# evanwang1990/FMwR

Measured on AMD Instinct MI355X. Metric: training examples/sec, 10Mx1M sparse FM SGD, higher is better.
Workload: dtype f32

## Files before the change

fmwr_amd/_lib.py:

```python
import ctypes as C
import os

_PKG = os.path.dirname(os.path.abspath(__file__))
LIB_PATH = os.environ.get("FMX_LIB_PATH") or os.path.join(_PKG, "libfmx.so")

OK, ERR_INVALID, ERR_HIP, ERR_NOGPU, ERR_STATE = 0, 1, 2, 3, 4
TASK_CLASSIFICATION, TASK_REGRESSION, TASK_RANKING = 10, 20, 30
SOLVER_MCMC, SOLVER_ALS, SOLVER_SGD, SOLVER_FTRL, SOLVER_TDAP = 100, 200, 300, 500, 600
MODE_SEQUENTIAL, MODE_MINIBATCH = 0, 1
LINK_NONE, LINK_LOGISTIC, LINK_CLAMP, LINK_PROBIT = 0, 1, 2, 3
DIV_REL_SCORE, DIV_REL_MINMAX = 0, 1
SIM_COSINE, SIM_DOT = 0, 1
REDUCE_MEAN, REDUCE_SUM = 0, 1
COLUMNS_UNIFORM, COLUMNS_ZIPF = 1, 2
EVAL_LL, EVAL_AUC, EVAL_ACC, EVAL_RMSE, EVAL_MSE, EVAL_MAE = 0, 111, 222, 333, 444, 555
EVAL_PAIR_ACC, EVAL_BPR = 666, 777
KERNEL_ROWS_FORWARD, KERNEL_COLS_UPDATE, KERNEL_SCALAR, KERNEL_SEQ, KERNEL_ALS_SWEEP = 0, 1, 2, 3, 4

SYMBOLS = [
    "fmx_last_error", "fmx_device_count", "fmx_config_default", "fmx_engine_create", "fmx_engine_destroy", "fmx_set_params",
    "fmx_get_params", "fmx_engine_save", "fmx_engine_load", "fmx_matrix_from_rlist", "fmx_matrix_from_dgc", "fmx_matrix_from_csr", "fmx_matrix_synthetic", "fmx_matrix_synthetic_fields", "fmx_matrix_synthetic_iid", "fmx_matrix_synthetic_ragged", "fmx_matrix_synthetic_values", "fmx_train_stream", "fmx_matrix_set_labels", "fmx_matrix_set_fields", "fmx_matrix_destroy",
    "fmx_matrix_info", "fmx_matrix_export", "fmx_matrix_scales", "fmx_matrix_normalize", "fmx_predict", "fmx_train", "fmx_train_grid", "fmx_train_order", "fmx_num_batches",
    "fmx_step", "fmx_grad", "fmx_grad_buffer", "fmx_grad_elem_bytes", "fmx_grad_layout", "fmx_grad_begin", "fmx_grad_chunk", "fmx_apply_chunk", "fmx_apply", "fmx_sync", "fmx_stream", "fmx_predict_device",
    "fmx_als_plan_info", "fmx_als_tiled_info", "fmx_als_order_info", "fmx_als_carry_q", "fmx_als_vsweep", "fmx_mcmc_vsweep", "fmx_als_train", "fmx_mcmc_train", "fmx_mcmc_train_from", "fmx_mcmc_v_hyper", "fmx_evaluate", "fmx_train_tracked", "fmx_trace_size", "fmx_trace_get", "fmx_trace_params",
    "fmx_profile_enable", "fmx_profile_get", "fmx_profile_reset", "fmx_rows_tune_info", "fmx_matrix_rows_form", "fmx_measure_gather", "fmx_measure_gather_occ", "fmx_measure_gather_matrix", "fmx_rccl_selftest",
    "fmx_get_rows", "fmx_set_rows", "fmx_init_normal", "fmx_compact_info", "fmx_compact_count", "fmx_compact_reserve", "fmx_grad_compact", "fmx_compact_records", "fmx_apply_compact",
    "fmx_vsweep_device", "fmx_group_info", "fmx_source_open", "fmx_source_next", "fmx_source_close",
    "fmx_apply_compact_parts", "fmx_layout_info", "fmx_owner_configure", "fmx_owner_info", "fmx_rows_pack", "fmx_rows_unpack",
    "fmx_topk", "fmx_topk_device", "fmx_contrib", "fmx_contrib_device", "fmx_contrib_summary",
    "fmx_matrix_pairs", "fmx_matrix_pairs_hard",
    "fmx_heldout_rank", "fmx_heldout_rank_device", "fmx_heldout_metrics",
    "fmx_rank_lists", "fmx_rank_lists_device", "fmx_topk_lists", "fmx_topk_lists_device", "fmx_project", "fmx_project_device",
    "fmx_fold_in", "fmx_fold_in_pairs",
    "fmx_diversify", "fmx_diversify_device",
    "fmx_neighbors", "fmx_neighbors_device",
    "fmx_interactions", "fmx_interactions_device", "fmx_interactions_summary",
    "fmx_metrics", "fmx_metrics_device",
    "fmx_predict_calibrated", "fmx_predict_calibrated_device", "fmx_reliability", "fmx_reliability_device",
    "fmx_calibrate_platt", "fmx_calibrate_platt_device", "fmx_calibrate_isotonic", "fmx_calibrate_isotonic_device",
    "fmx_matrix_take", "fmx_matrix_take_device", "fmx_split_assign", "fmx_split_assign_device", "fmx_matrix_select", "fmx_matrix_select_device",
    "fmx_free_device", "fmx_matrix_split_entries", "fmx_row_permutation", "fmx_row_permutation_device",
    "fmx_matrix_column_stats", "fmx_matrix_column_stats_device", "fmx_column_map_select", "fmx_column_map_select_device",
    "fmx_column_map_hash", "fmx_column_map_hash_device", "fmx_matrix_remap_columns", "fmx_matrix_remap_columns_device",
]
COLUMNS_BY_ROWS, COLUMNS_BY_ENTRIES = 0, 1
RARE_DROP, RARE_BUCKET = 0, 1
COMBINE_KEEP, COMBINE_SUM, COMBINE_FIRST = 0, 1, 2
COLUMN_DROP = 0xFFFFFFFF
SPLIT_ROWS, SPLIT_WITHIN_GROUPS, SPLIT_GROUPS = 0, 1, 2
SPLIT_ORDER_HASH, SPLIT_ORDER_TAIL = 0, 1
SPLIT_NO_PART = 0xFFFFFFFF
MET_VALUES, MET_COUNTS = 6, 4
MET_AUC, MET_LOGLOSS, MET_ACCURACY, MET_BRIER, MET_MEAN_PRED, MET_MEAN_LABEL = 0, 1, 2, 3, 4, 5
MET_MSE, MET_RMSE, MET_MAE, MET_MEAN_ERR = 0, 1, 2, 3
MET_ROWS, MET_POSITIVES, MET_PAIRS2, MET_CORRECT = 0, 1, 2, 3
CAL_NONE, CAL_PLATT, CAL_STEPS = 0, 1, 2
BINS_WIDTH, BINS_MASS = 0, 1
CAL_VALUES = 4
CAL_ECE, CAL_MCE, CAL_BRIER, CAL_LOGLOSS = 0, 1, 2, 3


TEST_HOOKS = ["fmx_debug_fail_next_plan_build", "fmx_debug_fail_next_comm_init", "fmx_debug_lose_next_seq_multiplier", "fmx_debug_stall_next_persistent_sweep",
              "fmx_debug_contrib_summary_chunk", "fmx_debug_foldin_slab", "fmx_debug_heldout_limits", "fmx_debug_pairs_hard_chunk", "fmx_debug_lists_limits", "fmx_debug_diversify_limits", "fmx_debug_neighbors_limits", "fmx_debug_interactions_limits", "fmx_debug_metrics_limits", "fmx_debug_take_limits", "fmx_debug_calibrate_limits", "fmx_debug_columns_limits", "fmx_debug_matrix_flags", "fmx_debug_cols_launches",
              "fmx_debug_long_launches", "fmx_debug_rows_launches", "fmx_debug_rows_merged_launches",
              "fmx_debug_rows_sched_launches", "fmx_debug_rows_sched_id_limit", "fmx_debug_rows_sched_export",
              "fmx_debug_rows_pace_launches", "fmx_debug_rows_pace_counters", "fmx_debug_rows_pace_counters_of", "fmx_debug_rows_pace_poison", "fmx_debug_rows_pace_trace"]


class Config(C.Structure):
    _fields_ = [
        ("struct_size", C.c_uint32), ("task", C.c_int32), ("solver", C.c_int32), ("num_factor", C.c_int32),
        ("keep_w0", C.c_int32), ("keep_w1", C.c_int32),
        ("l2_w0", C.c_double), ("l1_w1", C.c_double), ("l2_w1", C.c_double), ("l1_v", C.c_double), ("l2_v", C.c_double),
        ("learn_rate", C.c_double),
        ("alpha_w", C.c_double), ("alpha_v", C.c_double), ("beta_w", C.c_double), ("beta_v", C.c_double),
        ("random_step", C.c_int32), ("mode", C.c_int32), ("batch_rows", C.c_int64),
        ("min_target", C.c_double), ("max_target", C.c_double),
        ("device", C.c_int32), ("batch_reduce", C.c_int32), ("gamma", C.c_double), ("tile_rows", C.c_int64),
        ("state_fp64", C.c_int32), ("exchange_chunks", C.c_int32), ("n_gpus", C.c_int32), ("als_max_levels", C.c_int32), ("seq_reassociate", C.c_int32), ("gpus_share_device", C.c_int32),
    ]


class FieldsSpec(C.Structure):
    _fields_ = [("struct_size", C.c_uint32), ("n_dense", C.c_int32), ("n_fields", C.c_int32), ("reserved", C.c_int32),
                ("field_vocab", C.c_void_p), ("skew", C.c_double), ("seed", C.c_uint64)]


class TrackConfig(C.Structure):
    _fields_ = [("struct_size", C.c_uint32), ("metric", C.c_int32), ("step_size", C.c_int64), ("convergence", C.c_double),
                ("keep_params", C.c_int32), ("reserved", C.c_int32)]


class SplitSpec(C.Structure):
    _fields_ = [("struct_size", C.c_uint32), ("scope", C.c_int32), ("order", C.c_int32), ("n_folds", C.c_int32), ("hold_count", C.c_int64),
                ("hold_fraction", C.c_double), ("min_keep", C.c_int64), ("seed", C.c_uint64), ("salt", C.c_uint64)]


class ColumnRule(C.Structure):
    _fields_ = [("struct_size", C.c_uint32), ("by", C.c_int32), ("min_count", C.c_int64), ("max_count", C.c_int64), ("max_features", C.c_int64),
                ("keep_prefix", C.c_uint32), ("rare", C.c_int32), ("n_segments", C.c_int32), ("reserved", C.c_int32), ("segment_base", C.c_void_p)]


class Calibrator(C.Structure):
    _fields_ = [("struct_size", C.c_uint32), ("kind", C.c_int32), ("n_groups", C.c_int64), ("max_steps", C.c_int32), ("link", C.c_int32),
                ("platt", C.c_void_p), ("n_steps", C.c_void_p), ("thr", C.c_void_p), ("val", C.c_void_p)]


class FmxError(RuntimeError):
    def __init__(self, status, message):
        super().__init__(message)
        self.status = status


_lib = None


def lib():
    global _lib
    if _lib is None:
        if not os.path.exists(LIB_PATH):
            raise ImportError(f"{LIB_PATH} is missing: build the HIP library first (python -m fmwr_amd.build). "
                              "fmwr_amd has no CPU fallback.")
        L = C.CDLL(LIB_PATH)
        L.fmx_last_error.restype = C.c_char_p
        for name in SYMBOLS + TEST_HOOKS:
            if name != "fmx_last_error":
                getattr(L, name).restype = C.c_int
        L.fmx_matrix_pairs_hard.argtypes = [C.c_void_p, C.c_void_p, C.c_void_p, C.c_void_p, C.c_int32, C.c_int32, C.c_uint64, C.c_int64,
                                            C.POINTER(C.c_void_p)]
        L.fmx_fold_in.argtypes = [C.c_void_p, C.c_void_p, C.c_void_p, C.c_int64, C.c_double, C.c_double, C.c_int32, C.c_int32, C.c_void_p, C.c_void_p,
                                  C.c_void_p, C.c_void_p]
        L.fmx_fold_in_pairs.argtypes = L.fmx_fold_in.argtypes
        L.fmx_diversify.argtypes = [C.c_void_p, C.c_void_p, C.c_int64, C.c_int32, C.c_void_p, C.c_void_p, C.c_int32, C.c_double, C.c_int32, C.c_void_p,
                                    C.c_void_p, C.c_void_p]
        L.fmx_diversify_device.argtypes = L.fmx_diversify.argtypes
        L.fmx_neighbors.argtypes = [C.c_void_p, C.c_void_p, C.c_void_p, C.c_int32, C.c_int32, C.c_int32, C.c_void_p, C.c_void_p]
        L.fmx_neighbors_device.argtypes = [C.c_void_p, C.c_void_p, C.c_int64, C.c_int64, C.c_void_p, C.c_int32, C.c_int32, C.c_int32, C.c_void_p, C.c_void_p]
        L.fmx_debug_neighbors_limits.argtypes = [C.c_int64, C.c_int64]
        L.fmx_interactions.argtypes = [C.c_void_p, C.c_void_p, C.c_int32, C.c_void_p, C.c_void_p, C.c_void_p]
        L.fmx_interactions_device.argtypes = [C.c_void_p, C.c_void_p, C.c_int64, C.c_int64, C.c_int32, C.c_void_p, C.c_void_p, C.c_void_p]
        L.fmx_interactions_summary.argtypes = [C.c_void_p, C.c_void_p, C.c_void_p, C.c_int32, C.c_void_p, C.c_void_p, C.c_void_p]
        L.fmx_debug_interactions_limits.argtypes = [C.c_int32, C.c_int32, C.c_int64]
        L.fmx_metrics.argtypes = [C.c_void_p, C.c_void_p, C.c_void_p, C.c_int64, C.c_int, C.c_void_p, C.c_void_p]
        L.fmx_metrics_device.argtypes = [C.c_void_p, C.c_void_p, C.c_int64, C.c_int64, C.c_void_p, C.c_int64, C.c_int, C.c_void_p, C.c_void_p]
        L.fmx_debug_metrics_limits.argtypes = [C.c_int32, C.c_int32, C.c_int64]
        L.fmx_predict_calibrated.argtypes = [C.c_void_p, C.c_void_p, C.c_void_p, C.c_int64, C.POINTER(Calibrator), C.c_int, C.c_void_p]
        L.fmx_predict_calibrated_device.argtypes = [C.c_void_p, C.c_void_p, C.c_int64, C.c_int64, C.c_void_p, C.c_int64, C.POINTER(Calibrator), C.c_int, C.c_void_p]
        L.fmx_reliability.argtypes = [C.c_void_p, C.c_void_p, C.c_void_p, C.c_int64, C.c_int32, C.c_int32, C.POINTER(Calibrator), C.c_int] + [C.c_void_p] * 6
        L.fmx_reliability_device.argtypes = [C.c_void_p, C.c_void_p, C.c_int64, C.c_int64, C.c_void_p, C.c_int64, C.c_int32, C.c_int32, C.POINTER(Calibrator),
                                             C.c_int] + [C.c_void_p] * 6
        L.fmx_calibrate_platt.argtypes = [C.c_void_p, C.c_void_p, C.c_void_p, C.c_int64, C.c_double, C.c_int32, C.c_void_p, C.c_void_p, C.c_void_p]
        L.fmx_calibrate_platt_device.argtypes = [C.c_void_p, C.c_void_p, C.c_int64, C.c_int64, C.c_void_p, C.c_int64, C.c_double, C.c_int32, C.c_void_p, C.c_void_p,
                                                 C.c_void_p]
        L.fmx_calibrate_isotonic.argtypes = [C.c_void_p, C.c_void_p, C.c_void_p, C.c_int64, C.c_int32, C.c_void_p, C.c_void_p, C.c_void_p]
        L.fmx_calibrate_isotonic_device.argtypes = [C.c_void_p, C.c_void_p, C.c_int64, C.c_int64, C.c_void_p, C.c_int64, C.c_int32, C.c_void_p, C.c_void_p, C.c_void_p]
        L.fmx_debug_calibrate_limits.argtypes = [C.c_int64]
        L.fmx_matrix_take.argtypes = [C.c_void_p, C.c_void_p, C.c_int64, C.POINTER(C.c_void_p)]
        L.fmx_matrix_take_device.argtypes = L.fmx_matrix_take.argtypes
        L.fmx_split_assign.argtypes = [C.c_int, C.c_int64, C.c_void_p, C.c_int64, C.POINTER(SplitSpec), C.c_void_p]
        L.fmx_split_assign_device.argtypes = L.fmx_split_assign.argtypes
        L.fmx_matrix_select.argtypes = [C.c_void_p, C.c_void_p, C.c_uint32, C.c_int32, C.POINTER(C.c_void_p), C.c_void_p]
        L.fmx_matrix_select_device.argtypes = [C.c_void_p, C.c_void_p, C.c_uint32, C.c_int32, C.POINTER(C.c_void_p), C.POINTER(C.c_void_p)]
        L.fmx_free_device.argtypes = [C.c_void_p]
        L.fmx_matrix_split_entries.argtypes = [C.c_void_p, C.c_int32, C.c_int64, C.c_double, C.c_int64, C.c_uint64, C.c_uint64, C.POINTER(C.c_void_p),
                                               C.POINTER(C.c_void_p)]
        L.fmx_row_permutation.argtypes = [C.c_int, C.c_int64, C.c_uint64, C.c_uint64, C.c_void_p]
        L.fmx_row_permutation_device.argtypes = L.fmx_row_permutation.argtypes
        L.fmx_debug_take_limits.argtypes = [C.c_int32, C.c_int32, C.c_int64]
        L.fmx_matrix_column_stats.argtypes = [C.c_void_p, C.c_void_p, C.c_void_p]
        L.fmx_matrix_column_stats_device.argtypes = L.fmx_matrix_column_stats.argtypes
        L.fmx_column_map_select.argtypes = [C.c_int, C.c_uint32, C.c_void_p, C.POINTER(ColumnRule), C.c_void_p, C.POINTER(C.c_uint32), C.c_void_p]
        L.fmx_column_map_select_device.argtypes = L.fmx_column_map_select.argtypes
        L.fmx_column_map_hash.argtypes = [C.c_int, C.c_uint32, C.c_uint32, C.c_uint64, C.c_uint64, C.c_uint32, C.c_void_p, C.POINTER(C.c_uint32)]
        L.fmx_column_map_hash_device.argtypes = L.fmx_column_map_hash.argtypes
        L.fmx_matrix_remap_columns.argtypes = [C.c_void_p, C.c_void_p, C.c_uint32, C.c_int32, C.POINTER(C.c_void_p)]
        L.fmx_matrix_remap_columns_device.argtypes = L.fmx_matrix_remap_columns.argtypes
        L.fmx_debug_columns_limits.argtypes = [C.c_int32, C.c_int64, C.c_int64]
        L.fmx_debug_matrix_flags.argtypes = [C.c_void_p, C.c_void_p]
        _lib = L
    return _lib


def check(status):
    if status != OK:
        raise FmxError(status, lib().fmx_last_error().decode("utf-8", "replace"))


def default_config():
    cfg = Config()
    check(lib().fmx_config_default(C.byref(cfg)))
    return cfg
```

fmwr_amd/csrc/fm_batch_kernels.hip:

```cpp
#include <atomic>
#include <mutex>
#include <utility>
#include <vector>

#include "fmx_internal.h"
#include "fm_probit.h"
#include "fmx_test_hooks.h"

#ifndef FMX_U
#define FMX_U 4
#endif
#ifndef FMX_SPARSE_WAVES
#define FMX_SPARSE_WAVES 4
#endif
#ifndef FMX_DENSE_WAVES
#define FMX_DENSE_WAVES 4
#endif
#ifndef FMX_U_LARGE
#define FMX_U_LARGE 4
#endif
#ifndef FMX_U_SMALL
#define FMX_U_SMALL 8
#endif

// ... 347 lines not shown
    const int64_t row = R0 + s * NG + gid;
    const int64_t ra = row < a.nrows ? row : a.nrows, rb = row + 1 < a.nrows ? row + 1 : a.nrows;
    const int64_t ta = a.row_ptr[a.r0 + ra] - lo, tb = a.row_ptr[a.r0 + rb] - lo;
    pe[s] = (uint32_t)(ta < cnt ? ta : cnt) | ((uint32_t)(tb < cnt ? tb : cnt) << 16);
  }
  {
    uint32_t id[PER];
#pragma unroll
    for (int u = 0; u < PER; ++u) {
      const int i = tid + u * WG_THREADS;
      id[u] = i < cnt ? a.col[lo + i] : 0u;
    }
#pragma unroll
    for (int u = 0; u < PER; ++u) {
      const int i = tid + u * WG_THREADS;
      if (i < cnt) stage[i] = id[u];
    }
  }
  __syncthreads();

  const T* __restrict__ Vt = reinterpret_cast<const T*>(a.V) + lig * VEC;
  const T* __restrict__ wt = a.w ? reinterpret_cast<const T*>(a.w) : reinterpret_cast<const T*>(a.V);
  const bool k1 = h.k1 != 0;
  const int last = cnt > 0 ? cnt - 1 : 0;
  static_assert(MERGE_STAGE < (1 << 16), "positions are kept in 16 bits");
  uint32_t hd[MERGE_SLOTS];
  int left = 0;
#pragma unroll
  for (int s = 0; s < MERGE_SLOTS; ++s) {
    const int p0 = (int)(pe[s] & 0xFFFFu), p1 = (int)(pe[s] >> 16);
    const uint32_t v = stage[p0 < last ? p0 : last];
    hd[s] = p0 < p1 ? v : DONE;
    left += p1 - p0;
  }
  double sm[MERGE_SLOTS][VEC], qm[MERGE_SLOTS][VEC], lin[MERGE_SLOTS];
#pragma unroll
  for (int s = 0; s < MERGE_SLOTS; ++s) {
#pragma unroll
    for (int i = 0; i < VEC; ++i) { sm[s][i] = 0.0; qm[s][i] = 0.0; }
    lin[s] = h.k0 ? a.scal[SC_W0] : 0.0;
  }

  uint32_t safe = 0u;
  for (; left > 0; left -= U) {
    uint32_t eid[U];
    int esl[U];
#pragma unroll
    for (int u = 0; u < U; ++u) {
      uint32_t best = hd[0];
      int sel = 0;
#pragma unroll
      for (int s = 1; s < MERGE_SLOTS; ++s)
        if (hd[s] < best) { best = hd[s]; sel = s; }
      const bool live = best != DONE;
      eid[u] = live ? best : safe;
      esl[u] = live ? sel : MERGE_SLOTS;
      safe = eid[u];
      uint32_t nxt = 0u;
#pragma unroll
      for (int s = 0; s < MERGE_SLOTS; ++s)
        if (esl[u] == s) { pe[s] += 1u; nxt = pe[s]; }
      const int np = (int)(nxt & 0xFFFFu), ne = (int)(nxt >> 16);
      const uint32_t nx = stage[np < last ? np : last];
      const uint32_t nh = np < ne ? nx : DONE;
#pragma unroll
      for (int s = 0; s < MERGE_SLOTS; ++s)
        if (esl[u] == s) hd[s] = nh;
    }
    float4 vv[U];
    T wv[U];
#pragma unroll
    for (int u = 0; u < U; ++u) {
      vv[u] = gather_row(Vt + ((size_t)eid[u] << RowStride<T, LPR>::v(a.vsh)));
      wv[u] = wt[(size_t)eid[u] << RowStride<T, LPR>::w(a.wsh)];
    }
#pragma unroll
    for (int u = 0; u < U; ++u) {
      const double x = 1.0;
      const double wx = (double)wv[u] * x;
      double tmp[VEC], tsq[VEC];
      slice_get(vv[u], tmp);
#pragma unroll
      for (int i = 0; i < VEC; ++i) { tmp[i] = tmp[i] * x; tsq[i] = tmp[i] * tmp[i]; }
#pragma unroll
      for (int s = 0; s < MERGE_SLOTS; ++s) {
        if (esl[u] == s) {
          if (k1) lin[s] += wx;
#pragma unroll
          for (int i = 0; i < VEC; ++i) {
            sm[s][i] += tmp[i];
            if constexpr (U == 1) qm[s][i] += tsq[i]; else qm[s][i] += tmp[i] * tmp[i];
          }
        }
      }
    }
  }

  int eg = tid / LPR;
  asm volatile("" : "+v"(eg));
#pragma unroll
  for (int s = 0; s < MERGE_SLOTS; ++s) {
    const int64_t row = R0 + s * NG + eg;
    const bool have = row < a.nrows;
    double pair = 0.0;
#pragma unroll
    for (int i = 0; i < VEC; ++i) pair += 0.5 * (sm[s][i] * sm[s][i] - qm[s][i]);
#pragma unroll
    for (int off = LPR / 2; off > 0; off >>= 1) pair += __shfl_xor(pair, off);
    const double y_hat = lin[s] + pair;
    if constexpr (TRAIN) {
      double mult = 0.0;
      if (have) {
        mult = grad_mult(h, y_hat, a.y[a.r0 + row]);
        float4 srow = slice_make(sm[s], T());
        srow = embed_store<LPR>(srow, lig, (float)mult, a.embed);
        *reinterpret_cast<float4*>(reinterpret_cast<T*>(a.S) + (size_t)row * KP + lig * VEC) = srow;
        if (lig == 0) reinterpret_cast<T*>(a.amul)[row] = (T)mult;
      }
      if (lig == 0) red[s * NG + eg] = mult;
    } else {
      if (have && lig == 0 && a.yhat) a.yhat[row] = link_apply(h, y_hat, a.link, a.pn_y);
    }
  }
  if constexpr (TRAIN) {
    __syncthreads();
    if (tid % 64 == 0) {
      const int s = tid / 64;
      if (R0 + (int64_t)s * NG < a.nrows) {
        double g0 = 0.0, q0 = 0.0;
        for (int i = 0; i < NG; ++i) { const double m = red[s * NG + i]; g0 += m; q0 += m * m; }
        a.partials[2 * ((size_t)blockIdx.x * MERGE_SLOTS + s)] = g0;
        a.partials[2 * ((size_t)blockIdx.x * MERGE_SLOTS + s) + 1] = q0;
      }
    }
  }
}

#ifndef FMX_ROWS_PACE_EVERY
#define FMX_ROWS_PACE_EVERY 24
#endif
#ifndef FMX_ROWS_PACE_LEAD
#define FMX_ROWS_PACE_LEAD 2
#endif
#ifndef FMX_ROWS_PACE_SLEEP
#define FMX_ROWS_PACE_SLEEP 30
#endif
constexpr int PACE_MAX_CHECKINS = (SCHED_STAGE_STEPS - 1) / FMX_ROWS_PACE_EVERY;
constexpr int64_t PACE_STEP_CYCLES = 2120;
static_assert((int64_t)PACE_MAX_CHECKINS * 3 * FMX_ROWS_PACE_SLEEP * 64 * 10 <= SCHED_STAGE_STEPS * PACE_STEP_CYCLES, "check-ins x the longest sleep: at most a tenth of the longest block's walk");
static_assert((int64_t)((120 - 1) / FMX_ROWS_PACE_EVERY) * 3 * FMX_ROWS_PACE_SLEEP * 64 * 10 <= 120 * PACE_STEP_CYCLES, "the same for the headline's 120-step blocks");

__device__ __forceinline__ void pace_sleep(int units) {
  switch (units) {
    case 5: __builtin_amdgcn_s_sleep(5); break;
    case 10: __builtin_amdgcn_s_sleep(10); break;
    case 15: __builtin_amdgcn_s_sleep(15); break;
    case 20: __builtin_amdgcn_s_sleep(20); break;
    case 30: __builtin_amdgcn_s_sleep(30); break;
    case 40: __builtin_amdgcn_s_sleep(40); break;
    case 60: __builtin_amdgcn_s_sleep(60); break;
    case 80: __builtin_amdgcn_s_sleep(80); break;
    case 90: __builtin_amdgcn_s_sleep(90); break;
    case 120: __builtin_amdgcn_s_sleep(120); break;
    default: break;
  }
}

template <bool UNIFORM, bool PIPE, bool DEAL = false, bool PACE = false, bool TRACE = false>
__global__ __launch_bounds__(WG_THREADS, 4) void fm_rows_sched_k(RowsArgs a, Hyper h) {
  using T = float;
  constexpr int LPR = 4, VEC = 4, KP = LPR * VEC;
  constexpr int NG = WG_THREADS / LPR;
  constexpr int PER = MERGE_STAGE / WG_THREADS;
  static_assert(MERGE_STAGE == SCHED_STAGE_STEPS * NG && MERGE_SLOTS == 4, "the stage holds SCHED_STAGE_STEPS steps of one word per lane group");
  static_assert(UNIFORM || !PIPE, "only the unrolled walk has a round to request together");
  static_assert(!(UNIFORM && DEAL), "a DEAL schedule is walked as a MERGE one");
  static_assert(!(UNIFORM && (PACE || TRACE)), "the pace and its trace belong to the MERGE and DEAL walks");
  __shared__ uint32_t stage[MERGE_STAGE];
  __shared__ double red[MERGE_RPW];
  __shared__ uint32_t places[DEAL ? NG : 1];
  __shared__ uint32_t pace_box;

  const int tid = threadIdx.x;
  const int gid = tid / LPR;
  const int lig = tid % LPR;
  const int64_t R0 = (int64_t)blockIdx.x * MERGE_RPW;
  if constexpr (PACE) { if (tid == 0) pace_box = 0u; }
  const uint32_t w_hi = a.sched_dir[blockIdx.x + 1];
  uint32_t w_lo = a.sched_dir[blockIdx.x];
  if constexpr (DEAL) {
    const bool hdr = w_hi - w_lo >= (uint32_t)NG;
    if (tid < NG) places[tid] = hdr ? a.sched[(size_t)w_lo + tid] : 0u;
    w_lo += hdr ? (uint32_t)NG : 0u;
  }
  const int cnt = (w_hi - w_lo < (uint32_t)MERGE_STAGE) ? (int)(w_hi - w_lo) : MERGE_STAGE;
  const int steps = UNIFORM ? (cnt / NG) & ~3 : cnt / NG;
  {
    uint32_t id[PER];
#pragma unroll
    for (int u = 0; u < PER; ++u) {
      const int i = tid + u * WG_THREADS;
      id[u] = i < cnt ? a.sched[(size_t)w_lo + i] : SCHED_BUBBLE;
    }
#pragma unroll
    for (int u = 0; u < PER; ++u) {
      const int i = tid + u * WG_THREADS;
      if (i < cnt) stage[i] = id[u];
    }
  }
  __syncthreads();

  const __amdgpu_buffer_rsrc_t v_rsrc = table_rsrc(a.V, a.sched_vbytes);
  const __amdgpu_buffer_rsrc_t w_rsrc = table_rsrc(a.w ? a.w : a.V, a.w ? a.sched_wbytes : a.sched_vbytes);
  const bool k1 = h.k1 != 0;
  const int vsh = RowStride<T, LPR>::v(a.vsh) + 2, wsh = RowStride<T, LPR>::w(a.wsh) + 2;
  const uint32_t lane_off = (uint32_t)(lig * VEC * sizeof(T));
  double sm[MERGE_SLOTS][VEC], qm[MERGE_SLOTS][VEC], lin[MERGE_SLOTS];
#pragma unroll
  for (int s = 0; s < MERGE_SLOTS; ++s) {
#pragma unroll
    for (int i = 0; i < VEC; ++i) { sm[s][i] = 0.0; qm[s][i] = 0.0; }
    lin[s] = h.k0 ? a.scal[SC_W0] : 0.0;
  }
  const uint32_t* __restrict__ mine = stage + gid;

  if constexpr (UNIFORM) {
    for (int t = 0; t < steps; t += MERGE_SLOTS) {
      uint32_t wd[MERGE_SLOTS];
#pragma unroll
      for (int j = 0; j < MERGE_SLOTS; ++j) wd[j] = mine[(t + j) * NG];
      float4 vv[MERGE_SLOTS];
      T wv[MERGE_SLOTS];
      if constexpr (PIPE) {
#pragma unroll
        for (int j = 0; j < MERGE_SLOTS; ++j) {
          const bool live = wd[j] != SCHED_BUBBLE;
          const uint32_t c = wd[j] & SCHED_MAX_P;
          vv[j] = buf_row(v_rsrc, live ? (c << vsh) + lane_off : BUF_SKIP, T());
          wv[j] = buf_elem(w_rsrc, live ? c << wsh : BUF_SKIP, T());
        }
      }
#pragma unroll
      for (int j = 0; j < MERGE_SLOTS; ++j) {
        if constexpr (!PIPE) {
          const bool live = wd[j] != SCHED_BUBBLE;
          const uint32_t c = wd[j] & SCHED_MAX_P;
          vv[j] = buf_row(v_rsrc, live ? (c << vsh) + lane_off : BUF_SKIP, T());
          wv[j] = buf_elem(w_rsrc, live ? c << wsh : BUF_SKIP, T());
          asm volatile("s_waitcnt vmcnt(0)" ::: "memory");
        }
        const double x = 1.0;
        const double wx = (double)wv[j] * x;
        double tmp[VEC], tsq[VEC];
        slice_get(vv[j], tmp);
#pragma unroll
        for (int i = 0; i < VEC; ++i) { tmp[i] = tmp[i] * x; tsq[i] = tmp[i] * tmp[i]; }
        if (k1) lin[j] += wx;
#pragma unroll
        for (int i = 0; i < VEC; ++i) { sm[j][i] += tmp[i]; qm[j][i] += tsq[i]; }
      }
    }
  } else {
    uint32_t* pace_ctr = nullptr;
    int64_t pace_groups = 0;
    int pace_at = 0, pace_k = 0, pace_slept = 0;
    uint32_t pace_seen = 0;
    if constexpr (PACE) {
      const uint32_t lab = blockIdx.x & 7u;
      pace_ctr = a.pace + (size_t)(a.pace_set * 8 + (int)lab) * PACE_LINE;
      pace_groups = (int64_t)(a.pace_div + (lab < a.pace_rem ? 1u : 0u));
      pace_at = a.pace_every;
      if (blockIdx.x == 0 && tid < 8 && a.pace_zero)
        __hip_atomic_store(a.pace + (size_t)((a.pace_set ^ 1) * 8 + tid) * PACE_LINE, 0u, __ATOMIC_RELAXED, __HIP_MEMORY_SCOPE_AGENT);
    }
    uint64_t* trace = nullptr;
    if constexpr (TRACE) trace = a.pace_trace + ((size_t)blockIdx.x * (WG_THREADS / 64) + tid / 64) * PACE_TRACE_WORDS;
    for (int t = 0; t < steps; ++t) {
      if constexpr (TRACE) {
        if ((t & 15) == 0 && (tid & 63) == 0) trace[1 + (t >> 4)] = __builtin_amdgcn_s_memrealtime();
      }
      const uint32_t wd = mine[t * NG];
      const bool live = wd != SCHED_BUBBLE;
      const uint32_t c = wd & SCHED_MAX_P;
      const int esl = live ? (int)(wd >> 30) : MERGE_SLOTS;
      const float4 vv = buf_row(v_rsrc, live ? (c << vsh) + lane_off : BUF_SKIP, T());
      const T wv = buf_elem(w_rsrc, live ? c << wsh : BUF_SKIP, T());
      const double x = 1.0;
      const double wx = (double)wv * x;
      double tmp[VEC], tsq[VEC];
      slice_get(vv, tmp);
#pragma unroll
      for (int i = 0; i < VEC; ++i) { tmp[i] = tmp[i] * x; tsq[i] = tmp[i] * tmp[i]; }
#pragma unroll
      for (int s = 0; s < MERGE_SLOTS; ++s) {
        if (esl == s) {
          if (k1) lin[s] += wx;
#pragma unroll
          for (int i = 0; i < VEC; ++i) { sm[s][i] += tmp[i]; qm[s][i] += tsq[i]; }
        }
      }
      if constexpr (PACE) {
        if (t == pace_at) {
          ++pace_k;
          if (tid == 64 * (pace_k & 3)) pace_seen = __hip_atomic_fetch_add(pace_ctr, a.pace_inc, __ATOMIC_RELAXED, __HIP_MEMORY_SCOPE_AGENT);
        } else if (t == pace_at + 1) {
          if (tid == 64 * (pace_k & 3))
            __hip_atomic_store(&pace_box, (uint32_t)pace_k << 24 | (pace_seen < 0xFFFFFFu ? pace_seen : 0xFFFFFFu), __ATOMIC_RELAXED, __HIP_MEMORY_SCOPE_WORKGROUP);
          const uint32_t box = (uint32_t)__builtin_amdgcn_readfirstlane((int)__hip_atomic_load(&pace_box, __ATOMIC_RELAXED, __HIP_MEMORY_SCOPE_WORKGROUP));
          const int64_t k = (int64_t)(box >> 24), seen = (int64_t)(box & 0xFFFFFFu);
          const int64_t lead2 = 2 * (int64_t)a.pace_every * (k * pace_groups - seen) - (int64_t)(a.pace_every - 1) * pace_groups;
          const int64_t thr2 = 2 * (int64_t)a.pace_lead * pace_groups;
          const int level = k == 0 ? 0 : lead2 > 3 * thr2 ? 3 : lead2 > 2 * thr2 ? 2 : lead2 > thr2 ? 1 : 0;
          if (level) { pace_sleep(level * a.pace_sleep); pace_slept += 1 + (level << 16); }
          pace_at += a.pace_every;
        }
      }
    }
    if constexpr (TRACE) {
      if ((tid & 63) == 0) {
        trace[1 + ((steps + 15) >> 4)] = __builtin_amdgcn_s_memrealtime();
        trace[0] = (uint64_t)(__builtin_amdgcn_s_getreg((31 << 11) | 20) & 15u) | (uint64_t)steps << 8 | (uint64_t)pace_slept << 32;
      }
    }
  }

  int eg = tid / LPR;
  asm volatile("" : "+v"(eg));
  uint32_t place = 0;
  if constexpr (DEAL) place = places[eg];
#pragma unroll
  for (int s = 0; s < MERGE_SLOTS; ++s) {
    const int at = DEAL ? (int)((place >> (8 * s)) & 255u) : s * NG + eg;
    const int64_t row = R0 + at;
    const bool have = row < a.nrows;
    double pair = 0.0;
#pragma unroll
    for (int i = 0; i < VEC; ++i) pair += 0.5 * (sm[s][i] * sm[s][i] - qm[s][i]);
#pragma unroll
    for (int off = LPR / 2; off > 0; off >>= 1) pair += __shfl_xor(pair, off);
    const double y_hat = lin[s] + pair;
    double mult = 0.0;
    if (have) {
      mult = grad_mult(h, y_hat, a.y[a.r0 + row]);
      float4 srow = slice_make(sm[s], T());
      srow = embed_store<LPR>(srow, lig, (float)mult, a.embed);
      *reinterpret_cast<float4*>(reinterpret_cast<T*>(a.S) + (size_t)row * KP + lig * VEC) = srow;
      if (lig == 0) reinterpret_cast<T*>(a.amul)[row] = (T)mult;
    }
    if (lig == 0) red[at] = mult;
  }
  __syncthreads();
  if (tid % 64 == 0) {
    const int s = tid / 64;
    if (R0 + (int64_t)s * NG < a.nrows) {
      double g0 = 0.0, q0 = 0.0;
      for (int i = 0; i < NG; ++i) { const double m = red[s * NG + i]; g0 += m; q0 += m * m; }
      a.partials[2 * ((size_t)blockIdx.x * MERGE_SLOTS + s)] = g0;
      a.partials[2 * ((size_t)blockIdx.x * MERGE_SLOTS + s) + 1] = q0;
    }
  }
}

template <typename T, int LPR, bool TRAIN>
__global__ __launch_bounds__(WG_THREADS) void fm_rows_forward_dyn_k(RowsArgs a, Hyper h) {
  using vec_t = typename Slice<T>::vec;
  constexpr int VEC = Slice<T>::N;
  constexpr int KP = LPR * VEC;
  constexpr int GROUPS = WG_THREADS / LPR;
  constexpr int RPW = 4 * GROUPS;
  constexpr int RU = FMX_U_LARGE;
  constexpr int PER = (RU + LPR - 1) / LPR;
  __shared__ int next_row;
  __shared__ double red[TRAIN ? RPW : 1];
  const int tid = threadIdx.x;
  const int grp = tid / LPR, lig = tid % LPR;
  const int lane0 = (tid & 63) - lig;
  const int64_t R0 = (int64_t)blockIdx.x * RPW;
  const int rows_here = (int)((R0 + RPW < a.nrows ? R0 + RPW : a.nrows) - R0);
  if (tid == 0) next_row = GROUPS;
  if (TRAIN) for (int i = tid; i < RPW; i += WG_THREADS) red[i] = 0.0;
  __syncthreads();
  const T* __restrict__ Vt = reinterpret_cast<const T*>(a.V) + lig * VEC;
  const T* __restrict__ wt = a.w ? reinterpret_cast<const T*>(a.w) : reinterpret_cast<const T*>(a.V);
  const bool k1 = h.k1 != 0;
  const int64_t last = a.row_ptr[a.r0 + R0 + rows_here] - 1;
  int r = grp;
  while (r < rows_here) {
    const int64_t ta = a.row_ptr[a.r0 + R0 + r], tb = a.row_ptr[a.r0 + R0 + r + 1];
    double s[VEC], q[VEC];
#pragma unroll
    for (int i = 0; i < VEC; ++i) { s[i] = 0.0; q[i] = 0.0; }
    double lin = h.k0 ? a.scal[SC_W0] : 0.0;
    auto load_round = [&](int64_t t, uint32_t* id, uint32_t* xb) {
#pragma unroll
      for (int v = 0; v < PER; ++v) {
        const int64_t at = t + lig + v * LPR;
        const int64_t ac = at <= last ? (at >= 0 ? at : 0) : (last >= 0 ? last : 0);
        id[v] = a.col[ac];
        xb[v] = a.unit ? 0x3f800000u : __float_as_uint(a.val[ac]);
      }
    };
    uint32_t cid[PER], cxb[PER], nid[PER], nxb[PER];
    load_round(ta, cid, cxb);
    for (int64_t t = ta; t < tb; t += RU) {
      load_round(t + RU, nid, nxb);
      uint2 en[RU];
#pragma unroll
      for (int u = 0; u < RU; ++u) {
        en[u].x = (uint32_t)__shfl((int)cid[u / LPR], lane0 + (u % LPR));
        en[u].y = (uint32_t)__shfl((int)cxb[u / LPR], lane0 + (u % LPR));
      }
#pragma unroll
      for (int u = 1; u < RU; ++u)
        if (t + u >= tb) en[u] = make_uint2(en[0].x, 0u);
      vec_t vv[RU];
      T wv[RU];
#pragma unroll
      for (int u = 0; u < RU; ++u) {
        vv[u] = gather_row(Vt + ((size_t)en[u].x << RowStride<T, LPR>::v(a.vsh)));
        wv[u] = wt[(size_t)en[u].x << RowStride<T, LPR>::w(a.wsh)];
        if (a.serial) asm volatile("s_waitcnt vmcnt(0)" ::: "memory");
      }
#pragma unroll
      for (int u = 0; u < RU; ++u) {
        const double x = (double)__uint_as_float(en[u].y);
        if (k1) lin += (double)wv[u] * x;
        double vf[VEC];
        slice_get(vv[u], vf);
#pragma unroll
        for (int i = 0; i < VEC; ++i) {
          const double tmp = vf[i] * x;
          s[i] += tmp;
          q[i] += tmp * tmp;
        }
      }
#pragma unroll
      for (int v = 0; v < PER; ++v) { cid[v] = nid[v]; cxb[v] = nxb[v]; }
    }
    double pair = 0.0;
#pragma unroll
    for (int i = 0; i < VEC; ++i) pair += 0.5 * (s[i] * s[i] - q[i]);
#pragma unroll
    for (int off = LPR / 2; off > 0; off >>= 1) pair += __shfl_xor(pair, off);
    const double y_hat = lin + pair;
    const int64_t row = R0 + r;
    if constexpr (TRAIN) {
      const double mult = grad_mult(h, y_hat, a.y[a.r0 + row]);
      vec_t srow = slice_make(s, T());
      if constexpr (sizeof(T) == 4) srow = embed_store<LPR>(srow, lig, (float)mult, a.embed);
      *reinterpret_cast<vec_t*>(reinterpret_cast<T*>(a.S) + (size_t)row * KP + lig * VEC) = srow;
      if (lig == 0) { reinterpret_cast<T*>(a.amul)[row] = (T)mult; red[r] = mult; }
    } else {
      if (lig == 0 && a.yhat) a.yhat[row] = link_apply(h, y_hat, a.link, a.pn_y);
      if constexpr (sizeof(T) == 8) {
        if (a.qout) {
          if (a.qout_t > 0) { a.qout[(size_t)(lig * VEC) * a.qout_t + row] = s[0]; a.qout[(size_t)(lig * VEC + 1) * a.qout_t + row] = s[1]; }
          else *reinterpret_cast<double2*>(a.qout + (size_t)row * KP + lig * VEC) = make_double2(s[0], s[1]);
        }
      } else if (a.qout) {
        double2* q2 = reinterpret_cast<double2*>(a.qout + (size_t)row * KP + lig * VEC);
        q2[0] = make_double2(s[0], s[1]);
        q2[1] = make_double2(s[2], s[3]);
      }
    }
    int nr = 0;
    if (lig == 0) nr = atomicAdd(&next_row, 1);
    r = __shfl(nr, lane0);
  }
// ... 261 lines not shown
    count_rows_launch(counted, wide_form);
    return launch_rows_t<T, TRAIN, WG_THREADS, 1, true>(e, a, kp);
  }
  if (a.sort_rows && a.wg_threads != 64) { count_rows_launch(counted, ROWS_PULL); return launch_rows_dyn<T, TRAIN>(e, a, kp); }
  if (a.flat == 1 && a.wg_threads != 64) { count_rows_launch(counted, ROWS_FLAT); return launch_rows_flat<T, TRAIN>(e, a, kp); }
  if (a.wg_threads == 64) {
    count_rows_launch(counted, a.split == 4 ? ROWS_NARROW4 : ROWS_NARROW1);
    return a.split == 4 ? launch_rows_t<T, TRAIN, 64, 4>(e, a, kp) : launch_rows_t<T, TRAIN, 64, 1>(e, a, kp);
  }
  count_rows_launch(counted, wide_form);
  return launch_rows_t<T, TRAIN, WG_THREADS, 1>(e, a, kp);
}

static std::atomic<int64_t> g_rows_merged[2];
void debug_rows_merged_launches(int64_t out[2]) {
  for (int i = 0; i < 2; ++i) out[i] = g_rows_merged[i].load();
}
#ifndef FMX_ROWS_MERGE_U_DEFAULT
#define FMX_ROWS_MERGE_U_DEFAULT 1
#endif
static int rows_merge_mode() { static const int v = [] { const char* s = getenv("FMX_ROWS_MERGE"); return s ? atoi(s) : 1; }(); return v; }
static int rows_merge_u() {
  static const int v = [] { const char* s = getenv("FMX_ROWS_MERGE_U"); const int u = s ? atoi(s) : FMX_ROWS_MERGE_U_DEFAULT; return (u == 1 || u == 2) ? u : FMX_ROWS_MERGE_U_DEFAULT; }();
  return v;
}

template <bool TRAIN, int U>
static int64_t rows_merged_fill(const fmx_engine* e) {
  constexpr int MAX_DEV = 64;
  static std::atomic<int64_t> fill_dev[MAX_DEV];
  std::atomic<int64_t>& fill = fill_dev[(e->cfg.device >= 0 && e->cfg.device < MAX_DEV) ? e->cfg.device : 0];
  int64_t v = fill.load();
  if (v == 0) {
    hipDeviceProp_t pr{};
    const int cus = (hipGetDeviceProperties(&pr, e->cfg.device) == hipSuccess && pr.multiProcessorCount > 0) ? pr.multiProcessorCount : 256;
    int per = 0;
    if (hipOccupancyMaxActiveBlocksPerMultiprocessor(&per, fm_rows_merged_k<float, 4, TRAIN, U>, WG_THREADS, 0) != hipSuccess || per <= 0) per = 4;
    v = (int64_t)per * cus * MERGE_RPW;
    fill.store(v);
  }
  return v;
}

__global__ __launch_bounds__(WG_THREADS) void rows_block_max_k(const int64_t* __restrict__ row_ptr, int64_t r0, int64_t nrows, int64_t* __restrict__ out) {
  __shared__ int64_t part[WG_THREADS];
  const int64_t blocks = (nrows + MERGE_RPW - 1) / MERGE_RPW;
  int64_t m = 0;
  for (int64_t b = threadIdx.x; b < blocks; b += WG_THREADS) {
    const int64_t r1 = (b + 1) * MERGE_RPW < nrows ? (b + 1) * MERGE_RPW : nrows;
    const int64_t c = row_ptr[r0 + r1] - row_ptr[r0 + b * MERGE_RPW];
    m = c > m ? c : m;
  }
  part[threadIdx.x] = m;
  __syncthreads();
  if (threadIdx.x == 0) {
    for (int i = 1; i < WG_THREADS; ++i) m = part[i] > m ? part[i] : m;
    out[0] = m;
  }
}

static int rows_merged_fits(fmx_engine* e, const RowsArgs& a, bool* fits) {
  if ((int64_t)a.max_row_len * MERGE_RPW <= MERGE_STAGE) { *fits = true; return FMX_OK; }
  struct Key { uint64_t uid; int64_t r0, nrows; };
  static std::mutex mu;
  static std::vector<std::pair<Key, bool>> known;
  {
    std::lock_guard<std::mutex> g(mu);
    for (const auto& k : known)
      if (k.first.uid == a.mat_uid && k.first.r0 == a.r0 && k.first.nrows == a.nrows) { *fits = k.second; return FMX_OK; }
  }
  int64_t* d = nullptr;
  int64_t most = 0;
  FMX_HIP(hipMalloc(&d, sizeof(int64_t)));
  hipLaunchKernelGGL(rows_block_max_k, dim3(1), dim3(WG_THREADS), 0, e->stream, a.row_ptr, a.r0, a.nrows, d);
  hipError_t err = hipGetLastError();
  if (err == hipSuccess) err = hipMemcpyAsync(&most, d, sizeof(int64_t), hipMemcpyDeviceToHost, e->stream);
  if (err == hipSuccess) err = hipStreamSynchronize(e->stream);
  (void)hipFree(d);
  FMX_HIP(err);
  *fits = most <= MERGE_STAGE;
  std::lock_guard<std::mutex> g(mu);
  if (known.size() >= 4096) known.clear();
  known.push_back({Key{a.mat_uid, a.r0, a.nrows}, *fits});
  return FMX_OK;
}

template <bool TRAIN, int U>
static int launch_rows_merged_u(fmx_engine* e, const RowsArgs& a, int mode, bool* ran) {
  const size_t v_bytes = ((size_t)e->p << a.vsh) * sizeof(float);
  if (mode != 2 && (a.nrows < rows_merged_fill<TRAIN, U>(e) || a.col_skew != 1 || v_bytes <= MERGE_MIN_TABLE)) return FMX_OK;
  bool fits = false;
  FMX_TRY(rows_merged_fits(e, a, &fits));
  if (!fits) { g_rows_merged[1]++; return FMX_OK; }
  const int64_t grid = (a.nrows + MERGE_RPW - 1) / MERGE_RPW;
  FMX_CHECK(grid < (1LL << 31), FMX_ERR_INVALID, "rows_forward: grid too large (%lld)", (long long)grid);
  hipLaunchKernelGGL((fm_rows_merged_k<float, 4, TRAIN, U>), dim3((unsigned)grid), dim3(WG_THREADS), 0, e->stream, a, e->hyper);
  FMX_HIP(hipGetLastError());
  g_rows_merged[0]++;
  *ran = true;
  return FMX_OK;
}

template <bool TRAIN>
static int launch_rows_merged(fmx_engine* e, const RowsArgs& a, bool fp64_tables, bool* ran) {
  *ran = false;
  const int mode = rows_merge_mode();
  if (mode == 0 || fp64_tables || e->kp32 != 16 || !a.unit || a.qout || a.no_w || a.wg_threads == 64 || a.sort_rows || a.flat == 1) return FMX_OK;
  if (TRAIN && e->cfg.task == FMX_TASK_RANKING) return FMX_OK;
  if (a.nrows <= 0 || a.max_row_len <= 0 || a.mat_uid == 0) return FMX_OK;
  switch (rows_merge_u()) {
    case 2: return launch_rows_merged_u<TRAIN, 2>(e, a, mode, ran);
    default: return launch_rows_merged_u<TRAIN, 1>(e, a, mode, ran);
  }
}

#ifndef FMX_ROWS_SCHED_DEFAULT
#define FMX_ROWS_SCHED_DEFAULT 1
#endif
#ifndef FMX_ROWS_SCHED_POLICY_DEFAULT
#define FMX_ROWS_SCHED_POLICY_DEFAULT SCHED_DEAL
#endif
#ifndef FMX_ROWS_SCHED_RHO_DEFAULT
#define FMX_ROWS_SCHED_RHO_DEFAULT 1024
#endif
static std::atomic<int64_t> g_rows_sched[3];
void debug_rows_sched_launches(int64_t out[3]) {
  for (int i = 0; i < 3; ++i) out[i] = g_rows_sched[i].load();
}
void rows_sched_count_build() { g_rows_sched[2]++; }
static int rows_sched_mode() {
  static const int v = [] { const char* s = getenv("FMX_ROWS_SCHED"); return s ? atoi(s) : (getenv("FMX_ROWS_MERGE") ? 0 : FMX_ROWS_SCHED_DEFAULT); }();
  return v;
}
static int rows_sched_policy() {
  static const int v = [] {
    const char* s = getenv("FMX_ROWS_SCHED_POLICY");
    if (!s) return (int)FMX_ROWS_SCHED_POLICY_DEFAULT;
    return s[0] == 'm' ? (int)SCHED_MERGE : s[0] == 'f' ? (int)SCHED_FRONT : s[0] == 'r' ? (int)SCHED_ROUND : s[0] == 'd' ? (int)SCHED_DEAL : (int)FMX_ROWS_SCHED_POLICY_DEFAULT;
  }();
  return v;
}
static int rows_sched_rho_q() {
  static const int v = [] {
    const char* s = getenv("FMX_ROWS_SCHED_RHO");
    if (!s) return (int)FMX_ROWS_SCHED_RHO_DEFAULT;
    const double r = atof(s);
    return r <= 0.0 ? 0 : r >= 1.0 ? 1024 : (int)(r * 1024.0 + 0.5);
  }();
  return v;
}
static int rows_sched_u() { static const int v = [] { const char* s = getenv("FMX_ROWS_SCHED_U"); return (s && atoi(s) == 4) ? 4 : 1; }(); return v; }

#ifndef FMX_ROWS_PACE_DEFAULT
#define FMX_ROWS_PACE_DEFAULT 1
#endif
static std::atomic<int64_t> g_rows_pace[2];
void debug_rows_pace_launches(int64_t out[2]) {
  for (int i = 0; i < 2; ++i) out[i] = g_rows_pace[i].load();
}
static int rows_pace_mode() {
  static const int v = [] { const char* s = getenv("FMX_ROWS_PACE"); const int m = s ? atoi(s) : FMX_ROWS_PACE_DEFAULT; return (m >= 0 && m <= 2) ? m : FMX_ROWS_PACE_DEFAULT; }();
  return v;
}
static bool rows_pace_trace_on() { static const bool v = [] { const char* s = getenv("FMX_ROWS_PACE_TRACE"); return s && s[0] == '1'; }(); return v; }
struct PaceTune { int every, lead, sleep; };
static const PaceTune& rows_pace_tune() {
  static const PaceTune v = [] {
    PaceTune t{FMX_ROWS_PACE_EVERY, FMX_ROWS_PACE_LEAD, FMX_ROWS_PACE_SLEEP};
    int ev = 0, ld = 0, sl = 0;
    const char* s = getenv("FMX_ROWS_PACE_TUNE");
    if (s && sscanf(s, "%d,%d,%d", &ev, &ld, &sl) == 3 && ev >= 2 && ev <= 64 && ld >= 0 && ld <= 64 && (sl == 5 || sl == 10 || sl == 20 || sl == 30 || sl == 40)) t = PaceTune{ev, ld, sl};
    return t;
  }();
  return v;
}
int debug_rows_pace_counters(fmx_engine* e, uint32_t out[16]) {
  for (int i = 0; i < 16; ++i) out[i] = 0;
  if (!e->rows_pace) return FMX_OK;
  std::vector<uint32_t> all(PACE_WORDS);
  FMX_HIP(hipStreamSynchronize(e->stream));
  FMX_HIP(hipMemcpy(all.data(), e->rows_pace, PACE_WORDS * sizeof(uint32_t), hipMemcpyDeviceToHost));
  for (int i = 0; i < 16; ++i) out[i] = all[(size_t)i * PACE_LINE];
  return FMX_OK;
}
int debug_rows_pace_trace(fmx_engine* e, uint64_t* out, int64_t cap_words, int64_t* waves) {
  *waves = e->rows_pace_trace ? e->rows_pace_trace_waves : 0;
  if (*waves == 0 || !out) return FMX_OK;
  FMX_CHECK(cap_words >= *waves * PACE_TRACE_WORDS, FMX_ERR_INVALID, "rows_pace_trace: %lld words for %lld waves", (long long)cap_words, (long long)*waves);
  FMX_HIP(hipStreamSynchronize(e->stream));
  FMX_HIP(hipMemcpy(out, e->rows_pace_trace, (size_t)*waves * PACE_TRACE_WORDS * sizeof(uint64_t), hipMemcpyDeviceToHost));
  return FMX_OK;
}

bool rows_sched_wanted(fmx_engine* e, const RowsArgs& a, int* policy, int* rho_q) {
  const int mode = rows_sched_mode();
  if (mode == 0 || mb_wide(e) || e->kp32 != 16 || !a.unit || a.qout || a.no_w || a.wg_threads == 64 || a.sort_rows || a.flat == 1) return false;
  if (e->cfg.task == FMX_TASK_RANKING || a.nrows <= 0 || a.max_row_len <= 0 || a.mat_uid == 0 || !a.w) return false;
  const uint64_t v_bytes = (uint64_t)e->p * (uint64_t)a.vs * sizeof(float), w_bytes = (uint64_t)e->p * (uint64_t)a.ws * sizeof(float);
  if (v_bytes >= BUF_SKIP || w_bytes >= BUF_SKIP || e->p > SCHED_MAX_P) return false;
  if (mode != 2 && (a.nrows < rows_merged_fill<true, 1>(e) || a.col_skew != 1 || v_bytes <= MERGE_MIN_TABLE)) return false;
  *policy = rows_sched_policy();
  *rho_q = (*policy == SCHED_MERGE || *policy == SCHED_DEAL) ? 0 : rows_sched_rho_q();
  return true;
}

static int launch_rows_sched(fmx_engine* e, const RowsArgs& a_in, bool* ran) {
  *ran = false;
  if (a_in.sched_state == 0) return FMX_OK;
  int policy = 0, rho_q = 0;
  if (!rows_sched_wanted(e, a_in, &policy, &rho_q)) return FMX_OK;
  if (a_in.sched_state != 1 || !a_in.sched || !a_in.sched_dir) { g_rows_sched[1]++; return FMX_OK; }
  RowsArgs a = a_in;
  a.sched_vbytes = (uint32_t)((uint64_t)e->p * (uint64_t)a.vs * sizeof(float));
  a.sched_wbytes = (uint32_t)((((uint64_t)e->p - 1) * (uint64_t)a.ws + 1) * sizeof(float));
  const int64_t grid = (a.nrows + MERGE_RPW - 1) / MERGE_RPW;
  FMX_CHECK(grid < (1LL << 31), FMX_ERR_INVALID, "rows_forward: grid too large (%lld)", (long long)grid);
  if (!a.sched_uniform) {
    const int mode = rows_pace_mode();
    const bool traced = rows_pace_trace_on();
    using SchedKernel = void (*)(RowsArgs, Hyper);
    static const SchedKernel instance[2][2][2] = {
        {{fm_rows_sched_k<false, false, false, false, false>, fm_rows_sched_k<false, false, false, false, true>},
         {fm_rows_sched_k<false, false, false, true, false>, fm_rows_sched_k<false, false, false, true, true>}},
        {{fm_rows_sched_k<false, false, true, false, false>, fm_rows_sched_k<false, false, true, false, true>},
         {fm_rows_sched_k<false, false, true, true, false>, fm_rows_sched_k<false, false, true, true, true>}}};
    const int deal = a.sched_deal ? 1 : 0;
    bool paced = false;
    if (mode != 0 && e->rows_pace) {
      constexpr int MAX_DEV = 64;
      static std::atomic<int64_t> resident_dev[MAX_DEV][2][2];
      std::atomic<int64_t>& resident = resident_dev[(e->cfg.device >= 0 && e->cfg.device < MAX_DEV) ? e->cfg.device : 0][deal][traced ? 1 : 0];
      int64_t r = resident.load();
      if (r == 0) {
        hipDeviceProp_t pr{};
        int per = 0;
        if (hipGetDeviceProperties(&pr, e->cfg.device) == hipSuccess && pr.multiProcessorCount > 0 &&
            hipOccupancyMaxActiveBlocksPerMultiprocessor(&per, instance[deal][1][traced ? 1 : 0], WG_THREADS, 0) == hipSuccess && per > 0)
          r = (int64_t)per * pr.multiProcessorCount;
        else r = -1;
        resident.store(r);
      }
      paced = r > 0 && grid <= r;
    }
    if (paced) {
      const PaceTune& pt = rows_pace_tune();
      a.pace = e->rows_pace;
      a.pace_set = (int)(e->rows_pace_launches & 1);
      a.pace_zero = e->rows_pace_poisoned ? 0 : 1;
      a.pace_inc = e->rows_pace_poisoned ? 0u : 1u;
      a.pace_div = (uint32_t)(grid / 8); a.pace_rem = (uint32_t)(grid % 8);
      a.pace_every = pt.every; a.pace_lead = pt.lead; a.pace_sleep = pt.sleep;
      if (e->rows_pace_poisoned) FMX_HIP(hipMemsetD32Async((hipDeviceptr_t)e->rows_pace, (int)e->rows_pace_poison, PACE_WORDS, e->stream));
    }
    if (traced) {
      const int64_t waves = grid * (WG_THREADS / 64);
      if (waves > e->rows_pace_trace_cap) {
        FMX_HIP(hipStreamSynchronize(e->stream));
        (void)hipFree(e->rows_pace_trace); e->rows_pace_trace = nullptr; e->rows_pace_trace_cap = 0;
        FMX_HIP(hipMalloc(&e->rows_pace_trace, (size_t)waves * PACE_TRACE_WORDS * sizeof(uint64_t)));
        e->rows_pace_trace_cap = waves;
      }
      FMX_HIP(hipMemsetAsync(e->rows_pace_trace, 0, (size_t)waves * PACE_TRACE_WORDS * sizeof(uint64_t), e->stream));
      e->rows_pace_trace_waves = waves;
      a.pace_trace = e->rows_pace_trace;
    }
    hipLaunchKernelGGL(instance[deal][paced ? 1 : 0][traced ? 1 : 0], dim3((unsigned)grid), dim3(WG_THREADS), 0, e->stream, a, e->hyper);
    FMX_HIP(hipGetLastError());
    if (paced) ++e->rows_pace_launches;
    g_rows_pace[paced ? 0 : 1]++;
    g_rows_sched[0]++;
    *ran = true;
    return FMX_OK;
  }
  if (rows_sched_u() == 4) hipLaunchKernelGGL((fm_rows_sched_k<true, true>), dim3((unsigned)grid), dim3(WG_THREADS), 0, e->stream, a, e->hyper);
  else hipLaunchKernelGGL((fm_rows_sched_k<true, false>), dim3((unsigned)grid), dim3(WG_THREADS), 0, e->stream, a, e->hyper);
  FMX_HIP(hipGetLastError());
  g_rows_pace[1]++;
  g_rows_sched[0]++;
  *ran = true;
  return FMX_OK;
}

int launch_rows_forward(fmx_engine* e, const RowsArgs& a_in, bool train, bool fp64_tables) {
  RowsArgs a = a_in;
  FMX_CHECK(a.vs >= (fp64_tables ? e->kp64 : e->kp32) && a.ws >= 1 && (a.vs & (a.vs - 1)) == 0 && (a.ws & (a.ws - 1)) == 0, FMX_ERR_STATE,
            "rows_forward: table strides not set (%d, %d)", a.vs, a.ws);
  {
    const int kp = fp64_tables ? e->kp64 : e->kp32;
    FMX_CHECK((!fp64_tables && kp <= WIR_MAX_KP) || (a.vs == kp && a.ws == 1), FMX_ERR_STATE, "rows_forward: strides (%d, %d) on a table of compiled strides (%d, 1)",
              a.vs, a.ws, kp);
  }
  a.vsh = __builtin_ctz((unsigned)a.vs); a.wsh = __builtin_ctz((unsigned)a.ws);
  static const bool embed_ok = [] { const char* v = getenv("FMX_EMBED_MULT"); return !(v && v[0] == '0'); }();
  static const int force = [] { const char* v = getenv("FMX_ROWS_SERIAL"); return v ? atoi(v) : -1; }();
  RowsTune& tu = e->rows_tune;
  auto pick = [&](const RowsArgs& r, int* serial, int* trial) -> int {
    *trial = -1;
    *serial = 1;
    if (force >= 0) { *serial = force; return FMX_OK; }
    const bool timed = r.wg_threads != 64 && r.nrows >= RowsTune::MIN_ROWS;
    const int64_t key = r.unit ? 1 : 0;
    if (timed && key != tu.key) {
      if (tu.events && tu.launches > 0 && tu.decided < 0) FMX_HIP(hipStreamSynchronize(e->stream));
      tu.key = key; tu.decided = -1; tu.launches = 0;
    }
    if (tu.decided >= 0) { *serial = tu.decided; return FMX_OK; }
    if (!timed) return FMX_OK;
    if (!tu.events) {
      bool ok = true;
      for (auto& ev : tu.ev) ok = ok && hipEventCreate(&ev) == hipSuccess;
      FMX_CHECK(ok, FMX_ERR_HIP, "rows_forward: could not create the tuning events");
      tu.events = true;
    }
    if (tu.launches >= RowsTune::TRIALS) {
      tu.decided = 1;
      return FMX_OK;
    }
    *trial = tu.launches++;
    *serial = *trial % 2 == 0 ? 1 : 0;
    FMX_HIP(hipEventRecord(tu.ev[2 * *trial], e->stream));
    return FMX_OK;
  };
  auto done = [&](int trial) -> int {
    if (trial < 0) return FMX_OK;
    FMX_HIP(hipEventRecord(tu.ev[2 * trial + 1], e->stream));
    if (tu.launches >= RowsTune::TRIALS && tu.decided < 0) {
      FMX_HIP(hipEventSynchronize(tu.ev[2 * trial + 1]));
      double ms[2] = {0.0, 0.0};
      for (int i = 2; i < RowsTune::TRIALS; ++i) {
        float t = 0.f;
        FMX_HIP(hipEventElapsedTime(&t, tu.ev[2 * i], tu.ev[2 * i + 1]));
        ms[i % 2 == 0 ? 1 : 0] += t;
      }
      tu.ms[0] = ms[0]; tu.ms[1] = ms[1];
      tu.decided = ms[1] <= ms[0] ? 1 : 0;
    }
    return FMX_OK;
  };
  a.embed = (train && embed_ok) ? embed_mode(e->k, fp64_tables ? e->kp64 : e->kp32, !fp64_tables) : EMBED_NONE;
  prof_begin(e, FMX_KERNEL_ROWS_FORWARD);
  int st = FMX_OK;
  bool merged = false;
  if (train) {
    st = launch_rows_sched(e, a, &merged);
    if (st == FMX_OK && !merged) st = launch_rows_merged<true>(e, a, fp64_tables, &merged);
    if (st == FMX_OK && !merged) {
      int trial;
      FMX_TRY(pick(a, &a.serial, &trial));
      st = fp64_tables ? launch_rows_w<double, true>(e, a, e->kp64) : launch_rows_w<float, true>(e, a, e->kp32);
      { const int st2 = done(trial); if (st == FMX_OK) st = st2; }
    }
  } else {
    const int64_t SLAB = 1 << 18;
    const int kp = fp64_tables ? e->kp64 : e->kp32;
    for (int64_t off = 0; off < a.nrows && st == FMX_OK; off += SLAB) {
      RowsArgs s = a;
      s.r0 = a.r0 + off;
      s.nrows = a.nrows - off < SLAB ? a.nrows - off : SLAB;
      if (a.yhat) s.yhat = a.yhat + off;
      if (a.qout) s.qout = a.qout_t > 0 ? a.qout + off : a.qout + (size_t)off * kp;
      s.wg_threads = a.fixed_schedule ? WG_THREADS : rows_wg_threads(a.nrows, kp / (fp64_tables ? 2 : 4));
      s.split = a.fixed_schedule ? 1 : rows_split(a.nrows, kp / (fp64_tables ? 2 : 4));
      st = launch_rows_merged<false>(e, s, fp64_tables, &merged);
      if (st != FMX_OK || merged) continue;
      int trial;
      FMX_TRY(pick(s, &s.serial, &trial));
      st = fp64_tables ? launch_rows_w<double, false>(e, s, kp) : launch_rows_w<float, false>(e, s, kp);
      { const int st2 = done(trial); if (st == FMX_OK) st = st2; }
    }
  }
  prof_end(e);
  return st;
}

template <typename ST>
__device__ __forceinline__ void tail_put_rows(ST* gtail, double rows) {
  const double hi = floor(rows / 4096.0);
  gtail[2] = (ST)hi;
  gtail[3] = (ST)(rows - hi * 4096.0);
}
template <typename ST>
__device__ __forceinline__ double tail_get_rows(const ST* gtail) { return (double)gtail[2] * 4096.0 + (double)gtail[3]; }

template <typename ST>
__device__ __forceinline__ void scalar_update(const double* __restrict__ partials, int64_t n_partials, const double* sin,
                                              double* sout, ST* gtail, const Hyper& h, double rows, int mode,
                                              double* sg, double* sq) {
  const int phase = (mode == SCALAR_PUBLISH) ? 1 : (mode == SCALAR_FROM_TAIL) ? 2 : 0;
  double g0 = 0.0, q0 = 0.0;
  if (phase != 2) {
    for (int64_t i = threadIdx.x; i < n_partials; i += WG_THREADS) { g0 += partials[2 * i]; q0 += partials[2 * i + 1]; }
  }
  sg[threadIdx.x] = g0; sq[threadIdx.x] = q0;
  __syncthreads();
  for (int off = WG_THREADS / 2; off > 0; off >>= 1) {
    if ((int)threadIdx.x < off) { sg[threadIdx.x] += sg[threadIdx.x + off]; sq[threadIdx.x] += sq[threadIdx.x + off]; }
    __syncthreads();
  }
  if (threadIdx.x != 0) return;
  g0 = sg[0]; q0 = sq[0];
  if (phase == 1) { gtail[0] = (ST)g0; gtail[1] = (ST)q0; tail_put_rows(gtail, rows); return; }
  if (phase == 2) { g0 = gtail[0]; q0 = gtail[1]; if (rows <= 0.0) rows = tail_get_rows(gtail); }
  for (int i = 0; i < SC_COUNT; ++i) sout[i] = sin[i];
  if (h.task == FMX_TASK_RANKING) {
    sout[SC_G0] = 0.0; sout[SC_Q0] = 0.0;
    if (h.kind == UPD_SGD_L1) {
      const double steps = (h.mean && rows > 0.0) ? 1.0 : rows;
      sout[SC_UW] = sin[SC_UW] + steps * (h.lr * h.regw);
      sout[SC_UV] = sin[SC_UV] + steps * (h.lr * h.regv);
    }
    return;
  }
  sout[SC_G0] = g0; sout[SC_Q0] = q0;
  if (h.mean && rows > 0.0) {
    g0 /= rows;
    q0 = g0 * g0;
    rows = 1.0;
  }
  const double w0 = sin[SC_W0];
  if (h.kind == UPD_TDAP) {
    double u = sin[SC_N0], nu = sin[SC_T_NU], dl = sin[SC_T_DELTA], hh = sin[SC_T_H], z0 = sin[SC_Z0];
    if (h.k0) {
      const double u_new = u + q0;
      nu += g0;
      const double sigma = (sqrt(u_new) - sqrt(u)) / h.alpha_w;
      const double age = rows == 1.0 ? h.egamma : exp(-h.gamma * rows);
      dl = age * (dl + sigma);
      hh = age * (hh + sigma * w0);
      u = u_new;
      z0 = nu - hh;
    }
    sout[SC_N0] = u; sout[SC_T_NU] = nu; sout[SC_T_DELTA] = dl; sout[SC_T_H] = hh; sout[SC_Z0] = z0;
    sout[SC_W0] = -z0 / dl;
  } else if (h.kind == UPD_FTRL) {
    double z0 = sin[SC_Z0], n0 = sin[SC_N0];
    if (h.k0) {
      const double n_new = n0 + q0;
      z0 += g0 - w0 * (sqrt(n_new) - sqrt(n0)) / h.alpha_w;
      n0 = n_new;
    }
    sout[SC_Z0] = z0; sout[SC_N0] = n0;
    sout[SC_W0] = -z0 * h.alpha_w / (h.beta_w + sqrt(n0));
  } else {
    if (h.kind == UPD_SGD_L1) {
      sout[SC_UW] = sin[SC_UW] + rows * (h.lr * h.regw);
      sout[SC_UV] = sin[SC_UV] + rows * (h.lr * h.regv);
    }
    if (h.k0) sout[SC_W0] = w0 - h.lr * (g0 + rows * h.reg0 * w0);
  }
}

template <typename ST>
struct ColsTables {
  ST *V, *w, *sV, *sw, *nV, *nw;
  ST *t1V, *t1w, *t2V, *t2w, *t3V, *t3w;
  const ST* S;
  const ST* amul;
  const double* scal;
  double* scal_out;
  const double* partials;
  int64_t n_partials;
  ST* gbuf;
  uint32_t p;
  int has_q;
  uint32_t gb_feats;
  int64_t gb_block_elems;
  ST* gtail;
  int64_t s_rows;
  ST* crec;
  int rec_elems;
  int w_full;
  int vsh, wsh;
  int vs, ws;
};

__device__ __forceinline__ float id_to_elem(uint32_t id, float) { return __uint_as_float(id); }
__device__ __forceinline__ double id_to_elem(uint32_t id, double) { return __longlong_as_double((long long)id); }
__device__ __forceinline__ uint32_t elem_to_id(float v) { return __float_as_uint(v); }
__device__ __forceinline__ uint32_t elem_to_id(double v) { return (uint32_t)__double_as_longlong(v); }

__device__ __forceinline__ void apply_penalty(double& theta, double u, double& q) {
  const double old = theta;
  if (theta > 0) theta = fmax(0.0, old - (u + q));
  else if (theta < 0) theta = fmin(0.0, old + (u - q));
  q += theta - old;
}

__device__ __forceinline__ double ftrl_prox(double z, double n, double l1, double l2, double alpha, double beta) {
  if (fabs(z) <= l1) return 0.0;
  const double sign = z < 0.0 ? -1.0 : 1.0;
  return -(z - sign * l1) / ((beta + sqrt(n)) / alpha + l2);
}

template <int KIND, typename ST>
__device__ __forceinline__ double coord_update(const Hyper& h, bool is_w, double theta, double G, double Q, double cnt,
                                               double decay, double u, ST& st_a, ST& st_b, bool keep) {
  if constexpr (KIND == UPD_SGD_L2) {
// ... 1081 lines not shown
```

fmwr_amd/csrc/fmx_api.hip:

```cpp
#include <algorithm>
#include <cmath>
#include <cstdlib>
#include <cstring>
#include <ctime>
#include <atomic>
#include <memory>

#include "fmx_internal.h"
#include "fmx_test_hooks.h"
#include "fm_probit.h"

namespace fmx {

static thread_local std::string g_error;

void set_error(const char* fmt, ...) {
  char buf[1024];
  va_list ap;
  va_start(ap, fmt);
  vsnprintf(buf, sizeof(buf), fmt, ap);
  va_end(ap);
  g_error = buf;
}

void prof_begin(fmx_engine* e, int kernel) {
  e->prof_open = 0;
  if (!e->profile) return;
  if ((e->prof_seen[kernel]++ % e->profile) != 0) return;
  hipEvent_t a, b;
  if (hipEventCreate(&a) != hipSuccess || hipEventCreate(&b) != hipSuccess) return;
  (void)hipEventRecord(a, e->stream);
  e->prof_pending.push_back({kernel, {a, b}});
  e->prof_open = 1;
}

void prof_end(fmx_engine* e) {
  if (!e->prof_open || e->prof_pending.empty()) return;
  e->prof_open = 0;
  (void)hipEventRecord(e->prof_pending.back().second.second, e->stream);
}

static int prof_collect(fmx_engine* e) {
  if (e->prof_pending.empty()) return FMX_OK;
  FMX_HIP(hipStreamSynchronize(e->stream));
  for (auto& pr : e->prof_pending) {
    float ms = 0.f;
    if (hipEventElapsedTime(&ms, pr.second.first, pr.second.second) == hipSuccess) {
      e->prof_ms[pr.first] += ms;
      e->prof_n[pr.first] += 1;
    }
    (void)hipEventDestroy(pr.second.first);
    (void)hipEventDestroy(pr.second.second);
  }
  e->prof_pending.clear();
  return FMX_OK;
}

int use_device(int device) {
  int count = 0;
  hipError_t err = hipGetDeviceCount(&count);
  if (err != hipSuccess || count <= 0) {
    set_error("no HIP device available (%s); libfmx has no CPU fallback", err == hipSuccess ? "device count 0" : hipGetErrorString(err));
    return FMX_ERR_NOGPU;
  }
  FMX_CHECK(device >= 0 && device < count, FMX_ERR_INVALID, "device %d out of range (0..%d)", device, count - 1);
  FMX_HIP(hipSetDevice(device));
  return FMX_OK;
}

int seq_abort_check(fmx_engine* e) {
  if (!e->cfg.seq_reassociate && !getenv("FMX_SEQ_REASSOC")) return FMX_OK;
  double flag = 0.0;
  FMX_HIP(hipMemcpy(&flag, e->scal + SC_SEQ_ABORT, sizeof(double), hipMemcpyDeviceToHost));
  FMX_CHECK(flag == 0.0, FMX_ERR_HIP, "the reassociated sequential learner gave up waiting inside a launch (its workgroup's waves did not all run?): the parameters are not a valid state");
  return FMX_OK;
}

template <typename T>
static int dev_alloc_zero(T** ptr, size_t count) {
  const size_t bytes = (count ? count : 1) * sizeof(T);
  FMX_HIP(hipMalloc(ptr, bytes));
  FMX_HIP(hipMemset(*ptr, 0, bytes));
  return FMX_OK;
}

static int make_hyper(const fmx_config& c, Hyper* h) {
  h->task = c.task;
  h->k0 = c.keep_w0 != 0;
  h->k1 = c.keep_w1 != 0;
  h->lr = c.learn_rate;
  h->reg0 = c.l2_w0;
  h->l1w = c.l1_w1; h->l1v = c.l1_v; h->l2w = c.l2_w1; h->l2v = c.l2_v;
  h->alpha_w = c.alpha_w; h->alpha_v = c.alpha_v; h->beta_w = c.beta_w; h->beta_v = c.beta_v;
  h->min_t = c.min_target; h->max_t = c.max_target;
  h->mean = (c.batch_reduce == FMX_REDUCE_MEAN);
  h->egamma = std::exp(-c.gamma);
  h->gamma = c.gamma;
  if (c.solver == FMX_SOLVER_FTRL || c.solver == FMX_SOLVER_TDAP) {
    h->kind = c.solver == FMX_SOLVER_FTRL ? UPD_FTRL : UPD_TDAP;
    h->regw = 0; h->regv = 0;
  } else {
    bool l1 = false;
    if (c.l1_w1 > 0 || c.l1_v > 0) {
      l1 = true;
      h->regw = c.l1_w1; h->regv = c.l1_v;
    } else {
      h->regw = c.l2_w1; h->regv = c.l2_v;
    }
    if (c.task == FMX_TASK_REGRESSION) l1 = false;
    h->kind = l1 ? UPD_SGD_L1 : UPD_SGD_L2;
  }
  h->decay_w = 1.0 - h->lr * h->regw;
  h->decay_v = 1.0 - h->lr * h->regv;
  h->log_decay_w = h->decay_w > 0 ? std::log(h->decay_w) : 0.0;
  h->log_decay_v = h->decay_v > 0 ? std::log(h->decay_v) : 0.0;
  return FMX_OK;
}

static bool seq_mode(const fmx_engine* e) { return e->cfg.mode == FMX_MODE_SEQUENTIAL; }
static bool ranking(const fmx_engine* e) { return e->cfg.task == FMX_TASK_RANKING; }

static int check_pairs(const fmx_engine* e, const fmx_matrix* m, int64_t rows, const char* what) {
  if (!ranking(e)) return FMX_OK;
  FMX_CHECK(m->n % 2 == 0, FMX_ERR_INVALID, "a ranking engine trains on pair matrices (rows 2t, 2t + 1): this matrix has an odd row count (%lld)", (long long)m->n);
  FMX_CHECK(rows % 2 == 0, FMX_ERR_INVALID, "a ranking engine needs an even %s (got %lld): a step may not split a pair", what, (long long)rows);
  return FMX_OK;
}

static int reset_optimizer_state(fmx_engine* e) {
  const size_t p = e->p;
  double zeros[SC_COUNT] = {0};
  double w0 = 0;
  FMX_HIP(hipMemcpy(&w0, e->scal + SC_W0, sizeof(double), hipMemcpyDeviceToHost));
  zeros[SC_W0] = w0;
  FMX_HIP(hipMemcpy(e->scal, zeros, sizeof(zeros), hipMemcpyHostToDevice));
  if (e->sV) FMX_HIP(hipMemset(e->sV, 0, p * e->kp32 * sizeof(float)));
  if (e->sw) FMX_HIP(hipMemset(e->sw, 0, p * sizeof(float)));
  if (e->nV) FMX_HIP(hipMemset(e->nV, 0, p * e->kp32 * sizeof(float)));
  if (e->nw) FMX_HIP(hipMemset(e->nw, 0, p * sizeof(float)));
  for (float* t : {e->t1V, e->t2V, e->t3V}) if (t) FMX_HIP(hipMemset(t, 0, p * e->kp32 * sizeof(float)));
  for (float* t : {e->t1w, e->t2w, e->t3w}) if (t) FMX_HIP(hipMemset(t, 0, p * sizeof(float)));
  if (e->dsV) FMX_HIP(hipMemset(e->dsV, 0, p * e->kp64 * sizeof(double)));
  if (e->dsw) FMX_HIP(hipMemset(e->dsw, 0, p * sizeof(double)));
  if (e->dnV) FMX_HIP(hipMemset(e->dnV, 0, p * e->kp64 * sizeof(double)));
  if (e->dnw) FMX_HIP(hipMemset(e->dnw, 0, p * sizeof(double)));
  for (double* t : {e->dt1V, e->dt2V, e->dt3V}) if (t) FMX_HIP(hipMemset(t, 0, p * e->kp64 * sizeof(double)));
  for (double* t : {e->dt1w, e->dt2w, e->dt3w}) if (t) FMX_HIP(hipMemset(t, 0, p * sizeof(double)));
  return FMX_OK;
}

static int ensure_workspace(fmx_engine* e, int64_t s_rows, int64_t step_rows, int64_t tiles_per_step) {
  const int rpw = WG_THREADS / mb_lpr(e);
  const int64_t partials = (step_rows + rpw - 1) / rpw + (tiles_per_step > 0 ? tiles_per_step : 1) + 8 + 4096;
  if (!e->rows_pace) {
    FMX_HIP(hipMalloc(&e->rows_pace, PACE_WORDS * sizeof(uint32_t)));
    FMX_HIP(hipMemsetAsync(e->rows_pace, 0, PACE_WORDS * sizeof(uint32_t), e->stream));
  }
  if (s_rows <= e->ws_rows && partials <= e->ws_partials) return FMX_OK;
  FMX_HIP(hipStreamSynchronize(e->stream));
  (void)hipFree(e->S); (void)hipFree(e->amul); (void)hipFree(e->partials);
  e->S = nullptr; e->amul = nullptr; e->partials = nullptr; e->ws_rows = 0; e->ws_partials = 0;
  FMX_HIP(hipMalloc(&e->S, (size_t)s_rows * mb_kp(e) * mb_elem(e)));
  FMX_HIP(hipMalloc(&e->amul, (size_t)s_rows * mb_elem(e)));
  FMX_HIP(hipMalloc(&e->partials, (size_t)partials * 2 * sizeof(double)));
  e->ws_rows = s_rows;
  e->ws_partials = partials;
  return FMX_OK;
}

static int ensure_gbuf(fmx_engine* e) {
  if (e->gbuf) return FMX_OK;
  const bool has_q = exchange_has_q(e);
  const int64_t chunks = e->cfg.exchange_chunks > 1 ? e->cfg.exchange_chunks : 1;
  const int64_t per = ((int64_t)e->p + chunks - 1) / chunks;
  e->gb_feats = chunks > 1 ? (per + 63) / 64 * 64 : ((int64_t)e->p + 3) / 4 * 4;
  e->gb_blocks = ((int64_t)e->p + e->gb_feats - 1) / e->gb_feats;
  e->gb_block_elems = e->gb_feats * mb_kp(e) * (has_q ? 2 : 1) + e->gb_feats * (has_q ? 3 : 2);
  e->gbuf_floats = e->gb_blocks * e->gb_block_elems + 4;
  FMX_HIP(hipMalloc(&e->gbuf, (size_t)e->gbuf_floats * mb_elem(e)));
  FMX_HIP(hipMemset(e->gbuf, 0, (size_t)e->gbuf_floats * mb_elem(e)));
  FMX_HIP(hipDeviceSynchronize());
  return FMX_OK;
}

static uint32_t random_select(int n) {
  if (n == 1) return 1;
  return (uint32_t)((rand() / ((double)RAND_MAX + 1)) * n + 1);
}

struct VisitOrder {
  int64_t n;
  int step;
  uint64_t i = 0;
  bool in_pass = false;
  int idle = 0;
  VisitOrder(int64_t n_, int step_) : n(n_), step(step_) {}
  bool pending = false;
  bool next(int64_t count, std::vector<int64_t>* out) {
    out->clear();
    out->reserve((size_t)count);
    size_t pass_start = 0;
    while ((int64_t)out->size() < count) {
      if (!in_pass) { i = random_select(step); in_pass = true; pending = false; pass_start = out->size(); }
      else if (pending) { i += random_select(step); pending = false; }
      if (i < (uint64_t)n) {
        out->push_back((int64_t)i);
        pending = true;
        idle = 0;
      } else {
        in_pass = false;
        if (out->size() == pass_start && ++idle > 1000) return false;
      }
    }
    return true;
  }
};

void free_matrix(fmx_matrix* m) {
  if (!m) return;
  (void)hipFree(m->row_ptr); (void)hipFree(m->col); (void)hipFree(m->val); (void)hipFree(m->y);
  drop_plans(m);
  (void)hipFree(m->col_ptr); (void)hipFree(m->crow); (void)hipFree(m->cval); (void)hipFree(m->als_feats); (void)hipFree(m->als_heavy); (void)hipFree(m->als_level_ptr_dev); (void)hipFree(m->als_rank);
  (void)hipFree(m->als_vh); (void)hipFree(m->als_vh_seg0); (void)hipFree(m->als_vseg_feat); (void)hipFree(m->als_vseg_b); (void)hipFree(m->als_vseg_e); (void)hipFree(m->als_vh_work);
  als_tiled_free(m);
  delete m;
}

int alloc_matrix(int device, int64_t n, uint32_t p, int64_t nnz, bool labels, fmx_matrix** out) {
  FMX_CHECK(out != nullptr, FMX_ERR_INVALID, "out is NULL");
  *out = nullptr;
  FMX_CHECK(n >= 0 && nnz >= 0, FMX_ERR_INVALID, "negative size");
  FMX_TRY(use_device(device));
  std::unique_ptr<fmx_matrix, void (*)(fmx_matrix*)> m(new fmx_matrix(), free_matrix);
  static std::atomic<uint64_t> next_uid{1};
  m->uid = next_uid.fetch_add(1);
  m->device = device; m->n = n; m->p = p; m->nnz = nnz; m->has_labels = labels;
  FMX_HIP(hipMalloc(&m->row_ptr, ((size_t)n + 1) * sizeof(int64_t)));
  FMX_HIP(hipMalloc(&m->col, ((size_t)nnz + 1) * sizeof(uint32_t)));
  FMX_HIP(hipMalloc(&m->val, ((size_t)nnz + 1) * sizeof(float)));
  FMX_HIP(hipMalloc(&m->y, ((size_t)n + 1) * sizeof(float)));
  FMX_HIP(hipMemset(m->y, 0, ((size_t)n + 1) * sizeof(float)));
  *out = m.release();
  return FMX_OK;
}

int check_pair(const fmx_engine* e, const fmx_matrix* m) {
  FMX_CHECK(e && m, FMX_ERR_INVALID, "NULL handle");
  FMX_CHECK((uint64_t)m->p == e->p, FMX_ERR_INVALID, "number of input's features is not correct...");
  FMX_CHECK(m->device == e->cfg.device, FMX_ERR_INVALID, "matrix lives on device %d, engine on %d", m->device, e->cfg.device);
  return FMX_OK;
}

int forward_rows(fmx_engine* e, const fmx_matrix* m, int64_t r0, int64_t r1, double* d_out, int link) {
  FMX_CHECK(link >= FMX_LINK_NONE && link <= FMX_LINK_PROBIT, FMX_ERR_INVALID, "unknown link %d", link);
  if (link == FMX_LINK_PROBIT) FMX_TRY(ensure_probit(e));
  RowsArgs a{};
  a.row_ptr = m->row_ptr; a.col = m->col; a.val = m->val; a.y = nullptr;
  a.r0 = r0; a.nrows = r1 - r0;
  if (wide_state(e)) { a.V = e->dV; a.w = e->dw; a.vs = e->kp64; a.ws = 1; }
  else { a.V = e->V; a.w = mb_wbase(e); a.vs = e->vstride32; a.ws = mb_wstride(e); }
  a.scal = e->scal;
  a.yhat = d_out;
  a.link = link;
  a.pn_y = e->probit;
  a.unit = m->unit_values;
  a.sort_rows = rows_ragged(m);
  a.flat = rows_flat(m); a.nmat = m->n;
  a.mat_uid = m->uid; a.max_row_len = m->max_row_len;
  for (const auto& pl : m->plans) { const int s = rows_col_skew(m, pl); a.col_skew = s > a.col_skew ? s : a.col_skew; }
  FMX_TRY(launch_rows_forward(e, a, false, wide_state(e)));
  return FMX_OK;
}

int ensure_probit(fmx_engine* e) {
  if (e->probit) return FMX_OK;
  std::vector<double> t((size_t)PN_POINTS + 1 + DP_POINTS + 1);
  for (int i = 0; i < PN_POINTS; ++i) t[(size_t)i] = 0.5 * std::erfc(-pn_x(i) / std::sqrt(2.0));
  t[PN_POINTS] = t[PN_POINTS - 1];
  double* dp = t.data() + PN_POINTS + 1;
  for (int i = 0; i < DP_POINTS; ++i) {
    const double x = dp_x(i);
    const double r = std::exp(-0.5 * x * x) / std::sqrt(2.0 * 3.14159265358979323846) / (1.0 - 0.5 * std::erfc(-x / std::sqrt(2.0)));
    dp[i] = std::round(r * 1e12) / 1e12;
  }
  dp[DP_POINTS] = dp[DP_POINTS - 1];
  FMX_HIP(hipMalloc(&e->probit, t.size() * sizeof(double)));
  FMX_HIP(hipMemcpy(e->probit, t.data(), t.size() * sizeof(double), hipMemcpyHostToDevice));
  return FMX_OK;
}

static int64_t effective_tile_rows(const fmx_engine* e) {
  const int64_t want = e->cfg.tile_rows > 0 ? e->cfg.tile_rows : (e->kp32 >= 16 ? 524288 : 262144);
  if (e->cfg.batch_rows <= want) return e->cfg.batch_rows;
  const int64_t tiles = (e->cfg.batch_rows + want - 1) / want;
  const int64_t rows = (e->cfg.batch_rows + tiles - 1) / tiles;
  return (ranking(e) && rows % 2 != 0) ? rows + 1 : rows;
}

struct TileRun {
  int64_t tile;
  int64_t r0;
  int64_t nrows;
};

static int step_tiles(fmx_engine* e, fmx_matrix* m, int64_t batch, int64_t rows_limit, std::vector<TileRun>* out, int64_t* step_rows) {
  FMX_CHECK(!seq_mode(e), FMX_ERR_STATE, "step interface needs FMX_MODE_MINIBATCH");
  FMX_CHECK(m->has_labels || ranking(e), FMX_ERR_STATE, "there are no labels in data");
  FMX_TRY(check_pairs(e, m, rows_limit, "rows_limit"));
  const int64_t tile = effective_tile_rows(e);
  FMX_TRY(build_batch_csc(m, e->cfg.batch_rows, tile, e->stream));
  FMX_CHECK(batch >= 0 && batch < m->n_batches, FMX_ERR_INVALID, "batch %lld out of range (0..%lld)", (long long)batch, (long long)m->n_batches - 1);
  const int64_t step_cap = e->cfg.batch_rows < m->n ? e->cfg.batch_rows : (m->n > 0 ? m->n : 1);
  FMX_TRY(ensure_workspace(e, tile < step_cap ? tile : step_cap, step_cap, (step_cap + tile - 1) / tile));
  out->clear();
  int64_t left = rows_limit > 0 ? rows_limit : (int64_t)1 << 62;
  int64_t total = 0;
  for (int64_t t = m->step_first_tile[(size_t)batch]; t < m->step_first_tile[(size_t)batch + 1] && left > 0; ++t) {
    const auto& pl = m->plans[(size_t)t];
    int64_t nrows = pl.nrows;
    if (nrows > left) nrows = left;
    FMX_CHECK(!ranking(e) || (pl.r0 % 2 == 0 && nrows % 2 == 0), FMX_ERR_INVALID, "a ranking step's rows [%lld, +%lld) split a pair", (long long)pl.r0, (long long)nrows);
    out->push_back({t, pl.r0, nrows});
    left -= nrows;
    total += nrows;
  }
  *step_rows = total;
  return FMX_OK;
}

static int rows_phase(fmx_engine* e, fmx_matrix* m, const TileRun& t, int64_t step_rows, int64_t partial_offset, int64_t* n_partials, int64_t s_row0 = 0) {
  RowsArgs a{};
  a.row_ptr = m->row_ptr; a.col = m->col; a.val = m->val; a.y = m->y;
  a.r0 = t.r0; a.nrows = t.nrows;
  a.V = mb_vbase(e); a.w = mb_wbase(e); a.vs = mb_vstride(e); a.ws = mb_wstride(e);
  a.scal = e->scal;
  a.S = (char*)e->S + (size_t)s_row0 * mb_kp(e) * mb_elem(e);
  a.amul = (char*)e->amul + (size_t)s_row0 * mb_elem(e);
  a.partials = e->partials + 2 * partial_offset;
  a.unit = m->unit_values;
  a.sort_rows = rows_ragged(m);
  a.wg_threads = rows_wg_threads(step_rows, mb_lpr(e));
  a.split = rows_split(step_rows, mb_lpr(e));
  a.flat = rows_flat(m); a.nmat = m->n;
  a.mat_uid = m->uid; a.max_row_len = m->max_row_len; a.col_skew = rows_col_skew(m, m->plans[(size_t)t.tile]);
  {
    int policy = 0, rho_q = 0;
    if (rows_sched_wanted(e, a, &policy, &rho_q)) {
      FMX_TRY(rows_sched_build(m, policy, rho_q, e->stream));
      const auto& S = m->rows_sched;
      const auto& pl = m->plans[(size_t)t.tile];
      if (S.dir && S.generation == m->plan_generation && (size_t)t.tile < S.tile_words.size() && pl.r0 == t.r0 && pl.nrows == t.nrows) {
        if (S.tile_words[(size_t)t.tile] >= 0) {
          a.sched = S.words + S.tile_words[(size_t)t.tile];
          a.sched_dir = S.dir + S.tile_dir[(size_t)t.tile];
          a.sched_uniform = S.policy == SCHED_ROUND ? 1 : 0;
          a.sched_deal = S.policy == SCHED_DEAL ? 1 : 0;
          a.sched_state = 1;
        } else a.sched_state = 2;
      }
    }
  }
  const int rpw = a.wg_threads / (mb_lpr(e) * (a.wg_threads == 64 && a.split == 4 ? 4 : 1));
  *n_partials = (a.flat == 1 && !a.sort_rows && a.wg_threads != 64) ? rows_flat_blocks(t.r0, t.nrows, rpw) : (t.nrows + rpw - 1) / rpw;
  return launch_rows_forward(e, a, true, mb_wide(e));
}

static int cols_args(fmx_engine* e, fmx_matrix* m, const TileRun& t, bool sparse_ok, ColsArgs* out) {
  const auto& pl = m->plans[(size_t)t.tile];
  ColsArgs c{};
  c.brow = m->brow + pl.base;
  c.bval = m->bval + pl.base;
  c.rows_active = (uint32_t)t.nrows;
  c.walk = 1;
  c.unit = m->unit_values;
  if (pl.feat && sparse_ok) {
    c.tfeat = pl.feat; c.toff = pl.soff; c.n_tfeat = pl.n_lists;
    c.trow0 = pl.row0; c.tval0 = pl.val0;
    c.list_entries = pl.cnt;
  } else {
    if (!pl.off) FMX_TRY(plan_ensure_dense(m, t.tile, e->stream));
    c.bptr = m->plans[(size_t)t.tile].off;
    c.list_entries = m->plans[(size_t)t.tile].cnt;
  }
  *out = c;
  return FMX_OK;
}

static int long_args(fmx_engine* e, fmx_matrix* m, int64_t tile, LongArgs* la, ColsArgs* c) {
  const auto& pl = m->plans[(size_t)tile];
  if (pl.n_long == 0) return FMX_OK;
  const int64_t need = m->max_long_seg * (2 * (int64_t)mb_kp(e) + 4);
  if (need > e->long_partial_cap) {
    FMX_HIP(hipStreamSynchronize(e->stream));
    (void)hipFree(e->long_partial); e->long_partial = nullptr; e->long_partial_cap = 0;
    FMX_HIP(hipMalloc(&e->long_partial, (size_t)need * sizeof(double)));
    e->long_partial_cap = need;
  }
  *la = LongArgs{pl.lfeat, pl.lpos, pl.lseg_ptr, pl.seg_list, pl.seg_begin, pl.seg_end, e->long_partial, (int64_t)pl.n_long, (int64_t)pl.n_seg};
  c->long_min = list_long_min();
  return FMX_OK;
}

static int run_step(fmx_engine* e, fmx_matrix* m, int64_t batch, int64_t rows_limit, bool finish_local, bool empty_share = false) {
  std::vector<TileRun> tiles;
  int64_t step_rows = 0;
  FMX_TRY(step_tiles(e, m, batch, rows_limit, &tiles, &step_rows));
  if (empty_share) { tiles.clear(); step_rows = 0; }
  if (tiles.empty()) {
    if (finish_local) return FMX_OK;
    tiles.push_back({m->step_first_tile[(size_t)batch], 0, 0});
  }
  const bool single = tiles.size() == 1;
  if (!(single && finish_local)) FMX_TRY(ensure_gbuf(e));
  int64_t partials = 0;
  for (size_t i = 0; i < tiles.size(); ++i) {
    int64_t np = 0;
    FMX_TRY(rows_phase(e, m, tiles[i], step_rows, partials, &np));
    partials += np;
    const bool last = i + 1 == tiles.size();
    ColsArgs c{};
    FMX_TRY(cols_args(e, m, tiles[i], single && finish_local, &c));
    c.load_gbuf = i > 0;
    c.store_gbuf = !(last && finish_local);
    c.apply = last && finish_local;
    c.scalar = !last ? SCALAR_NONE : (finish_local ? SCALAR_FUSED : SCALAR_PUBLISH);
    c.n_partials = last ? partials : 0;
    c.global_rows = (double)step_rows;
    LongArgs la{};
    FMX_TRY(long_args(e, m, tiles[i].tile, &la, &c));
    FMX_TRY(launch_cols_update(e, c, la));
  }
  return FMX_OK;
}

static int grad_begin(fmx_engine* e, fmx_matrix* m, int64_t batch, int64_t rows_limit) {
  std::vector<TileRun> tiles;
  int64_t step_rows = 0;
  FMX_TRY(step_tiles(e, m, batch, rows_limit, &tiles, &step_rows));
  FMX_TRY(ensure_gbuf(e));
  const int64_t cap = e->cfg.batch_rows < m->n ? e->cfg.batch_rows : (m->n > 0 ? m->n : 1);
  FMX_TRY(ensure_workspace(e, cap, cap, (int64_t)tiles.size()));
  e->open_tiles.clear();
  int64_t partials = 0, s_row0 = 0;
  for (const TileRun& t : tiles) {
    int64_t np = 0;
    FMX_TRY(rows_phase(e, m, t, step_rows, partials, &np, s_row0));
    partials += np;
    e->open_tiles.push_back({t.tile, t.r0, t.nrows, s_row0});
    s_row0 += t.nrows;
  }
  e->open_rows = step_rows;
  e->open_partials = partials;
  e->open_matrix = m;
  e->open_generation = m->plan_generation;
  ColsArgs c{};
  c.f0 = c.f1 = (uint32_t)e->p;
  c.scalar = SCALAR_PUBLISH;
  c.n_partials = partials;
  c.global_rows = (double)step_rows;
  return launch_cols_update(e, c, LongArgs{});
}

static int grad_block(fmx_engine* e, fmx_matrix* m, int64_t block) {
  FMX_CHECK(e->open_matrix == m && m != nullptr, FMX_ERR_STATE, "fmx_grad_chunk needs a preceding fmx_grad_begin on the same matrix");
  FMX_CHECK(e->open_generation == m->plan_generation, FMX_ERR_STATE, "the matrix's tile plans changed since fmx_grad_begin (another tiling, or scales / normalize): begin the step again");
  FMX_CHECK(block >= 0 && block < e->gb_blocks, FMX_ERR_INVALID, "chunk %lld out of range (0..%lld)", (long long)block, (long long)e->gb_blocks - 1);
  const uint32_t f0 = (uint32_t)(block * e->gb_feats);
  const uint32_t f1 = (uint32_t)(((block + 1) * e->gb_feats < (int64_t)e->p) ? (block + 1) * e->gb_feats : (int64_t)e->p);
  if (e->open_tiles.empty()) {
    ColsArgs c{};
    c.f0 = f0; c.f1 = f1; c.store_gbuf = 1;
    return launch_cols_update(e, c, LongArgs{});
  }
  for (size_t i = 0; i < e->open_tiles.size(); ++i) {
    const auto& ot = e->open_tiles[i];
    const TileRun t{ot.tile, ot.r0, ot.nrows};
    ColsArgs c{};
    FMX_TRY(cols_args(e, m, t, false, &c));
    c.f0 = f0; c.f1 = f1;
    c.s_row0 = ot.s_row0;
    c.load_gbuf = i > 0;
    c.store_gbuf = 1;
    c.global_rows = (double)e->open_rows;
    LongArgs la{};
    FMX_TRY(long_args(e, m, t.tile, &la, &c));
    FMX_TRY(launch_cols_update(e, c, la));
  }
  return FMX_OK;
}

static int apply_block(fmx_engine* e, int64_t block, int64_t global_rows, bool last) {
  FMX_CHECK(e->gbuf != nullptr, FMX_ERR_STATE, "fmx_apply_chunk needs a preceding fmx_grad_begin");
  FMX_CHECK(block >= 0 && block < e->gb_blocks, FMX_ERR_INVALID, "chunk %lld out of range (0..%lld)", (long long)block, (long long)e->gb_blocks - 1);
  ColsArgs c{};
  c.f0 = (uint32_t)(block * e->gb_feats);
  c.f1 = (uint32_t)(((block + 1) * e->gb_feats < (int64_t)e->p) ? (block + 1) * e->gb_feats : (int64_t)e->p);
  c.load_gbuf = 1;
// ... 50 lines not shown
  if (tiles.empty()) tiles.push_back({m->step_first_tile[(size_t)batch], 0, 0});
  const auto& pl = m->plans[(size_t)tiles[0].tile];
  FMX_CHECK(pl.feat != nullptr, FMX_ERR_STATE, "the compact exchange needs sparse tiles (fewer entries than features per tile); use fmx_grad for dense ones");
  FMX_TRY(ensure_compact(e, (int64_t)pl.n_lists > 0 ? (int64_t)pl.n_lists : 1));
  int64_t np = 0;
  FMX_TRY(rows_phase(e, m, tiles[0], step_rows, 0, &np));
  ColsArgs c{};
  FMX_TRY(cols_args(e, m, tiles[0], true, &c));
  c.store_compact = 1;
  c.compact_tail = 1;
  c.scalar = SCALAR_PUBLISH;
  c.n_partials = np;
  c.global_rows = (double)step_rows;
  if (e->owner_parts > 1) {
    FMX_TRY(ensure_owner_plan(e, m, tiles[0].tile));
    c.rec_pos = m->plans[(size_t)tiles[0].tile].own_pos;
  }
  LongArgs la{};
  FMX_TRY(long_args(e, m, tiles[0].tile, &la, &c));
  e->crec_count = pl.dcounts;
  e->crec_n = (int64_t)pl.n_lists;
  return launch_cols_update(e, c, la);
}

int group_grad_empty(fmx_engine* e, fmx_matrix* m, int64_t batch) { return run_step(e, m, batch, 0, false, true); }
int group_grad_compact(fmx_engine* e, fmx_matrix* m, int64_t batch, int64_t rows) { return grad_compact(e, m, batch, rows, rows <= 0); }

}

using namespace fmx;

extern "C" {

const char* fmx_last_error(void) { return g_error.c_str(); }

int fmx_device_count(int32_t* count) {
  FMX_CHECK(count != nullptr, FMX_ERR_INVALID, "count is NULL");
  int c = 0;
  const hipError_t err = hipGetDeviceCount(&c);
  *count = (err == hipSuccess) ? c : 0;
  if (err != hipSuccess || c <= 0) { set_error("no HIP device available (%s); libfmx has no CPU fallback", err == hipSuccess ? "device count 0" : hipGetErrorString(err)); return FMX_ERR_NOGPU; }
  return FMX_OK;
}

int fmx_config_default(fmx_config* cfg) {
  FMX_CHECK(cfg != nullptr, FMX_ERR_INVALID, "cfg is NULL");
  memset(cfg, 0, sizeof(*cfg));
  cfg->struct_size = sizeof(fmx_config);
  cfg->task = FMX_TASK_CLASSIFICATION;
  cfg->solver = FMX_SOLVER_SGD;
  cfg->num_factor = 2;
  cfg->keep_w0 = 1; cfg->keep_w1 = 1;
  cfg->learn_rate = 0.01;
  cfg->alpha_w = 0.1; cfg->alpha_v = 0.1; cfg->beta_w = 1.0; cfg->beta_v = 1.0;
  cfg->random_step = 1;
  cfg->mode = FMX_MODE_SEQUENTIAL;
  cfg->batch_rows = 65536;
  cfg->min_target = -1.0; cfg->max_target = 1.0;
  cfg->device = 0;
  cfg->batch_reduce = FMX_REDUCE_MEAN;
  cfg->gamma = 1e-4;
  cfg->n_gpus = 1;
  return FMX_OK;
}

int fmx_engine_create(const fmx_config* cfg, uint64_t num_features, fmx_engine** out) {
  FMX_CHECK(out != nullptr, FMX_ERR_INVALID, "out is NULL");
  *out = nullptr;
  FMX_CHECK(cfg != nullptr, FMX_ERR_INVALID, "cfg is NULL");
  FMX_CHECK(cfg->struct_size == sizeof(fmx_config), FMX_ERR_INVALID, "fmx_config size mismatch (%u vs %zu): header/library skew",
            cfg->struct_size, sizeof(fmx_config));
  FMX_CHECK(cfg->task == FMX_TASK_CLASSIFICATION || cfg->task == FMX_TASK_REGRESSION || cfg->task == FMX_TASK_RANKING, FMX_ERR_INVALID, "unknown task...");
  if (cfg->task == FMX_TASK_RANKING) {
    FMX_CHECK(cfg->mode == FMX_MODE_MINIBATCH && (cfg->solver == FMX_SOLVER_SGD || cfg->solver == FMX_SOLVER_FTRL), FMX_ERR_INVALID,
              "FMX_TASK_RANKING runs in FMX_MODE_MINIBATCH with FMX_SOLVER_SGD or FMX_SOLVER_FTRL only (got mode %d, solver %d)", cfg->mode, cfg->solver);
    FMX_CHECK(cfg->batch_rows % 2 == 0 && cfg->tile_rows % 2 == 0, FMX_ERR_INVALID,
              "FMX_TASK_RANKING needs an even batch_rows and an even (or 0) tile_rows: a step or tile may not split a pair (got %lld, %lld)",
              (long long)cfg->batch_rows, (long long)cfg->tile_rows);
  }
  FMX_CHECK(cfg->solver == FMX_SOLVER_SGD || cfg->solver == FMX_SOLVER_FTRL || cfg->solver == FMX_SOLVER_ALS || cfg->solver == FMX_SOLVER_TDAP ||
                cfg->solver == FMX_SOLVER_MCMC,
            FMX_ERR_INVALID, "Unknown solver...");
  FMX_CHECK(cfg->num_factor >= 0 && cfg->num_factor <= 128, FMX_ERR_INVALID, "factor.number must be in 0..128 (got %d)", cfg->num_factor);
  FMX_CHECK(cfg->mode == FMX_MODE_SEQUENTIAL || cfg->mode == FMX_MODE_MINIBATCH, FMX_ERR_INVALID, "unknown mode %d", cfg->mode);
  FMX_CHECK(cfg->random_step >= 1, FMX_ERR_INVALID, "random_step must be >= 1");
  FMX_CHECK(cfg->n_gpus >= 0, FMX_ERR_INVALID, "n_gpus must be >= 0");
  FMX_CHECK(cfg->als_max_levels >= -2, FMX_ERR_INVALID, "als_max_levels must be >= 0, or -1 / -2 (the coloured orders)");
  FMX_CHECK(cfg->batch_reduce == FMX_REDUCE_MEAN || cfg->batch_reduce == FMX_REDUCE_SUM, FMX_ERR_INVALID, "unknown batch_reduce %d", cfg->batch_reduce);
  FMX_CHECK(num_features > 0 && num_features < (1ull << 32), FMX_ERR_INVALID, "number of features must be in 1..2^32-1");
  if (cfg->mode == FMX_MODE_MINIBATCH) FMX_CHECK(cfg->batch_rows >= 1 && cfg->tile_rows >= 0, FMX_ERR_INVALID, "batch_rows must be >= 1 and tile_rows >= 0");
  FMX_TRY(use_device(cfg->device));

  std::unique_ptr<fmx_engine, int (*)(fmx_engine*)> e(new fmx_engine(), fmx_engine_destroy);
  e->cfg = *cfg;
  e->p = num_features;
  e->k = cfg->num_factor;
  e->kp32 = pad_factor(e->k, 4);
  e->kp64 = pad_factor(e->k, 2);
  FMX_TRY(make_hyper(*cfg, &e->hyper));
  FMX_HIP(hipStreamCreateWithFlags(&e->stream, hipStreamNonBlocking));
  FMX_TRY(dev_alloc_zero(&e->scal_base, (size_t)2 * SC_COUNT));
  e->scal = e->scal_base;
  e->scal_next = e->scal_base + SC_COUNT;
  const size_t p = (size_t)e->p;
  if (cfg->mode == FMX_MODE_MINIBATCH && !cfg->state_fp64) {
    {
      const char* v = getenv("FMX_W_IN_ROW");
      const bool want = v ? v[0] == '1' : num_features >= 3000000ull;
      e->w_in_row = (want && e->kp32 <= WIR_MAX_KP && e->k > 0) ? 1 : 0;
      e->vstride32 = e->w_in_row ? 2 * e->kp32 : e->kp32;
    }
    FMX_TRY(dev_alloc_zero(&e->V, p * e->vstride32));
    if (!e->w_in_row) FMX_TRY(dev_alloc_zero(&e->w, p));
    if (e->hyper.kind != UPD_SGD_L2) { FMX_TRY(dev_alloc_zero(&e->sV, p * e->kp32)); FMX_TRY(dev_alloc_zero(&e->sw, p)); }
    if (e->hyper.kind == UPD_FTRL || e->hyper.kind == UPD_TDAP) { FMX_TRY(dev_alloc_zero(&e->nV, p * e->kp32)); FMX_TRY(dev_alloc_zero(&e->nw, p)); }
    if (e->hyper.kind == UPD_TDAP) {
      FMX_TRY(dev_alloc_zero(&e->t1V, p * e->kp32)); FMX_TRY(dev_alloc_zero(&e->t1w, p));
      FMX_TRY(dev_alloc_zero(&e->t2V, p * e->kp32)); FMX_TRY(dev_alloc_zero(&e->t2w, p));
      FMX_TRY(dev_alloc_zero(&e->t3V, p * e->kp32)); FMX_TRY(dev_alloc_zero(&e->t3w, p));
    }
  } else {
    FMX_TRY(dev_alloc_zero(&e->dV, p * e->kp64));
    FMX_TRY(dev_alloc_zero(&e->dw, p));
    if (e->hyper.kind != UPD_SGD_L2) { FMX_TRY(dev_alloc_zero(&e->dsV, p * e->kp64)); FMX_TRY(dev_alloc_zero(&e->dsw, p)); }
    if (e->hyper.kind == UPD_FTRL || e->hyper.kind == UPD_TDAP) { FMX_TRY(dev_alloc_zero(&e->dnV, p * e->kp64)); FMX_TRY(dev_alloc_zero(&e->dnw, p)); }
    if (e->hyper.kind == UPD_TDAP) {
      FMX_TRY(dev_alloc_zero(&e->dt1V, p * e->kp64)); FMX_TRY(dev_alloc_zero(&e->dt1w, p));
      FMX_TRY(dev_alloc_zero(&e->dt2V, p * e->kp64)); FMX_TRY(dev_alloc_zero(&e->dt2w, p));
      FMX_TRY(dev_alloc_zero(&e->dt3V, p * e->kp64)); FMX_TRY(dev_alloc_zero(&e->dt3w, p));
    }
  }
  FMX_HIP(hipDeviceSynchronize());
  if (cfg->n_gpus > 1) FMX_TRY(group_create(e.get()));
  *out = e.release();
  return FMX_OK;
}

int fmx_engine_destroy(fmx_engine* e) {
  if (!e) return FMX_OK;
  group_destroy(e);
  (void)hipSetDevice(e->cfg.device);
  if (e->stream) (void)hipStreamSynchronize(e->stream);
  for (auto& pr : e->prof_pending) { (void)hipEventDestroy(pr.second.first); (void)hipEventDestroy(pr.second.second); }
  if (e->rows_tune.events) for (auto& ev : e->rows_tune.ev) (void)hipEventDestroy(ev);
  (void)hipFree(e->scal_base);
  (void)hipFree(e->V); (void)hipFree(e->w); (void)hipFree(e->sV); (void)hipFree(e->sw); (void)hipFree(e->nV); (void)hipFree(e->nw);
  (void)hipFree(e->t1V); (void)hipFree(e->t1w); (void)hipFree(e->t2V); (void)hipFree(e->t2w); (void)hipFree(e->t3V); (void)hipFree(e->t3w);
  (void)hipFree(e->dV); (void)hipFree(e->dw); (void)hipFree(e->dsV); (void)hipFree(e->dsw); (void)hipFree(e->dnV); (void)hipFree(e->dnw);
  (void)hipFree(e->dt1V); (void)hipFree(e->dt1w); (void)hipFree(e->dt2V); (void)hipFree(e->dt2w); (void)hipFree(e->dt3V); (void)hipFree(e->dt3w);
  (void)hipFree(e->seq_b); (void)hipFree(e->seq_len); (void)hipFree(e->seq_y);
  (void)hipFree(e->seq_packed); (void)hipFree(e->seq_conf); (void)hipFree(e->seq_keys); (void)hipFree(e->seq_sort_tmp);
  (void)hipFree(e->long_partial); (void)hipFree(e->probit);
  (void)hipFree(e->S); (void)hipFree(e->amul); (void)hipFree(e->partials); (void)hipFree(e->gbuf);
  (void)hipFree(e->rows_pace); (void)hipFree(e->rows_pace_trace);
  (void)hipFree(e->crec); (void)hipFree(e->ctail); merge_ws_free(e->merge); (void)hipFree(e->als_qe_new); (void)hipFree(e->als_Q); (void)hipFree(e->als_qe); (void)hipFree(e->als_dyn); (void)hipFree(e->als_backup); (void)hipFree(e->als_tile_ws); (void)hipFree(e->als_lo[0]); (void)hipFree(e->als_lo[1]); (void)hipFree(e->als_hash_word); (void)hipFree(e->als_lam_mu); (void)hipFree(e->als_persist_ctl); (void)hipFree(e->als_rec);
  als_graph_free(e->als_graph_w); als_graph_free(e->als_graph_v);
  if (e->side_fork) (void)hipEventDestroy(e->side_fork);
  if (e->side_join) (void)hipEventDestroy(e->side_join);
  if (e->side) (void)hipStreamDestroy(e->side);
  if (e->stream) (void)hipStreamDestroy(e->stream);
  delete e;
  return FMX_OK;
}

int fmx_set_params(fmx_engine* e, double w0, const double* w, const double* v) {
  FMX_CHECK(e != nullptr, FMX_ERR_INVALID, "NULL engine");
  FMX_TRY(use_device(e->cfg.device));
  FMX_HIP(hipStreamSynchronize(e->stream));
  FMX_HIP(hipMemcpy(e->scal + SC_W0, &w0, sizeof(double), hipMemcpyHostToDevice));
  e->als_q_invalidate();
  FMX_TRY(params_to_device(e, w, v));
  e->trace_iters.clear(); e->trace_evals.clear(); e->trace_params.clear();
  FMX_TRY(reset_optimizer_state(e));
  FMX_HIP(hipDeviceSynchronize());
  if (e->group) FMX_TRY(group_set_params(e, w0, w, v));
  return FMX_OK;
}

int fmx_get_params(fmx_engine* e, double* w0, double* w, double* v) {
  FMX_CHECK(e != nullptr, FMX_ERR_INVALID, "NULL engine");
  FMX_TRY(use_device(e->cfg.device));
  FMX_HIP(hipStreamSynchronize(e->stream));
  FMX_TRY(seq_abort_check(e));
  if (w0) FMX_HIP(hipMemcpy(w0, e->scal + SC_W0, sizeof(double), hipMemcpyDeviceToHost));
  FMX_TRY(params_from_device(e, w, v));
  return FMX_OK;
}

int fmx_init_normal(fmx_engine* e, uint64_t seed, double mean, double stdev) {
  FMX_CHECK(e != nullptr, FMX_ERR_INVALID, "NULL engine");
  FMX_TRY(use_device(e->cfg.device));
  FMX_TRY(fmx_set_params(e, 0.0, nullptr, nullptr));
  FMX_TRY(init_normal(e, seed, mean, stdev));
  FMX_HIP(hipStreamSynchronize(e->stream));
  if (e->group) FMX_TRY(group_init_normal(e, seed, mean, stdev));
  return FMX_OK;
}

static int rows_io(fmx_engine* e, const uint32_t* ids, int64_t n, double* w, double* v, bool set) {
  FMX_CHECK(e != nullptr && n >= 0 && (n == 0 || ids), FMX_ERR_INVALID, "bad argument");
  for (int64_t i = 0; i < n; ++i) FMX_CHECK((uint64_t)ids[i] < e->p, FMX_ERR_INVALID, "feature id %u out of range", ids[i]);
  FMX_TRY(use_device(e->cfg.device));
  if (n == 0) return FMX_OK;
  uint32_t* d_ids = nullptr; double *d_w = nullptr, *d_v = nullptr;
  const size_t kk = (size_t)(e->k > 0 ? e->k : 1);
  int st = FMX_OK;
  auto body = [&]() -> int {
    FMX_HIP(hipMalloc(&d_ids, (size_t)n * sizeof(uint32_t)));
    FMX_HIP(hipMalloc(&d_w, (size_t)n * sizeof(double)));
    FMX_HIP(hipMalloc(&d_v, (size_t)n * kk * sizeof(double)));
    FMX_HIP(hipMemcpy(d_ids, ids, (size_t)n * sizeof(uint32_t), hipMemcpyHostToDevice));
    if (set) {
      FMX_TRY(rows_copy(e, d_ids, n, d_w, d_v, false));
      FMX_HIP(hipStreamSynchronize(e->stream));
      if (w) FMX_HIP(hipMemcpy(d_w, w, (size_t)n * sizeof(double), hipMemcpyHostToDevice));
      if (v && e->k > 0) FMX_HIP(hipMemcpy(d_v, v, (size_t)n * kk * sizeof(double), hipMemcpyHostToDevice));
    }
    FMX_TRY(rows_copy(e, d_ids, n, d_w, d_v, set));
    FMX_HIP(hipStreamSynchronize(e->stream));
    if (!set) {
      if (w) FMX_HIP(hipMemcpy(w, d_w, (size_t)n * sizeof(double), hipMemcpyDeviceToHost));
      if (v && e->k > 0) FMX_HIP(hipMemcpy(v, d_v, (size_t)n * kk * sizeof(double), hipMemcpyDeviceToHost));
    }
    return FMX_OK;
  };
  st = body();
  (void)hipFree(d_ids); (void)hipFree(d_w); (void)hipFree(d_v);
  return st;
}

int fmx_get_rows(fmx_engine* e, const uint32_t* ids, int64_t n, double* w, double* v) { return rows_io(e, ids, n, w, v, false); }
int fmx_set_rows(fmx_engine* e, const uint32_t* ids, int64_t n, const double* w, const double* v) {
  if (e) e->als_q_invalidate();
  FMX_TRY(rows_io(e, ids, n, const_cast<double*>(w), const_cast<double*>(v), true));
  if (e->group) FMX_TRY(group_set_rows(e, ids, n, w, v));
  return FMX_OK;
}

namespace fmx {

struct CkptHeader {
  char magic[4];
  uint32_t version;
  uint64_t p;
  int32_t k, kp, mode, kind;
  uint32_t scalars;
  uint32_t reserved[7];
};
static_assert(sizeof(CkptHeader) == 64, "checkpoint header is 64 bytes");

static void ckpt_tables(fmx_engine* e, std::vector<std::pair<void*, size_t>>* out) {
  const size_t p = (size_t)e->p;
  auto add = [&](void* ptr, size_t bytes) { if (ptr) out->push_back({ptr, bytes}); };
  add(e->V, p * (e->vstride32 ? e->vstride32 : e->kp32) * sizeof(float)); add(e->w, p * sizeof(float));
  add(e->sV, p * e->kp32 * sizeof(float)); add(e->sw, p * sizeof(float));
  add(e->nV, p * e->kp32 * sizeof(float)); add(e->nw, p * sizeof(float));
  add(e->t1V, p * e->kp32 * sizeof(float)); add(e->t1w, p * sizeof(float));
  add(e->t2V, p * e->kp32 * sizeof(float)); add(e->t2w, p * sizeof(float));
  add(e->t3V, p * e->kp32 * sizeof(float)); add(e->t3w, p * sizeof(float));
  add(e->dV, p * e->kp64 * sizeof(double)); add(e->dw, p * sizeof(double));
  add(e->dsV, p * e->kp64 * sizeof(double)); add(e->dsw, p * sizeof(double));
  add(e->dnV, p * e->kp64 * sizeof(double)); add(e->dnw, p * sizeof(double));
  add(e->dt1V, p * e->kp64 * sizeof(double)); add(e->dt1w, p * sizeof(double));
  add(e->dt2V, p * e->kp64 * sizeof(double)); add(e->dt2w, p * sizeof(double));
  add(e->dt3V, p * e->kp64 * sizeof(double)); add(e->dt3w, p * sizeof(double));
}

extern "C++" void engine_tables(fmx_engine* e, std::vector<std::pair<void*, size_t>>* out, bool params_only) {
  std::vector<std::pair<void*, size_t>> all;
  ckpt_tables(e, &all);
  for (auto& t : all) {
    const bool param = t.first == (void*)e->V || t.first == (void*)e->w || t.first == (void*)e->dV || t.first == (void*)e->dw;
    if (!params_only || param) out->push_back({t.first, t.second / (size_t)(e->p ? e->p : 1)});
  }
}

static CkptHeader ckpt_header(const fmx_engine* e) {
  CkptHeader h{};
  memcpy(h.magic, "FMX1", 4);
  h.version = 1; h.p = e->p; h.k = e->k; h.kp = wide_state(e) ? e->kp64 : e->kp32; h.mode = e->cfg.mode; h.kind = e->hyper.kind;
  h.scalars = SC_COUNT;
  h.reserved[0] = mb_wide(e) ? 1u : 0u;
  h.reserved[1] = 0u;
  return h;
}

constexpr size_t CKPT_PIECE = 1u << 18;
static bool ckpt_save_params32(fmx_engine* e, FILE* f) {
  const size_t p = (size_t)e->p, kp = (size_t)e->kp32, ds = (size_t)e->vstride32;
  std::vector<float> dev(CKPT_PIECE * ds), rows(CKPT_PIECE * kp), w(p);
  for (size_t j0 = 0; j0 < p; j0 += CKPT_PIECE) {
    const size_t c = p - j0 < CKPT_PIECE ? p - j0 : CKPT_PIECE;
    if (hipMemcpy(dev.data(), e->V + j0 * ds, c * ds * sizeof(float), hipMemcpyDeviceToHost) != hipSuccess) return false;
    for (size_t j = 0; j < c; ++j) {
      memcpy(&rows[j * kp], &dev[j * ds], kp * sizeof(float));
      w[j0 + j] = dev[j * ds + kp];
    }
    if (fwrite(rows.data(), sizeof(float), c * kp, f) != c * kp) return false;
  }
  return fwrite(w.data(), sizeof(float), p, f) == p;
}
static bool ckpt_load_params32(fmx_engine* e, FILE* f, bool file_wir) {
  const size_t p = (size_t)e->p, kp = (size_t)e->kp32, ds = (size_t)e->vstride32, fs = file_wir ? 2 * kp : kp;
  std::vector<float> dev(CKPT_PIECE * ds), rows(CKPT_PIECE * fs), w(p, 0.f);
  if (!file_wir && e->w_in_row) {
    const long at = ftell(f);
    if (at < 0 || fseek(f, (long)(p * kp * sizeof(float)), SEEK_CUR) != 0 || fread(w.data(), sizeof(float), p, f) != p || fseek(f, at, SEEK_SET) != 0) return false;
// ... 1047 lines not shown

int fmx_mcmc_vsweep(fmx_engine* e, fmx_matrix* m, double* error, double alpha, const double* v_lambda, const double* v_mu,
                    const double* std_normals) {
  FMX_CHECK(std_normals != nullptr, FMX_ERR_INVALID, "std_normals is NULL (use fmx_als_vsweep for the ALS form)");
  return vsweep_impl(e, m, error, alpha, v_lambda, v_mu, std_normals);
}

int fmx_vsweep_device(fmx_engine* e, fmx_matrix* m, void* dev_error_f64, double alpha, const double* v_lambda, const double* v_mu, const void* dev_std_normals_f64) {
  FMX_TRY(check_pair(e, m));
  FMX_CHECK(seq_mode(e), FMX_ERR_STATE, "the ALS sweep runs on the fp64 tables: create the engine with FMX_MODE_SEQUENTIAL");
  FMX_CHECK(dev_error_f64 != nullptr || m->n == 0, FMX_ERR_INVALID, "dev_error_f64 is NULL");
  FMX_TRY(use_device(e->cfg.device));
  if (m->n == 0 || e->k == 0) return FMX_OK;
  return launch_als_vsweep_device(e, m, (double*)dev_error_f64, alpha, v_lambda, v_mu, (const double*)dev_std_normals_f64);
}

int fmx_als_plan_info(fmx_engine* e, fmx_matrix* m, int64_t* levels, int64_t* largest_level, int32_t* approximate, int32_t* level_of_feature) {
  FMX_TRY(check_pair(e, m));
  FMX_CHECK(seq_mode(e), FMX_ERR_STATE, "the ALS sweeps run on the fp64 tables: create the engine with FMX_MODE_SEQUENTIAL");
  FMX_TRY(use_device(e->cfg.device));
  return als_plan_info(e, m, levels, largest_level, approximate, level_of_feature);
}

int fmx_als_tiled_info(fmx_engine* e, fmx_matrix* m, int32_t* levels_tiled, int64_t* tile_rows, int32_t* n_tiles) {
  FMX_TRY(check_pair(e, m));
  FMX_CHECK(seq_mode(e), FMX_ERR_STATE, "the ALS sweeps run on the fp64 tables: create the engine with FMX_MODE_SEQUENTIAL");
  FMX_TRY(use_device(e->cfg.device));
  FMX_TRY(als_plan_info(e, m, nullptr, nullptr, nullptr, nullptr));
  return als_tiled_info(m, levels_tiled, tile_rows, n_tiles);
}

int fmx_als_order_info(fmx_engine* e, fmx_matrix* m, int32_t* level_order) {
  FMX_TRY(check_pair(e, m));
  FMX_CHECK(seq_mode(e), FMX_ERR_STATE, "the ALS sweeps run on the fp64 tables: create the engine with FMX_MODE_SEQUENTIAL");
  FMX_CHECK(level_order != nullptr, FMX_ERR_INVALID, "NULL argument");
  FMX_TRY(use_device(e->cfg.device));
  FMX_TRY(als_plan_info(e, m, nullptr, nullptr, nullptr, nullptr));
  *level_order = als_order_form(m);
  return FMX_OK;
}

int fmx_als_carry_q(fmx_engine* e, int32_t on) {
  FMX_CHECK(e != nullptr, FMX_ERR_INVALID, "NULL engine");
  e->als_carry_q = on ? 1 : 0;
  e->als_q_have = 0;
  return FMX_OK;
}

int fmx_als_train(fmx_engine* e, fmx_matrix* m, int32_t max_iter, int32_t with_v) {
  FMX_TRY(check_pair(e, m));
  FMX_CHECK(seq_mode(e), FMX_ERR_STATE, "ALS runs on the fp64 tables: create the engine with FMX_MODE_SEQUENTIAL");
  FMX_CHECK(max_iter >= 0, FMX_ERR_INVALID, "max_iter must be >= 0");
  FMX_CHECK(m->has_labels, FMX_ERR_STATE, "there are no labels in data");
  FMX_TRY(use_device(e->cfg.device));
  if (m->n == 0 || max_iter == 0) return FMX_OK;
  return launch_als_train(e, m, max_iter, with_v);
}

int fmx_mcmc_train(fmx_engine* e, fmx_matrix* m, int32_t max_iter, const double* std_gammas, const double* std_normals, double* state_out) {
  FMX_TRY(check_pair(e, m));
  FMX_CHECK(seq_mode(e), FMX_ERR_STATE, "MCMC runs on the fp64 tables: create the engine with FMX_MODE_SEQUENTIAL");
  FMX_CHECK(max_iter >= 0, FMX_ERR_INVALID, "max_iter must be >= 0");
  FMX_CHECK(m->has_labels, FMX_ERR_STATE, "there are no labels in data");
  FMX_CHECK(max_iter == 0 || (std_gammas != nullptr && std_normals != nullptr), FMX_ERR_INVALID, "the pre-drawn variates are NULL");
  FMX_TRY(use_device(e->cfg.device));
  if (m->n == 0 || max_iter == 0) return FMX_OK;
  return launch_mcmc_train(e, m, max_iter, std_gammas, std_normals, state_out);
}

int fmx_mcmc_train_from(fmx_engine* e, fmx_matrix* m, int32_t max_iter, const double* std_gammas, const double* std_normals, double* state_io) {
  FMX_TRY(check_pair(e, m));
  FMX_CHECK(seq_mode(e), FMX_ERR_STATE, "MCMC runs on the fp64 tables: create the engine with FMX_MODE_SEQUENTIAL");
  FMX_CHECK(state_io != nullptr, FMX_ERR_INVALID, "state_io is NULL (use fmx_mcmc_train to start a chain)");
  FMX_CHECK(max_iter >= 0, FMX_ERR_INVALID, "max_iter must be >= 0");
  FMX_CHECK(m->has_labels, FMX_ERR_STATE, "there are no labels in data");
  FMX_CHECK(max_iter == 0 || (std_gammas != nullptr && std_normals != nullptr), FMX_ERR_INVALID, "the pre-drawn variates are NULL");
  FMX_TRY(use_device(e->cfg.device));
  if (m->n == 0 || max_iter == 0) return FMX_OK;
  const double in[3] = {state_io[0], state_io[1], state_io[2]};
  return launch_mcmc_train(e, m, max_iter, std_gammas, std_normals, state_io, in);
}

int fmx_mcmc_v_hyper(fmx_engine* e, const double* std_gammas, const double* std_normals, double* v_lambda, double* v_mu, int32_t sample) {
  FMX_CHECK(e != nullptr && v_lambda != nullptr && v_mu != nullptr, FMX_ERR_INVALID, "NULL argument");
  FMX_CHECK(seq_mode(e), FMX_ERR_STATE, "MCMC / ALS run on the fp64 tables: create the engine with FMX_MODE_SEQUENTIAL");
  FMX_CHECK(!sample || (std_gammas != nullptr && std_normals != nullptr), FMX_ERR_INVALID, "the pre-drawn variates are NULL");
  FMX_TRY(use_device(e->cfg.device));
  return launch_mcmc_v_hyper(e, std_gammas, std_normals, v_lambda, v_mu, sample);
}

int fmx_rccl_selftest(int32_t n, double* max_err) { return group_rccl_selftest(n, max_err); }

int fmx_debug_fail_next_plan_build(void) { debug_fail_next_plan_build(); return FMX_OK; }
int fmx_debug_fail_next_comm_init(void) { debug_fail_next_comm_init(); return FMX_OK; }
int fmx_debug_lose_next_seq_multiplier(void) { debug_lose_next_seq_multiplier(); return FMX_OK; }
int fmx_debug_stall_next_persistent_sweep(void) { debug_stall_next_persistent_sweep(); return FMX_OK; }
int fmx_debug_contrib_summary_chunk(int64_t entries) { debug_contrib_summary_chunk(entries); return FMX_OK; }
int fmx_debug_foldin_slab(int64_t rows, int64_t groups) { debug_foldin_slab(rows, groups); return FMX_OK; }
int fmx_debug_heldout_limits(int32_t window, int64_t chunk) { debug_heldout_limits(window, chunk); return FMX_OK; }
int fmx_debug_pairs_hard_chunk(int64_t contexts) { debug_pairs_hard_chunk(contexts); return FMX_OK; }
int fmx_debug_lists_limits(int32_t lds_entries, int64_t chunk) { debug_lists_limits(lds_entries, chunk); return FMX_OK; }
int fmx_debug_diversify_limits(int32_t lds_rows, int64_t chunk) { debug_diversify_limits(lds_rows, chunk); return FMX_OK; }
int fmx_debug_neighbors_limits(int64_t slice_items, int64_t chunk_rows) { debug_neighbors_limits(slice_items, chunk_rows); return FMX_OK; }
int fmx_debug_interactions_limits(int32_t wave_entries, int32_t tile_entries, int64_t summary_rows_per_group) {
  debug_interactions_limits(wave_entries, tile_entries, summary_rows_per_group);
  return FMX_OK;
}
int fmx_debug_metrics_limits(int32_t wave_rows, int32_t lds_rows, int64_t chunk_rows) { debug_metrics_limits(wave_rows, lds_rows, chunk_rows); return FMX_OK; }
int fmx_debug_calibrate_limits(int64_t chunk_rows) { debug_calibrate_limits(chunk_rows); return FMX_OK; }
int fmx_debug_take_limits(int32_t fixed_entries, int32_t group_entries, int64_t rows_per_launch) {
  debug_take_limits(fixed_entries, group_entries, rows_per_launch);
  return FMX_OK;
}
int fmx_debug_long_launches(int64_t* out) {
  FMX_CHECK(out != nullptr, FMX_ERR_INVALID, "out is NULL");
  debug_long_launches(out);
  return FMX_OK;
}
int fmx_debug_rows_launches(int64_t* out) {
  FMX_CHECK(out != nullptr, FMX_ERR_INVALID, "out is NULL");
  debug_rows_launches(out);
  return FMX_OK;
}
int fmx_debug_rows_merged_launches(int64_t* out) {
  FMX_CHECK(out != nullptr, FMX_ERR_INVALID, "out is NULL");
  debug_rows_merged_launches(out);
  return FMX_OK;
}
int fmx_debug_rows_sched_launches(int64_t* out) {
  FMX_CHECK(out != nullptr, FMX_ERR_INVALID, "out is NULL");
  debug_rows_sched_launches(out);
  return FMX_OK;
}
int fmx_debug_rows_pace_launches(int64_t* out) {
  FMX_CHECK(out != nullptr, FMX_ERR_INVALID, "out is NULL");
  debug_rows_pace_launches(out);
  return FMX_OK;
}
int fmx_debug_rows_pace_counters_of(fmx_engine* e, int32_t replica, uint32_t* out) {
  FMX_CHECK(e != nullptr && out != nullptr, FMX_ERR_INVALID, "NULL engine or out");
  fmx_engine* r = group_replica(e, replica);
  FMX_CHECK(r != nullptr, FMX_ERR_INVALID, "no replica %d", (int)replica);
  FMX_HIP(hipSetDevice(r->cfg.device));
  const int st = debug_rows_pace_counters(r, out);
  (void)hipSetDevice(e->cfg.device);
  return st;
}
int fmx_debug_rows_pace_counters(fmx_engine* e, uint32_t* out) { return fmx_debug_rows_pace_counters_of(e, 0, out); }
int fmx_debug_rows_pace_poison(fmx_engine* e, uint32_t value) {
  FMX_CHECK(e != nullptr, FMX_ERR_INVALID, "NULL engine");
  for (int i = 0; group_replica(e, i) != nullptr; ++i) { fmx_engine* r = group_replica(e, i); r->rows_pace_poisoned = 1; r->rows_pace_poison = value; }
  return FMX_OK;
}
int fmx_debug_rows_pace_trace(fmx_engine* e, uint64_t* out, int64_t cap_words, int64_t* waves) {
  FMX_CHECK(e != nullptr && waves != nullptr, FMX_ERR_INVALID, "NULL engine or waves");
  return debug_rows_pace_trace(e, out, cap_words, waves);
}
int fmx_debug_rows_sched_id_limit(uint32_t limit) { debug_rows_sched_id_limit(limit); return FMX_OK; }
int fmx_debug_rows_sched_export(const fmx_matrix* m, int64_t tile, int64_t block, uint32_t* out, int64_t cap_words, int64_t* steps, int64_t* info) {
  FMX_CHECK(m != nullptr, FMX_ERR_INVALID, "NULL matrix");
  if (info) { info[0] = (int64_t)m->rows_sched.bytes; info[1] = (int64_t)(m->rows_sched.build_ms * 1e3); info[2] = m->rows_sched.policy; info[3] = m->rows_sched.rho_q; }
  return debug_rows_sched_export(m, tile, block, out, cap_words, steps);
}
int fmx_group_info(fmx_engine* e, int32_t* n_replicas, int32_t* share_device, int32_t* peer_pairs, int32_t* peer_pairs_direct, int32_t* sparse_exchange) {
  FMX_CHECK(e != nullptr, FMX_ERR_INVALID, "NULL engine");
  return group_info(e, n_replicas, share_device, peer_pairs, peer_pairs_direct, sparse_exchange);
}

int fmx_profile_enable(fmx_engine* e, int on) {
  FMX_CHECK(e != nullptr, FMX_ERR_INVALID, "NULL engine");
  FMX_TRY(prof_collect(e));
  e->profile = on > 0 ? on : 0;
  for (int i = 0; i < FMX_KERNEL_COUNT; ++i) e->prof_seen[i] = 0;
  return FMX_OK;
}

int fmx_profile_get(fmx_engine* e, int kernel, double* total_ms, int64_t* launches) {
  FMX_CHECK(e != nullptr && kernel >= 0 && kernel < FMX_KERNEL_COUNT, FMX_ERR_INVALID, "bad kernel id");
  FMX_TRY(prof_collect(e));
  if (total_ms) *total_ms = e->prof_ms[kernel];
  if (launches) *launches = e->prof_n[kernel];
  return FMX_OK;
}

int fmx_rows_tune_info(fmx_engine* e, int32_t* serial, double* ms_serial, double* ms_pipelined) {
  FMX_CHECK(e != nullptr, FMX_ERR_INVALID, "NULL engine");
  if (serial) *serial = e->rows_tune.decided;
  if (ms_serial) *ms_serial = e->rows_tune.ms[1];
  if (ms_pipelined) *ms_pipelined = e->rows_tune.ms[0];
  return FMX_OK;
}

int fmx_matrix_rows_form(const fmx_matrix* m, int32_t* form) {
  FMX_CHECK(m != nullptr && form != nullptr, FMX_ERR_INVALID, "NULL matrix or output");
  *form = rows_ragged(m) ? 2 : (rows_flat(m) ? 1 : 0);
  return FMX_OK;
}

int fmx_layout_info(fmx_engine* e, int32_t* v_row_stride, int32_t* w_in_row) {
  FMX_CHECK(e != nullptr, FMX_ERR_INVALID, "NULL engine");
  if (v_row_stride) *v_row_stride = wide_state(e) ? e->kp64 : e->vstride32;
  if (w_in_row) *w_in_row = (!wide_state(e) && e->w_in_row) ? 1 : 0;
  return FMX_OK;
}

int fmx_profile_reset(fmx_engine* e) {
  FMX_CHECK(e != nullptr, FMX_ERR_INVALID, "NULL engine");
  FMX_TRY(prof_collect(e));
  for (int i = 0; i < FMX_KERNEL_COUNT; ++i) { e->prof_ms[i] = 0; e->prof_n[i] = 0; }
  return FMX_OK;
}

}
```

fmwr_amd/csrc/fmx_internal.h:

```cpp
#pragma once
#include <hip/hip_runtime.h>

#include <cstdarg>
#include <cstdint>
#include <cstdio>
#include <cstdlib>
#include <functional>
#include <string>
#include <utility>
#include <vector>

#include "../../include/fmx.h"

namespace fmx {

void set_error(const char* fmt, ...);

#define FMX_HIP(call)                                                                         \
  do {                                                                                        \
    hipError_t _e = (call);                                                                   \
    if (_e != hipSuccess) {                                                                   \
      fmx::set_error("%s failed: %s (%s:%d)", #call, hipGetErrorString(_e), __FILE__, __LINE__); \
      return FMX_ERR_HIP;                                                                     \
    }                                                                                         \
// ... 67 lines not shown
  uint64_t uid = 0;
  int device = 0;
  int64_t n = 0;
  uint32_t p = 0;
  int64_t nnz = 0;
  int64_t* row_ptr = nullptr;
  uint32_t* col = nullptr;
  float* val = nullptr;
  float* y = nullptr;
  int has_labels = 0;
  int rows_sorted = 0;
  int fixed_row_len = 0;
  int unit_values = 0;
  int dense_prefix = 0;
  std::vector<uint32_t> field_base;
  int max_row_len = 0;
  int64_t batch_rows = 0;
  int64_t tile_rows = 0;
  int64_t n_batches = 0;
  std::vector<int64_t> step_first_tile;
  struct TilePlan {
    int64_t r0 = 0, nrows = 0;
    int64_t base = 0, cnt = 0;
    uint32_t* off = nullptr;
    uint32_t* feat = nullptr;
    uint32_t* soff = nullptr;
    uint32_t* row0 = nullptr;
    uint32_t* val0 = nullptr;
    uint32_t n_lists = 0;
    uint32_t cap_lists = 0;
    uint32_t* lfeat = nullptr;
    uint32_t* lpos = nullptr;
    uint32_t* lseg_ptr = nullptr;
    uint32_t* seg_list = nullptr;
    uint32_t* seg_begin = nullptr;
    uint32_t* seg_end = nullptr;
    uint32_t n_long = 0, n_seg = 0, cap_long = 0, cap_seg = 0;
    uint32_t* dcounts = nullptr;
    void* pool = nullptr;
    int off_in_pool = 0;
    int own_n = 0;
    uint32_t* own_pos = nullptr;
    uint32_t* own_ids = nullptr;
    uint32_t* own_counts = nullptr;
    int64_t own_counts_h[17] = {0};
    void* own_pool = nullptr;
    uint32_t own_cap = 0;
  };
  std::vector<TilePlan> plans;
  uint64_t value_generation = 0;
  uint64_t plan_generation = 0;
  int64_t max_long_seg = 0;
  int64_t max_tile_cnt = 0;
  uint32_t* brow = nullptr;
  float* bval = nullptr;
  struct RowsSched {
    uint32_t* words = nullptr;
    uint32_t* dir = nullptr;
    std::vector<int64_t> tile_words;
    std::vector<int64_t> tile_dir;
    int policy = -1, rho_q = 0;
    uint64_t generation = 0;
    int tried = 0;
    size_t bytes = 0;
    double build_ms = 0.0;
  } rows_sched;
  int refilled_in_place = 0;
  int64_t* col_ptr = nullptr;
  uint32_t* crow = nullptr;
  float* cval = nullptr;
  uint32_t* als_feats = nullptr;
  std::vector<int64_t> als_level_ptr;
  uint32_t* als_heavy = nullptr;
  std::vector<int64_t> als_heavy_ptr;
  uint32_t* als_vh = nullptr;
  uint32_t* als_vh_seg0 = nullptr;
  uint32_t* als_vseg_feat = nullptr;
  int64_t* als_vseg_b = nullptr;
  int64_t* als_vseg_e = nullptr;
  double* als_vh_work = nullptr;
  int64_t als_n_vh = 0, als_n_vseg = 0;
  std::vector<int64_t> als_vh_ptr, als_vseg_ptr;
  std::vector<int32_t> als_level_of;
  int als_approx = 0;
  int als_coloured = 0;
  std::vector<int64_t> als_level_maxlen;
  int als_force_exact = 0;
  int als_plan_cap = -1;
  int64_t* als_level_ptr_dev = nullptr;
  uint16_t* als_rank = nullptr;
  int als_rank_state = 0;
  void* als_tiled = nullptr;
  int als_tiled_tried = 0;
};

struct RowsTune {
  static constexpr int TRIALS = 14;
  static constexpr int64_t MIN_ROWS = 65536;
  int decided = -1;
  int launches = 0;
  int64_t key = -1;
  hipEvent_t ev[2 * TRIALS] = {};
  bool events = false;
  double ms[2] = {0, 0};
};

struct fmx_engine {
  fmx_config cfg{};
  fmx::Hyper hyper{};
  uint64_t p = 0;
  int k = 0;
  int kp32 = 0;
  int vstride32 = 0;
  int w_in_row = 0;
  int kp64 = 0;
  hipStream_t stream = nullptr;
  hipStream_t side = nullptr;
  hipEvent_t side_fork = nullptr, side_join = nullptr;
  double* scal = nullptr;
  double* scal_next = nullptr;
  double* scal_base = nullptr;
  float *V = nullptr, *w = nullptr;
  float *sV = nullptr, *sw = nullptr;
  float *nV = nullptr, *nw = nullptr;
  float *t1V = nullptr, *t1w = nullptr;
  float *t2V = nullptr, *t2w = nullptr;
  float *t3V = nullptr, *t3w = nullptr;
  double *dV = nullptr, *dw = nullptr;
  double *dsV = nullptr, *dsw = nullptr;
  double *dnV = nullptr, *dnw = nullptr;
  double *dt1V = nullptr, *dt1w = nullptr;
  double *dt2V = nullptr, *dt2w = nullptr;
  double *dt3V = nullptr, *dt3w = nullptr;
  int64_t* seq_b = nullptr;
  int* seq_len = nullptr;
  float* seq_y = nullptr;
  int64_t seq_cap = 0;
  void* seq_packed = nullptr;
  int32_t* seq_conf = nullptr;
  uint32_t* seq_keys = nullptr;
  void* seq_sort_tmp = nullptr;
  size_t seq_sort_tmp_bytes = 0;
  int64_t seq_wcap = 0;
  int64_t ws_rows = 0;
  int64_t tile_rows = 0;
  void* S = nullptr;
  void* amul = nullptr;
  double* partials = nullptr;
  int64_t ws_partials = 0;
  uint32_t* rows_pace = nullptr;
  int64_t rows_pace_launches = 0;
  int rows_pace_poisoned = 0;
  uint32_t rows_pace_poison = 0;
  uint64_t* rows_pace_trace = nullptr;
  int64_t rows_pace_trace_cap = 0, rows_pace_trace_waves = 0;
  double* probit = nullptr;
  double* long_partial = nullptr;
  int64_t long_partial_cap = 0;
  void* crec = nullptr;
  int64_t crec_cap = 0;
  int rec_elems = 0;
  void* ctail = nullptr;
  uint32_t* crec_count = nullptr;
  int64_t crec_n = 0;
  int owner_parts = 0;
  int owner_rank = 0;
  fmx::MergeWs* merge = nullptr;
  void* als_qe_new = nullptr;
  int64_t als_qe_new_rows = 0;
  double* als_Q = nullptr;
  size_t als_Q_elems = 0;
  void* als_qe = nullptr;
  int64_t als_qe_rows = 0;
  void* als_dyn = nullptr;
  void* als_tile_ws = nullptr;
  size_t als_tile_ws_bytes = 0;
  void* als_lo[2] = {nullptr, nullptr};
  int64_t als_lo_rows = 0;
  int als_lo_cur = 0;
  int als_q_level0 = 0;
  int als_carry_q = 0;
  int als_q_have = 0, als_q_age = 0;
  uint64_t als_q_trusted = 0;
  uint64_t als_q_hash = 0, als_q_plan = 0;
  void* als_hash_word = nullptr;
  double* als_lam_mu = nullptr;
  void als_q_invalidate() { als_q_have = 0; als_q_trusted = 0; }
  uint32_t* als_rec = nullptr;
  int64_t als_rec_rows = 0;
  unsigned int* als_persist_ctl = nullptr;
  const double* als_qnext = nullptr;
  int als_vf_slot = -1, als_vf_buf = 0;
  void *als_graph_w = nullptr, *als_graph_v = nullptr;
  double* als_backup = nullptr;
  size_t als_backup_elems = 0;
  fmx::Group* group = nullptr;
  void* gbuf = nullptr;
  int64_t gbuf_floats = 0;
  int64_t gb_feats = 0, gb_blocks = 0, gb_block_elems = 0;
  struct OpenTile { int64_t tile, r0, nrows, s_row0; };
  std::vector<OpenTile> open_tiles;
  int64_t open_rows = 0;
  int64_t open_partials = 0;
  fmx_matrix* open_matrix = nullptr;
  uint64_t open_generation = 0;
  struct Snapshot { double w0; std::vector<double> w, v; };
  std::vector<int64_t> trace_iters;
  std::vector<double> trace_evals;
  std::vector<Snapshot> trace_params;
  int profile = 0;
  int64_t prof_seen[FMX_KERNEL_COUNT] = {0};
  int prof_open = 0;
  double prof_ms[FMX_KERNEL_COUNT] = {0};
  int64_t prof_n[FMX_KERNEL_COUNT] = {0};
  std::vector<std::pair<int, std::pair<hipEvent_t, hipEvent_t>>> prof_pending;
  RowsTune rows_tune;
};

namespace fmx {

inline bool mb_wide(const fmx_engine* e) { return e->cfg.mode == FMX_MODE_MINIBATCH && e->cfg.state_fp64 != 0; }
inline bool wide_state(const fmx_engine* e) { return e->cfg.mode == FMX_MODE_SEQUENTIAL || e->cfg.state_fp64 != 0; }
inline int mb_kp(const fmx_engine* e) { return mb_wide(e) ? e->kp64 : e->kp32; }
inline int mb_lpr(const fmx_engine* e) { return mb_wide(e) ? e->kp64 / 2 : e->kp32 / 4; }
inline size_t mb_elem(const fmx_engine* e) { return mb_wide(e) ? sizeof(double) : sizeof(float); }
inline int mb_vstride(const fmx_engine* e) { return mb_wide(e) ? e->kp64 : e->vstride32; }
inline void* mb_vbase(const fmx_engine* e) { return mb_wide(e) ? (void*)e->dV : (void*)e->V; }
inline void* mb_wbase(const fmx_engine* e) { return mb_wide(e) ? (void*)e->dw : (e->w_in_row ? (void*)(e->V + e->kp32) : (void*)e->w); }
inline int mb_wstride(const fmx_engine* e) { return (!mb_wide(e) && e->w_in_row) ? e->vstride32 : 1; }
inline bool exchange_has_q(const fmx_engine* e) { return (e->hyper.kind == UPD_FTRL || e->hyper.kind == UPD_TDAP) && !e->hyper.mean; }

struct RowsArgs {
  const int64_t* row_ptr;
  const uint32_t* col;
  const float* val;
  const float* y;
  int64_t r0;
  int64_t nrows;
  const void* V;
  const void* w;
  int vs, ws;
  int vsh, wsh;
  const double* scal;
  void* S;
  void* amul;
  double* partials;
  double* yhat;
  double* qout;
  int64_t qout_t;
  const double* pn_y;
  int link;
  int unit;
  int no_w;
  int embed;
  int wg_threads;
  int split;
  int serial;
  int flat;
  int64_t nmat;
  int sort_rows;
  uint64_t mat_uid;
  int max_row_len;
  int col_skew;
  const uint32_t* sched;
  const uint32_t* sched_dir;
  int sched_state;
  uint32_t sched_vbytes, sched_wbytes;
  int sched_uniform;
  int sched_deal;
  uint32_t* pace;
  int pace_set;
  int pace_zero;
  uint32_t pace_inc;
  uint32_t pace_div, pace_rem;
  int pace_every, pace_lead, pace_sleep;
  uint64_t* pace_trace;
  int fixed_schedule;
};
constexpr size_t FMX_SERIAL_TABLE_MAX = 1ull << 30;
inline int rows_wg_threads(int64_t step_rows, int lpr) { return step_rows * lpr < 512LL * WG_THREADS ? 64 : WG_THREADS; }
inline int rows_split(int64_t step_rows, int lpr) { return (lpr <= 16 && step_rows * lpr < 1024LL * 64) ? 4 : 1; }
inline int rows_ragged(const fmx_matrix* m) {
  const char* s = getenv("FMX_ROWS_PULL");
  return (s && s[0] == '1' && m->fixed_row_len == 0 && m->n > 0) ? 1 : 0;
}
inline int rows_flat(const fmx_matrix* m) {
  if (m->fixed_row_len != 0 || m->n <= 0 || m->nnz <= 0) return 0;
  if ((int64_t)m->max_row_len * WG_THREADS >= (1LL << 31)) return 0;
  const char* s = getenv("FMX_ROWS_FLAT");
  return (s && s[0] == '1') ? 1 : 0;
}
inline int64_t rows_flat_blocks(int64_t r0, int64_t nrows, int g) { return nrows > 0 ? (r0 + nrows - 1) / g - r0 / g + 1 : 0; }
inline int rows_col_skew(const fmx_matrix* m, const fmx_matrix::TilePlan& pl) {
  const uint64_t lists = pl.feat ? pl.n_lists : m->p;
  if (lists == 0 || pl.n_long == 0) return 1;
  return ((uint64_t)pl.cnt <= 32ull * lists && (uint64_t)pl.n_long * 1024ull >= lists) ? 2 : 1;
}
int launch_rows_forward(fmx_engine* e, const RowsArgs& a, bool train, bool fp64_tables);
enum RowsSchedPolicy : int { SCHED_MERGE = 0, SCHED_FRONT = 1, SCHED_ROUND = 2, SCHED_DEAL = 3 };
constexpr int SCHED_STAGE_STEPS = 144;
constexpr uint32_t SCHED_BUBBLE = 0xFFFFFFFFu;
constexpr uint32_t SCHED_MAX_P = (1u << 30) - 1;
bool rows_sched_wanted(fmx_engine* e, const RowsArgs& a, int* policy, int* rho_q);
void rows_sched_count_build();
void debug_rows_sched_launches(int64_t out[3]);
constexpr int PACE_LINE = 32;
constexpr int PACE_WORDS = 2 * 8 * PACE_LINE;
constexpr int PACE_TRACE_WORDS = 16;
void debug_rows_pace_launches(int64_t out[2]);
int debug_rows_pace_counters(fmx_engine* e, uint32_t out[16]);
int debug_rows_pace_trace(fmx_engine* e, uint64_t* out, int64_t cap_words, int64_t* waves);
int rows_sched_build(fmx_matrix* m, int policy, int rho_q, hipStream_t stream);
void rows_sched_free(fmx_matrix* m);
void debug_rows_sched_id_limit(uint32_t limit);
int debug_rows_sched_export(const fmx_matrix* m, int64_t tile, int64_t block, uint32_t* out, int64_t cap_words, int64_t* steps);
int ensure_probit(fmx_engine* e);
int topk_run(fmx_engine* e, const fmx_matrix* C, int64_t r0, int64_t r1, const fmx_matrix* I, const fmx_matrix* X, int K, int link, int64_t* d_index,
             double* d_score);
int heldout_run(fmx_engine* e, const fmx_matrix* C, int64_t r0, int64_t r1, const fmx_matrix* I, const fmx_matrix* H, const fmx_matrix* X, int64_t* d_rank,
                double* d_score, const int32_t* ks, int n_ks, double* pc);
int heldout_means(fmx_engine* e, const double* pc, int64_t n, int cols, double* out, int64_t* counted);
void debug_heldout_limits(int window, int64_t chunk);
int lists_run(fmx_engine* e, const fmx_matrix* C, int64_t r0, int64_t r1, const fmx_matrix* I, const fmx_matrix* Lm, int link, int K, double* d_score,
              int64_t* d_pos, int64_t* d_index, double* d_tscore);
int project_run(fmx_engine* e, const fmx_matrix* m, int64_t r0, int64_t r1, bool with_w0, double* d_base, double* d_s);
void debug_lists_limits(int lds_entries, int64_t chunk);
int diversify_run(fmx_engine* e, const fmx_matrix* I, int64_t n, int P, const int64_t* index, const double* score, int K, double lambda, int relevance,
                  int64_t* oi, double* os, double* om, bool host);
void debug_diversify_limits(int lds_rows, int64_t chunk);
int neighbors_run(fmx_engine* e, const fmx_matrix* Q, int64_t r0, int64_t r1, const fmx_matrix* I, int K, int metric, bool skip_self, int64_t* d_index,
                  double* d_score);
void debug_neighbors_limits(int64_t slice_items, int64_t chunk_rows);
int contrib_run(fmx_engine* e, const fmx_matrix* m, int64_t r0, int64_t r1, double* d_out);
int pairs_build(const fmx_matrix* C, const fmx_matrix* I, const fmx_matrix* X, int n_neg, uint64_t seed, int64_t epoch, fmx_matrix** out,
                fmx_engine* e = nullptr, int n_cand = 1);
void debug_pairs_hard_chunk(int64_t contexts);
int contrib_summary_run(fmx_engine* e, const fmx_matrix* m, double* sum, double* abs_sum, int64_t* count);
int foldin_run(fmx_engine* e, const fmx_matrix* m, const uint32_t* ids, int64_t n_ids, double lw, double lv, int n_newton, bool pairs,
               std::vector<double>* theta, std::vector<int64_t>* rows, std::vector<int32_t>* status);
void debug_foldin_slab(int64_t rows, int64_t groups);
void debug_contrib_summary_chunk(int64_t entries);
struct InterLimits {
  int wave_entries = 0;
  int tile_entries = 0;
  int64_t summary_rows = 0;
};
InterLimits interactions_take_limits();
int interactions_run(fmx_engine* e, const fmx_matrix* m, int64_t r0, int64_t r1, int top_m, const InterLimits& lim, int64_t* d_a, int64_t* d_b, double* d_v);
int interactions_summary_run(fmx_engine* e, const fmx_matrix* m, const uint32_t* groups, int G, const InterLimits& lim, double* sum, double* abs_sum,
                             int64_t* count);
void debug_interactions_limits(int wave_entries, int tile_entries, int64_t summary_rows);
struct MetLimits {
  int wave_rows = 0;
  int lds_rows = 0;
  int64_t chunk_rows = 0;
};
MetLimits metrics_limits();
int metrics_run(fmx_engine* e, const fmx_matrix* m, int64_t r0, int64_t r1, const uint32_t* d_group, int64_t G, int link, const MetLimits& lim, double* d_value,
                int64_t* d_count);
void debug_metrics_limits(int wave_rows, int lds_rows, int64_t chunk_rows);
int predict_calibrated_run(fmx_engine* e, const fmx_matrix* m, int64_t r0, int64_t r1, const uint32_t* d_group, int64_t G, const fmx_calibrator* cal, int link,
                           double* d_out);
int reliability_run(fmx_engine* e, const fmx_matrix* m, int64_t r0, int64_t r1, const uint32_t* d_group, int64_t G, int B, int binning, const fmx_calibrator* cal,
                    int link, int64_t* d_count, double* d_sum_p, double* d_lo_z, double* d_hi_z, int64_t* d_nan_rows, double* d_value);
int platt_run(fmx_engine* e, const fmx_matrix* m, int64_t r0, int64_t r1, const uint32_t* d_group, int64_t G, double lambda, int n_newton, double* d_ab,
              int64_t* d_rows, int32_t* d_status);
int isotonic_run(fmx_engine* e, const fmx_matrix* m, int64_t r0, int64_t r1, const uint32_t* d_group, int64_t G, int B, int32_t* d_n_steps, double* d_thr,
                 double* d_val);
void debug_calibrate_limits(int64_t chunk_rows);
void debug_take_limits(int fixed_entries, int group_entries, int64_t rows_per_launch);
void debug_long_launches(int64_t out[2]);
void debug_rows_launches(int64_t out[6]);
void debug_rows_merged_launches(int64_t out[2]);

enum ScalarMode : int { SCALAR_NONE = 0, SCALAR_FUSED = 1, SCALAR_PUBLISH = 2, SCALAR_FROM_TAIL = 3 };

struct ColsArgs {
  const uint32_t* bptr;
  const uint32_t* brow;
  const float* bval;
  uint32_t rows_active;
  uint32_t long_min;
  const uint32_t* tfeat;
  const uint32_t* toff;
  uint32_t n_tfeat;
  const uint32_t* trow0;
  const uint32_t* tval0;
  int inline0;
  int walk;
  int load_gbuf;
  int store_gbuf;
  int apply;
  int scalar;
  int64_t n_partials;
  double global_rows;
  uint32_t f0, f1;
  int64_t s_row0;
  int store_compact;
  const uint32_t* rec_pos;
  int compact_tail;
  int unit;
  int direct;
  int64_t list_entries;
  int embed;
  int buf_gather;
};
struct LongArgs {
  const uint32_t* lfeat;
  const uint32_t* lpos;
  const uint32_t* lseg_ptr;
  const uint32_t* seg_feat;
  const uint32_t* seg_begin;
  const uint32_t* seg_end;
  double* partial;
  int64_t n_long, n_seg;
};
inline uint32_t list_long_min() {
  static const uint32_t v = [] { const char* s = getenv("FMX_LONG_MIN"); const long x = s ? atol(s) : 0; return x > 0 ? (uint32_t)x : 64u; }();
  return v;
}
constexpr int WIR_MAX_KP = 16;
constexpr uint32_t LIST_SEG = 1024;
int launch_cols_update(fmx_engine* e, const ColsArgs& a, const LongArgs& la);
constexpr int REC_PARTS_MAX = 64;
struct RecParts { int n; int64_t prefix[REC_PARTS_MAX + 1]; int64_t start[REC_PARTS_MAX]; };
int launch_record_keys(fmx_engine* e, const void* recs, const RecParts& parts, int64_t total, uint32_t* keys, uint32_t* pos);
int launch_apply_records(fmx_engine* e, const void* recs, const uint32_t* pos, const uint32_t* roff, const uint32_t* rfeat, const uint32_t* d_n,
                         int64_t max_lists, int64_t global_rows);
struct MergeWs;
int merge_records(fmx_engine* e, const void* recs, const int64_t* counts, const int64_t* starts, int n_parts, int64_t stride, int64_t* total_out);
void merge_ws_free(MergeWs* w);
void merge_result(const fmx_engine* e, const uint32_t** pos, const uint32_t** roff, const uint32_t** rfeat, const uint32_t** d_n);

int launch_seq_learn(fmx_engine* e, const fmx_matrix* m, const int64_t* d_order, int64_t count);
int launch_seq_learn_grid(fmx_engine* const* es, int n, const fmx_matrix* m, const int64_t* d_order, int64_t count);

struct PlanWorkspace {
  int64_t max_cnt = 0;
  uint32_t p = 0;
  int bits = 0;
  uint32_t* keys_out = nullptr;
  uint64_t *vals_in = nullptr, *vals_out = nullptr;
  void* sort_temp = nullptr;
  size_t sort_bytes = 0;
  uint8_t* flags = nullptr;
  uint32_t* nseg = nullptr;
  uint32_t* blk = nullptr;
  void* prim_temp = nullptr;
  size_t prim_bytes = 0;
  uint32_t *fq_counts = nullptr, *fq_totals = nullptr;
  int reserve(int64_t cnt, uint32_t p, hipStream_t stream);
  PlanWorkspace() = default;
  PlanWorkspace(const PlanWorkspace&) = delete;
  PlanWorkspace& operator=(const PlanWorkspace&) = delete;
  ~PlanWorkspace();
};
int plan_alloc(fmx_matrix::TilePlan& t, uint32_t p, int64_t cap_cnt, bool dense);
void plan_free(fmx_matrix::TilePlan& t);
int plan_build(fmx_matrix::TilePlan& t, PlanWorkspace& ws, uint32_t p, const int64_t* row_ptr, const uint32_t* col, const float* val,
               uint32_t* brow, float* bval, hipStream_t stream, int unit_values, int fixed_row_len, int dense_prefix = 0,
               const std::vector<uint32_t>* field_base = nullptr, bool presplit = false);
bool plan_fields_split_applies(const PlanWorkspace& ws, int unit_values, int fixed_row_len, int dense_prefix, const std::vector<uint32_t>* field_base);
// ... 125 lines not shown
```

fmwr_amd/csrc/fmx_test_hooks.h:

```cpp
#ifndef FMX_TEST_HOOKS_H_
#define FMX_TEST_HOOKS_H_
#include <stdint.h>
#ifdef __cplusplus
extern "C" {
#endif
int fmx_debug_fail_next_plan_build(void);
int fmx_debug_fail_next_comm_init(void);
int fmx_debug_lose_next_seq_multiplier(void);
int fmx_debug_stall_next_persistent_sweep(void);
int fmx_debug_contrib_summary_chunk(int64_t entries);
int fmx_debug_foldin_slab(int64_t rows, int64_t groups);
int fmx_debug_heldout_limits(int32_t window, int64_t chunk);
int fmx_debug_pairs_hard_chunk(int64_t contexts);
int fmx_debug_lists_limits(int32_t lds_entries, int64_t chunk);
int fmx_debug_diversify_limits(int32_t lds_rows, int64_t chunk);
int fmx_debug_neighbors_limits(int64_t slice_items, int64_t chunk_rows);
int fmx_debug_interactions_limits(int32_t wave_entries, int32_t tile_entries, int64_t summary_rows_per_group);
int fmx_debug_metrics_limits(int32_t wave_rows, int32_t lds_rows, int64_t chunk_rows);
int fmx_debug_take_limits(int32_t fixed_entries, int32_t group_entries, int64_t rows_per_launch);
int fmx_debug_calibrate_limits(int64_t chunk_rows);
int fmx_debug_columns_limits(int32_t group_entries, int64_t chunk_entries, int64_t rows_per_launch);
int fmx_debug_matrix_flags(const fmx_matrix* m, int32_t* out );
int fmx_debug_cols_launches(int64_t* out);
int fmx_debug_long_launches(int64_t* out);
int fmx_debug_rows_launches(int64_t* out );
int fmx_debug_rows_merged_launches(int64_t* out );
int fmx_debug_rows_sched_launches(int64_t* out );
int fmx_debug_rows_sched_id_limit(uint32_t limit);
int fmx_debug_rows_sched_export(const fmx_matrix* m, int64_t tile, int64_t block, uint32_t* out, int64_t cap_words, int64_t* steps, int64_t* info );
int fmx_debug_rows_pace_launches(int64_t* out );
int fmx_debug_rows_pace_counters(fmx_engine* e, uint32_t* out );
int fmx_debug_rows_pace_counters_of(fmx_engine* e, int32_t replica, uint32_t* out );
int fmx_debug_rows_pace_poison(fmx_engine* e, uint32_t value);
int fmx_debug_rows_pace_trace(fmx_engine* e, uint64_t* out, int64_t cap_words, int64_t* waves);
#ifdef __cplusplus
}
#endif
#endif
```

profiles/rows_pace_sim.py:

```python
import argparse
import os
import sys
import time

import numpy as np

sys.path.insert(0, os.path.dirname(os.path.abspath(__file__)))
import rows_deal_sim as S

STEP_CYCLES = 1870.0
N_STEPS = S.SLOTS * S.NNZ


def arrival_times(rng, rate, start, inside, pace):
    o = rng.normal(0.0, start, S.BLOCKS)
    r = rng.normal(0.0, rate, S.BLOCKS)
    t = np.arange(N_STEPS, dtype=np.float64)
    held = np.zeros((S.BLOCKS, N_STEPS))
    slept = 0
    if pace is not None:
        every, lead, sleep = pace
        delay = np.zeros(S.BLOCKS)
        for k in range(1, (N_STEPS - 1) // every + 1):
            s = k * every
            mine = o + s * (1.0 + r) + delay
            at = (mine[:, None] - o[None, :] - delay[None, :]) / (1.0 + r[None, :])
            seen = np.clip(np.floor(at / every), 0, (N_STEPS - 1) // every).sum(axis=1)
            lead_steps = every * (k - seen / S.BLOCKS) - (every - 1) / 2.0
            level = (lead_steps > lead).astype(int) + (lead_steps > 2 * lead) + (lead_steps > 3 * lead)
            slept += int((level > 0).sum())
            delay = delay + level * sleep * 64.0 / STEP_CYCLES
            held[:, s + 1:] = delay[:, None]
    wg = o[:, None] + t[None, :] * (1.0 + r[:, None]) + held
    waves = np.repeat(wg, 4, axis=0) + rng.normal(0.0, inside, S.BLOCKS * 4)[:, None]
    return waves, slept


def lines_fetched(cols, when_wave):
    when = np.repeat(when_wave, 16, axis=0).ravel()
    order = np.argsort(when, kind="stable")
    flat = cols.ravel()[order]
    v_line, w_line = (flat >> 1).tolist(), ((flat >> 5) + S.W_BASE).tolist()
    lru, miss_v, miss_w = {}, 0, 0
    for v, w in zip(v_line, w_line):
        for key in (v, w):
            if key in lru:
                del lru[key]
            else:
                if key >= S.W_BASE:
                    miss_w += 1
                else:
                    miss_v += 1
                if len(lru) >= S.LRU_LINES:
                    del lru[next(iter(lru))]
            lru[key] = None
    return miss_v, miss_w


def spread(when_wave):
    return {s: float(when_wave[:, s].std()) for s in (0, 32, 64, 96, N_STEPS - 1)}


def main():
    ap = argparse.ArgumentParser()
    ap.add_argument("--rate", type=float, nargs="*", default=[0.0, 0.04, 0.08])
    ap.add_argument("--start", type=float, default=0.7)
    ap.add_argument("--inside", type=float, default=0.7)
    ap.add_argument("--every", type=int, default=8)
    ap.add_argument("--lead", type=float, nargs="*", default=[1.0, 2.0, 4.0])
    ap.add_argument("--sleep", type=int, nargs="*", default=[10, 20])
    ap.add_argument("--seed", type=int, default=1)
    a = ap.parse_args()
    t0 = time.time()
    cols = S.streams(np.random.default_rng(a.seed), "deal")
    print(f"DEAL streams made in {time.time() - t0:.1f} s")
    print("M lines per tile (8 XCDs); spread = sd over the XCD's waves of the time a step is reached, in steps")
    for rate in a.rate:
        w, _ = arrival_times(np.random.default_rng(a.seed + 1000), rate, a.start, a.inside, None)
        v, wl = lines_fetched(cols, w)
        sp = spread(w)
        print(f"rate {rate:.2f}  no pace              V {S.XCDS * v / 1e6:5.2f}  w {S.XCDS * wl / 1e6:4.2f}  spread " + " ".join(f"{s}:{x:.1f}" for s, x in sp.items()), flush=True)
        if rate == 0.0:
            continue
        for lead in a.lead:
            for sleep in a.sleep:
                w, slept = arrival_times(np.random.default_rng(a.seed + 1000), rate, a.start, a.inside, (a.every, lead, sleep))
                v, wl = lines_fetched(cols, w)
                sp = spread(w)
                print(f"rate {rate:.2f}  every {a.every} lead {lead:.0f} sleep {sleep:2d}  V {S.XCDS * v / 1e6:5.2f}  w {S.XCDS * wl / 1e6:4.2f}  spread " +
                      " ".join(f"{s}:{x:.1f}" for s, x in sp.items()) + f"  sleeps {slept}  end {w.max() - w.min():.1f} steps", flush=True)
    print(f"{time.time() - t0:.1f} s")


if __name__ == "__main__":
    main()
```

profiles/rows_pace_trace.py:

```python
import argparse
import ctypes
import json
import os
import sys

import numpy as np

ROOT = os.path.dirname(os.path.dirname(os.path.abspath(__file__)))
sys.path.insert(0, ROOT)
WORDS = 16


def reduce_launch(tr):
    waves = tr.shape[0]
    xcc = (tr[:, 0] & 15).astype(np.int64)
    steps = ((tr[:, 0] >> 8) & 0xFFFF).astype(np.int64)
    slept = ((tr[:, 0] >> 32) & 0xFFFF).astype(np.int64)
    label = (np.arange(waves) // 4) % 8
    labels_ok = all(len(np.unique(xcc[label == lb])) == 1 for lb in range(8)) and len(np.unique(xcc)) == 8
    n = int(steps.min())
    assert n == int(steps.max()) and n >= 32, "the headline's blocks hold the same number of steps"
    at = list(range(0, n, 16))
    stamps = tr[:, 1:1 + len(at) + 1].astype(np.int64)
    t0 = stamps[:, 0].min()
    tm = (stamps - t0).astype(np.float64) * 0.01
    pos = np.array(at + [n], np.float64)
    step_us = float(np.mean((tm[:, -1] - tm[:, 0]) / n))
    out = {"waves": waves, "steps": n, "labels_are_xcds": bool(labels_ok), "launch_us": float(tm[:, -1].max()), "first_step_spread_us": float(tm[:, 0].max()),
           "step_us": step_us, "sleeps": int(slept.sum()), "waves_that_slept": int((slept > 0).sum())}
    drift = np.zeros((8, len(pos)))
    for x in range(8):
        sel = tm[label == x]
        drift[x] = sel.std(axis=0) / step_us
    out["drift_steps_by_step"] = {str(int(s)): float(v) for s, v in zip(pos, drift.mean(axis=0))}
    out["drift_steps_by_step_per_xcd_end"] = [float(v) for v in drift[:, -1]]
    b, a = np.polyfit(pos, (drift ** 2).mean(axis=0), 1)
    out["variance_fit"] = {"at_step_0": float(a), "per_step": float(b), "fixed_share_at_end": float(a / max(a + b * n, 1e-12))}
    frac = [0.1, 0.25, 0.5, 0.75, 0.9]
    lo, hi = float(np.median(tm[:, 0])), float(np.median(tm[:, -1]))
    reached = {}
    for f in frac:
        t = lo + f * (hi - lo)
        sd = []
        for x in range(8):
            sel = tm[label == x]
            sd.append(float(np.std([np.interp(t, w, pos) for w in sel])))
        reached[str(f)] = float(np.mean(sd))
    out["sd_of_step_reached_at_time"] = reached
    for name, j in (("middle", len(pos) // 2), ("end", len(pos) - 1)):
        inside, between = [], []
        for x in range(8):
            sel = tm[label == x][:, j].reshape(-1, 4)
            inside.append(float(np.mean(sel.var(axis=1))))
            between.append(float(sel.mean(axis=1).var()))
        out[f"sd_inside_workgroup_steps_{name}"] = float(np.sqrt(np.mean(inside)) / step_us)
        out[f"sd_between_workgroups_steps_{name}"] = float(np.sqrt(np.mean(between)) / step_us)
    return out


def main():
    ap = argparse.ArgumentParser()
    ap.add_argument("--pace", default="0")
    ap.add_argument("--tune", default=None)
    ap.add_argument("--launches", type=int, default=5)
    ap.add_argument("--rows", type=int, default=262144)
    ap.add_argument("--json", default=None)
    ap.add_argument("--raw", default=None, help="save the last launch's stamps as .npy")
    a = ap.parse_args()
    os.environ["FMX_ROWS_PACE_TRACE"] = "1"
    os.environ["FMX_ROWS_PACE"] = a.pace
    if a.tune:
        os.environ["FMX_ROWS_PACE_TUNE"] = a.tune
    from fmwr_amd import _lib as L
    from fmwr_amd import engine
    lib = L.lib()
    p, z, k, B = 1_000_000, 30, 16, a.rows
    m = engine.Matrix.synthetic_iid(2 * B, p, z, 20240001, law=L.COLUMNS_UNIFORM)
    e = engine.Engine(p, task=L.TASK_CLASSIFICATION, solver=L.SOLVER_SGD, num_factor=k, learn_rate=0.01, l2_w1=1e-4, l2_v=1e-4, mode=L.MODE_MINIBATCH, batch_rows=B)
    e.init_normal(1, 0.0, 0.01)
    for i in range(40):
        e.step(m, i % 2)
    e.sync()
    per = []
    for i in range(a.launches):
        e.step(m, i % 2)
        e.sync()
        waves = ctypes.c_int64(0)
        L.check(lib.fmx_debug_rows_pace_trace(e.h, None, ctypes.c_int64(0), ctypes.byref(waves)))
        if waves.value == 0:
            raise SystemExit("no traced launch: the step did not take the MERGE or DEAL walk of the scheduled form")
        buf = np.zeros(waves.value * WORDS, np.uint64)
        L.check(lib.fmx_debug_rows_pace_trace(e.h, buf.ctypes.data_as(ctypes.c_void_p), ctypes.c_int64(len(buf)), ctypes.byref(waves)))
        per.append(reduce_launch(buf.reshape(-1, WORDS)))
        if a.raw and i == a.launches - 1:
            np.save(a.raw, buf.reshape(-1, WORDS))
    pl = (ctypes.c_int64 * 2)()
    L.check(lib.fmx_debug_rows_pace_launches(pl))
    keys = ["launch_us", "step_us", "first_step_spread_us", "sleeps", "waves_that_slept", "sd_inside_workgroup_steps_middle", "sd_between_workgroups_steps_middle",
            "sd_inside_workgroup_steps_end", "sd_between_workgroups_steps_end"]
    med = {q: float(np.median([r[q] for r in per])) for q in keys}
    med["drift_steps_by_step"] = {s: float(np.median([r["drift_steps_by_step"][s] for r in per])) for s in per[0]["drift_steps_by_step"]}
    med["sd_of_step_reached_at_time"] = {s: float(np.median([r["sd_of_step_reached_at_time"][s] for r in per])) for s in per[0]["sd_of_step_reached_at_time"]}
    med["variance_fit"] = {s: float(np.median([r["variance_fit"][s] for r in per])) for s in per[0]["variance_fit"]}
    out = {"pace": a.pace, "tune": a.tune, "paced_launches": int(pl[0]), "unpaced_launches": int(pl[1]), "labels_are_xcds": all(r["labels_are_xcds"] for r in per),
           "median": med, "launches": per}
    print(json.dumps({q: out[q] for q in ("pace", "tune", "paced_launches", "unpaced_launches", "labels_are_xcds", "median")}, indent=1))
    if a.json:
        with open(a.json, "w") as f:
            json.dump(out, f, indent=1)
    e.close()
    m.close()


if __name__ == "__main__":
    main()
```

Measured before the change: 1.091 billion.

## Add clock-based pacing of row-sweep blocks using previous launch's observed pace

```diff
diff --git a/fmwr_amd/_lib.py b/fmwr_amd/_lib.py
--- a/fmwr_amd/_lib.py
+++ b/fmwr_amd/_lib.py
@@ -64,7 +64,8 @@
               "fmx_debug_contrib_summary_chunk", "fmx_debug_foldin_slab", "fmx_debug_heldout_limits", "fmx_debug_pairs_hard_chunk", "fmx_debug_lists_limits", "fmx_debug_diversify_limits", "fmx_debug_neighbors_limits", "fmx_debug_interactions_limits", "fmx_debug_metrics_limits", "fmx_debug_take_limits", "fmx_debug_calibrate_limits", "fmx_debug_columns_limits", "fmx_debug_matrix_flags", "fmx_debug_cols_launches",
               "fmx_debug_long_launches", "fmx_debug_rows_launches", "fmx_debug_rows_merged_launches",
               "fmx_debug_rows_sched_launches", "fmx_debug_rows_sched_id_limit", "fmx_debug_rows_sched_export",
-              "fmx_debug_rows_pace_launches", "fmx_debug_rows_pace_counters", "fmx_debug_rows_pace_counters_of", "fmx_debug_rows_pace_poison", "fmx_debug_rows_pace_trace"]
+              "fmx_debug_rows_pace_launches", "fmx_debug_rows_pace_counters", "fmx_debug_rows_pace_counters_of", "fmx_debug_rows_pace_poison", "fmx_debug_rows_pace_trace",
+              "fmx_debug_rows_clock_launches", "fmx_debug_rows_clock_records_of", "fmx_debug_rows_clock_poison"]
 
 
 class Config(C.Structure):
diff --git a/fmwr_amd/csrc/fm_batch_kernels.hip b/fmwr_amd/csrc/fm_batch_kernels.hip
--- a/fmwr_amd/csrc/fm_batch_kernels.hip
+++ b/fmwr_amd/csrc/fm_batch_kernels.hip
@@ -523,9 +523,17 @@
 
 __device__ __forceinline__ void pace_sleep(int units) {
   switch (units) {
+    case 3: __builtin_amdgcn_s_sleep(3); break;
+    case 4: __builtin_amdgcn_s_sleep(4); break;
     case 5: __builtin_amdgcn_s_sleep(5); break;
+    case 6: __builtin_amdgcn_s_sleep(6); break;
+    case 8: __builtin_amdgcn_s_sleep(8); break;
+    case 9: __builtin_amdgcn_s_sleep(9); break;
     case 10: __builtin_amdgcn_s_sleep(10); break;
+    case 12: __builtin_amdgcn_s_sleep(12); break;
     case 15: __builtin_amdgcn_s_sleep(15); break;
+    case 16: __builtin_amdgcn_s_sleep(16); break;
+    case 24: __builtin_amdgcn_s_sleep(24); break;
     case 20: __builtin_amdgcn_s_sleep(20); break;
     case 30: __builtin_amdgcn_s_sleep(30); break;
     case 40: __builtin_amdgcn_s_sleep(40); break;
@@ -537,7 +545,24 @@
   }
 }
 
-template <bool UNIFORM, bool PIPE, bool DEAL = false, bool PACE = false, bool TRACE = false>
+enum { PACE_NONE = 0, PACE_COUNTER = 1, PACE_CLOCK = 2 };
+#ifndef FMX_ROWS_PACE_CLOCK_EVERY
+#define FMX_ROWS_PACE_CLOCK_EVERY 24
+#endif
+#ifndef FMX_ROWS_PACE_CLOCK_LEAD
+#define FMX_ROWS_PACE_CLOCK_LEAD 0.5
+#endif
+#ifndef FMX_ROWS_PACE_CLOCK_SLEEP
+#define FMX_ROWS_PACE_CLOCK_SLEEP 30
+#endif
+#ifndef FMX_ROWS_PACE_CLOCK_GAIN
+#define FMX_ROWS_PACE_CLOCK_GAIN 1.00
+#endif
+static_assert((int64_t)((SCHED_STAGE_STEPS - 1) / FMX_ROWS_PACE_CLOCK_EVERY) * 3 * FMX_ROWS_PACE_CLOCK_SLEEP * 64 * 10 <= SCHED_STAGE_STEPS * PACE_STEP_CYCLES, "clock checks x the longest sleep: at most a tenth of the longest block's walk");
+static_assert((int64_t)((120 - 1) / FMX_ROWS_PACE_CLOCK_EVERY) * 3 * FMX_ROWS_PACE_CLOCK_SLEEP * 64 * 10 <= 120 * PACE_STEP_CYCLES, "the same for the headline's 120-step blocks");
+static_assert(FMX_ROWS_PACE_CLOCK_GAIN > 0.0 && FMX_ROWS_PACE_CLOCK_GAIN <= 1.0, "a gain above 1 would hold a launch to a pace slower than the one observed");
+
+template <bool UNIFORM, bool PIPE, bool DEAL = false, int PACE = PACE_NONE, bool TRACE = false>
 __global__ __launch_bounds__(WG_THREADS, 4) void fm_rows_sched_k(RowsArgs a, Hyper h) {
   using T = float;
   constexpr int LPR = 4, VEC = 4, KP = LPR * VEC;
@@ -546,7 +571,7 @@
   static_assert(MERGE_STAGE == SCHED_STAGE_STEPS * NG && MERGE_SLOTS == 4, "the stage holds SCHED_STAGE_STEPS steps of one word per lane group");
   static_assert(UNIFORM || !PIPE, "only the unrolled walk has a round to request together");
   static_assert(!(UNIFORM && DEAL), "a DEAL schedule is walked as a MERGE one");
-  static_assert(!(UNIFORM && (PACE || TRACE)), "the pace and its trace belong to the MERGE and DEAL walks");
+  static_assert(!(UNIFORM && (PACE != PACE_NONE || TRACE)), "the pace and its trace belong to the MERGE and DEAL walks");
   __shared__ uint32_t stage[MERGE_STAGE];
   __shared__ double red[MERGE_RPW];
   __shared__ uint32_t places[DEAL ? NG : 1];
@@ -556,7 +581,7 @@
   const int gid = tid / LPR;
   const int lig = tid % LPR;
   const int64_t R0 = (int64_t)blockIdx.x * MERGE_RPW;
-  if constexpr (PACE) { if (tid == 0) pace_box = 0u; }
+  if constexpr (PACE == PACE_COUNTER) { if (tid == 0) pace_box = 0u; }
   const uint32_t w_hi = a.sched_dir[blockIdx.x + 1];
   uint32_t w_lo = a.sched_dir[blockIdx.x];
   if constexpr (DEAL) {
@@ -636,13 +661,36 @@
     int64_t pace_groups = 0;
     int pace_at = 0, pace_k = 0, pace_slept = 0;
     uint32_t pace_seen = 0;
-    if constexpr (PACE) {
+    if constexpr (PACE == PACE_COUNTER) {
       const uint32_t lab = blockIdx.x & 7u;
       pace_ctr = a.pace + (size_t)(a.pace_set * 8 + (int)lab) * PACE_LINE;
       pace_groups = (int64_t)(a.pace_div + (lab < a.pace_rem ? 1u : 0u));
       pace_at = a.pace_every;
       if (blockIdx.x == 0 && tid < 8 && a.pace_zero)
         __hip_atomic_store(a.pace + (size_t)((a.pace_set ^ 1) * 8 + tid) * PACE_LINE, 0u, __ATOMIC_RELAXED, __HIP_MEMORY_SCOPE_AGENT);
+    }
+    uint64_t clk_t0 = 0;
+    int64_t clk_target = 0;
+    int clk_at = 0x7FFFFFFF;
+    if constexpr (PACE == PACE_CLOCK) {
+      const uint32_t lab = blockIdx.x & 7u;
+      uint32_t target = 0;
+      if (a.clk_read >= 0) {
+        const uint64_t* rec = a.clk + (size_t)(a.clk_read * 8 + (int)lab) * CLK_LINE;
+        const uint64_t sums = __hip_atomic_load(rec, __ATOMIC_RELAXED, __HIP_MEMORY_SCOPE_AGENT);
+        const uint64_t planted = __hip_atomic_load(rec + 1, __ATOMIC_RELAXED, __HIP_MEMORY_SCOPE_AGENT);
+        const uint64_t ticks = sums & ((1ull << CLK_TICK_BITS) - 1), done = sums >> CLK_TICK_BITS;
+        if (planted) target = (uint32_t)planted;
+        else if (done) {
+          const double q8 = (double)a.clk_gain_q10 * 0.25 * (double)ticks / (double)done;
+          target = q8 < 4294967295.0 ? (uint32_t)q8 : 0xFFFFFFFFu;
+        }
+      }
+      clk_target = (int64_t)(uint32_t)__builtin_amdgcn_readfirstlane((int)target);
+      if (clk_target) clk_at = a.pace_every;
+      if (blockIdx.x == 0 && tid < 8 && a.clk_zero)
+        __hip_atomic_store(a.clk + (size_t)(((a.clk_write + 1) % 3) * 8 + tid) * CLK_LINE, (uint64_t)0, __ATOMIC_RELAXED, __HIP_MEMORY_SCOPE_AGENT);
+      clk_t0 = __builtin_amdgcn_s_memrealtime();
     }
     uint64_t* trace = nullptr;
     if constexpr (TRACE) trace = a.pace_trace + ((size_t)blockIdx.x * (WG_THREADS / 64) + tid / 64) * PACE_TRACE_WORDS;
@@ -670,7 +718,7 @@
           for (int i = 0; i < VEC; ++i) { sm[s][i] += tmp[i]; qm[s][i] += tsq[i]; }
         }
       }
-      if constexpr (PACE) {
+      if constexpr (PACE == PACE_COUNTER) {
         if (t == pace_at) {
           ++pace_k;
           if (tid == 64 * (pace_k & 3)) pace_seen = __hip_atomic_fetch_add(pace_ctr, a.pace_inc, __ATOMIC_RELAXED, __HIP_MEMORY_SCOPE_AGENT);
@@ -685,6 +733,22 @@
           if (level) { pace_sleep(level * a.pace_sleep); pace_slept += 1 + (level << 16); }
           pace_at += a.pace_every;
         }
+      }
+      if constexpr (PACE == PACE_CLOCK) {
+        if (t == clk_at) {
+          clk_at += a.pace_every;
+          const int64_t gone = (int64_t)((__builtin_amdgcn_s_memrealtime() - clk_t0) << 10);
+          const int64_t done = 4 * (t + 1), lead = a.pace_lead;
+          const int level = (done - 3 * lead) * clk_target > gone ? 3 : (done - 2 * lead) * clk_target > gone ? 2 : (done - lead) * clk_target > gone ? 1 : 0;
+          if (level) { pace_sleep(level * a.pace_sleep); pace_slept += 1 + (level << 16); }
+        }
+      }
+    }
+    if constexpr (PACE == PACE_CLOCK) {
+      if (tid == 0) {
+        const uint64_t ticks = __builtin_amdgcn_s_memrealtime() - clk_t0;
+        (void)__hip_atomic_fetch_add(a.clk + (size_t)(a.clk_write * 8 + (int)(blockIdx.x & 7u)) * CLK_LINE,
+                                     (ticks & ((1ull << CLK_TICK_BITS) - 1)) | (uint64_t)steps << CLK_TICK_BITS, __ATOMIC_RELAXED, __HIP_MEMORY_SCOPE_AGENT);
       }
     }
     if constexpr (TRACE) {
@@ -1252,14 +1316,18 @@
 static int rows_sched_u() { static const int v = [] { const char* s = getenv("FMX_ROWS_SCHED_U"); return (s && atoi(s) == 4) ? 4 : 1; }(); return v; }
 
 #ifndef FMX_ROWS_PACE_DEFAULT
-#define FMX_ROWS_PACE_DEFAULT 1
+#define FMX_ROWS_PACE_DEFAULT 3
 #endif
 static std::atomic<int64_t> g_rows_pace[2];
 void debug_rows_pace_launches(int64_t out[2]) {
   for (int i = 0; i < 2; ++i) out[i] = g_rows_pace[i].load();
 }
+static std::atomic<int64_t> g_rows_clock[2];
+void debug_rows_clock_launches(int64_t out[2]) {
+  for (int i = 0; i < 2; ++i) out[i] = g_rows_clock[i].load();
+}
 static int rows_pace_mode() {
-  static const int v = [] { const char* s = getenv("FMX_ROWS_PACE"); const int m = s ? atoi(s) : FMX_ROWS_PACE_DEFAULT; return (m >= 0 && m <= 2) ? m : FMX_ROWS_PACE_DEFAULT; }();
+  static const int v = [] { const char* s = getenv("FMX_ROWS_PACE"); const int m = s ? atoi(s) : FMX_ROWS_PACE_DEFAULT; return (m >= 0 && m <= 4) ? m : FMX_ROWS_PACE_DEFAULT; }();
   return v;
 }
 static bool rows_pace_trace_on() { static const bool v = [] { const char* s = getenv("FMX_ROWS_PACE_TRACE"); return s && s[0] == '1'; }(); return v; }
@@ -1273,6 +1341,28 @@
     return t;
   }();
   return v;
+}
+struct ClockTune { int every, lead_q2, sleep, gain_q10; };
+static const ClockTune& rows_clock_tune() {
+  static const ClockTune v = [] {
+    ClockTune t{FMX_ROWS_PACE_CLOCK_EVERY, (int)(FMX_ROWS_PACE_CLOCK_LEAD * 4.0 + 0.5), FMX_ROWS_PACE_CLOCK_SLEEP, (int)(FMX_ROWS_PACE_CLOCK_GAIN * 1024.0 + 0.5)};
+    int ev = 0, sl = 0;
+    double ld = -1.0, g = 0.0;
+    const char* s = getenv("FMX_ROWS_PACE_CLOCK_TUNE");
+    if (s && sscanf(s, "%d,%lf,%d,%lf", &ev, &ld, &sl, &g) == 4 && ev >= 2 && ev <= 64 && ld >= 0.0 && ld <= 64.0 && (sl == 3 || sl == 4 || sl == 5 || sl == 8 || sl == 10 || sl == 20 || sl == 30 || sl == 40) && g > 0.0 && g <= 1.0)
+      t = ClockTune{ev, (int)(ld * 4.0 + 0.5), sl, (int)(g * 1024.0 + 0.5)};
+    return t;
+  }();
+  return v;
+}
+int debug_rows_clock_records(fmx_engine* e, uint64_t out[48]) {
+  for (int i = 0; i < 48; ++i) out[i] = 0;
+  if (!e->rows_clock) return FMX_OK;
+  std::vector<uint64_t> all(CLK_WORDS);
+  FMX_HIP(hipStreamSynchronize(e->stream));
+  FMX_HIP(hipMemcpy(all.data(), e->rows_clock, CLK_WORDS * sizeof(uint64_t), hipMemcpyDeviceToHost));
+  for (int i = 0; i < 24; ++i) { out[2 * i] = all[(size_t)i * CLK_LINE]; out[2 * i + 1] = all[(size_t)i * CLK_LINE + 1]; }
+  return FMX_OK;
 }
 int debug_rows_pace_counters(fmx_engine* e, uint32_t out[16]) {
   for (int i = 0; i < 16; ++i) out[i] = 0;
@@ -1319,30 +1409,50 @@
     const int mode = rows_pace_mode();
     const bool traced = rows_pace_trace_on();
     using SchedKernel = void (*)(RowsArgs, Hyper);
-    static const SchedKernel instance[2][2][2] = {
-        {{fm_rows_sched_k<false, false, false, false, false>, fm_rows_sched_k<false, false, false, false, true>},
-         {fm_rows_sched_k<false, false, false, true, false>, fm_rows_sched_k<false, false, false, true, true>}},
-        {{fm_rows_sched_k<false, false, true, false, false>, fm_rows_sched_k<false, false, true, false, true>},
-         {fm_rows_sched_k<false, false, true, true, false>, fm_rows_sched_k<false, false, true, true, true>}}};
+    static const SchedKernel instance[2][3][2] = {
+        {{fm_rows_sched_k<false, false, false, PACE_NONE, false>, fm_rows_sched_k<false, false, false, PACE_NONE, true>},
+         {fm_rows_sched_k<false, false, false, PACE_COUNTER, false>, fm_rows_sched_k<false, false, false, PACE_COUNTER, true>},
+         {fm_rows_sched_k<false, false, false, PACE_CLOCK, false>, fm_rows_sched_k<false, false, false, PACE_CLOCK, true>}},
+        {{fm_rows_sched_k<false, false, true, PACE_NONE, false>, fm_rows_sched_k<false, false, true, PACE_NONE, true>},
+         {fm_rows_sched_k<false, false, true, PACE_COUNTER, false>, fm_rows_sched_k<false, false, true, PACE_COUNTER, true>},
+         {fm_rows_sched_k<false, false, true, PACE_CLOCK, false>, fm_rows_sched_k<false, false, true, PACE_CLOCK, true>}}};
     const int deal = a.sched_deal ? 1 : 0;
+    const bool clock = mode >= 3;
     bool paced = false;
-    if (mode != 0 && e->rows_pace) {
+    if (mode != 0 && (clock ? e->rows_clock != nullptr : e->rows_pace != nullptr)) {
       constexpr int MAX_DEV = 64;
-      static std::atomic<int64_t> resident_dev[MAX_DEV][2][2];
-      std::atomic<int64_t>& resident = resident_dev[(e->cfg.device >= 0 && e->cfg.device < MAX_DEV) ? e->cfg.device : 0][deal][traced ? 1 : 0];
+      static std::atomic<int64_t> resident_dev[MAX_DEV][2][2][2];
+      std::atomic<int64_t>& resident = resident_dev[(e->cfg.device >= 0 && e->cfg.device < MAX_DEV) ? e->cfg.device : 0][clock ? 1 : 0][deal][traced ? 1 : 0];
       int64_t r = resident.load();
       if (r == 0) {
         hipDeviceProp_t pr{};
         int per = 0;
         if (hipGetDeviceProperties(&pr, e->cfg.device) == hipSuccess && pr.multiProcessorCount > 0 &&
-            hipOccupancyMaxActiveBlocksPerMultiprocessor(&per, instance[deal][1][traced ? 1 : 0], WG_THREADS, 0) == hipSuccess && per > 0)
+            hipOccupancyMaxActiveBlocksPerMultiprocessor(&per, instance[deal][clock ? PACE_CLOCK : PACE_COUNTER][traced ? 1 : 0], WG_THREADS, 0) == hipSuccess && per > 0)
           r = (int64_t)per * pr.multiProcessorCount;
         else r = -1;
         resident.store(r);
       }
       paced = r > 0 && grid <= r;
     }
-    if (paced) {
+    bool with_target = false;
+    if (paced && clock) {
+      const ClockTune& ct = rows_clock_tune();
+      const int64_t n = e->rows_clock_launches;
+      with_target = e->rows_clock_poisoned || (e->rows_clock_prev && e->rows_clock_uid == a.mat_uid && e->rows_clock_gen == a.mat_gen && e->rows_clock_nrows == a.nrows);
+      a.clk = e->rows_clock;
+      a.clk_write = (int)(n % 3);
+      a.clk_read = with_target ? (int)((n + 2) % 3) : -1;
+      a.clk_zero = e->rows_clock_poisoned ? 0 : 1;
+      a.clk_gain_q10 = (uint32_t)ct.gain_q10;
+      a.pace_every = ct.every; a.pace_lead = ct.lead_q2; a.pace_sleep = ct.sleep;
+      if (e->rows_clock_poisoned) {
+        std::vector<uint64_t> img(CLK_WORDS, 0);
+        for (int i = 0; i < 3 * 8; ++i) img[(size_t)i * CLK_LINE + 1] = e->rows_clock_poison;
+        FMX_HIP(hipMemcpyAsync(e->rows_clock, img.data(), CLK_WORDS * sizeof(uint64_t), hipMemcpyHostToDevice, e->stream));
+        FMX_HIP(hipStreamSynchronize(e->stream));
+      }
+    } else if (paced) {
       const PaceTune& pt = rows_pace_tune();
       a.pace = e->rows_pace;
       a.pace_set = (int)(e->rows_pace_launches & 1);
@@ -1364,9 +1474,13 @@
       e->rows_pace_trace_waves = waves;
       a.pace_trace = e->rows_pace_trace;
     }
-    hipLaunchKernelGGL(instance[deal][paced ? 1 : 0][traced ? 1 : 0], dim3((unsigned)grid), dim3(WG_THREADS), 0, e->stream, a, e->hyper);
+    hipLaunchKernelGGL(instance[deal][!paced ? PACE_NONE : clock ? PACE_CLOCK : PACE_COUNTER][traced ? 1 : 0], dim3((unsigned)grid), dim3(WG_THREADS), 0, e->stream, a, e->hyper);
     FMX_HIP(hipGetLastError());
-    if (paced) ++e->rows_pace_launches;
+    if (paced && clock) {
+      ++e->rows_clock_launches;
+      e->rows_clock_prev = 1; e->rows_clock_uid = a.mat_uid; e->rows_clock_gen = a.mat_gen; e->rows_clock_nrows = a.nrows;
+      g_rows_clock[with_target ? 0 : 1]++;
+    } else if (paced) ++e->rows_pace_launches;
     g_rows_pace[paced ? 0 : 1]++;
     g_rows_sched[0]++;
     *ran = true;
@@ -1442,7 +1556,9 @@
   int st = FMX_OK;
   bool merged = false;
   if (train) {
+    const int64_t clocked = e->rows_clock_launches;
     st = launch_rows_sched(e, a, &merged);
+    if (e->rows_clock_launches == clocked) e->rows_clock_prev = 0;
     if (st == FMX_OK && !merged) st = launch_rows_merged<true>(e, a, fp64_tables, &merged);
     if (st == FMX_OK && !merged) {
       int trial;
diff --git a/fmwr_amd/csrc/fmx_api.hip b/fmwr_amd/csrc/fmx_api.hip
--- a/fmwr_amd/csrc/fmx_api.hip
+++ b/fmwr_amd/csrc/fmx_api.hip
@@ -156,6 +156,10 @@
     FMX_HIP(hipMalloc(&e->rows_pace, PACE_WORDS * sizeof(uint32_t)));
     FMX_HIP(hipMemsetAsync(e->rows_pace, 0, PACE_WORDS * sizeof(uint32_t), e->stream));
   }
+  if (!e->rows_clock) {
+    FMX_HIP(hipMalloc(&e->rows_clock, CLK_WORDS * sizeof(uint64_t)));
+    FMX_HIP(hipMemsetAsync(e->rows_clock, 0, CLK_WORDS * sizeof(uint64_t), e->stream));
+  }
   if (s_rows <= e->ws_rows && partials <= e->ws_partials) return FMX_OK;
   FMX_HIP(hipStreamSynchronize(e->stream));
   (void)hipFree(e->S); (void)hipFree(e->amul); (void)hipFree(e->partials);
@@ -342,7 +346,7 @@
   a.wg_threads = rows_wg_threads(step_rows, mb_lpr(e));
   a.split = rows_split(step_rows, mb_lpr(e));
   a.flat = rows_flat(m); a.nmat = m->n;
-  a.mat_uid = m->uid; a.max_row_len = m->max_row_len; a.col_skew = rows_col_skew(m, m->plans[(size_t)t.tile]);
+  a.mat_uid = m->uid; a.mat_gen = m->plan_generation; a.max_row_len = m->max_row_len; a.col_skew = rows_col_skew(m, m->plans[(size_t)t.tile]);
   {
     int policy = 0, rho_q = 0;
     if (rows_sched_wanted(e, a, &policy, &rho_q)) {
@@ -699,7 +703,7 @@
   (void)hipFree(e->seq_packed); (void)hipFree(e->seq_conf); (void)hipFree(e->seq_keys); (void)hipFree(e->seq_sort_tmp);
   (void)hipFree(e->long_partial); (void)hipFree(e->probit);
   (void)hipFree(e->S); (void)hipFree(e->amul); (void)hipFree(e->partials); (void)hipFree(e->gbuf);
-  (void)hipFree(e->rows_pace); (void)hipFree(e->rows_pace_trace);
+  (void)hipFree(e->rows_pace); (void)hipFree(e->rows_clock); (void)hipFree(e->rows_pace_trace);
   (void)hipFree(e->crec); (void)hipFree(e->ctail); merge_ws_free(e->merge); (void)hipFree(e->als_qe_new); (void)hipFree(e->als_Q); (void)hipFree(e->als_qe); (void)hipFree(e->als_dyn); (void)hipFree(e->als_backup); (void)hipFree(e->als_tile_ws); (void)hipFree(e->als_lo[0]); (void)hipFree(e->als_lo[1]); (void)hipFree(e->als_hash_word); (void)hipFree(e->als_lam_mu); (void)hipFree(e->als_persist_ctl); (void)hipFree(e->als_rec);
   als_graph_free(e->als_graph_w); als_graph_free(e->als_graph_v);
   if (e->side_fork) (void)hipEventDestroy(e->side_fork);
@@ -2053,6 +2057,25 @@
   for (int i = 0; group_replica(e, i) != nullptr; ++i) { fmx_engine* r = group_replica(e, i); r->rows_pace_poisoned = 1; r->rows_pace_poison = value; }
   return FMX_OK;
 }
+int fmx_debug_rows_clock_launches(int64_t* out) {
+  FMX_CHECK(out != nullptr, FMX_ERR_INVALID, "out is NULL");
+  debug_rows_clock_launches(out);
+  return FMX_OK;
+}
+int fmx_debug_rows_clock_records_of(fmx_engine* e, int32_t replica, uint64_t* out) {
+  FMX_CHECK(e != nullptr && out != nullptr, FMX_ERR_INVALID, "NULL engine or out");
+  fmx_engine* r = group_replica(e, replica);
+  FMX_CHECK(r != nullptr, FMX_ERR_INVALID, "no replica %d", (int)replica);
+  FMX_HIP(hipSetDevice(r->cfg.device));
+  const int st = debug_rows_clock_records(r, out);
+  (void)hipSetDevice(e->cfg.device);
+  return st;
+}
+int fmx_debug_rows_clock_poison(fmx_engine* e, uint32_t value) {
+  FMX_CHECK(e != nullptr && value != 0u, FMX_ERR_INVALID, "NULL engine, or a target of 0 (which means none)");
+  for (int i = 0; group_replica(e, i) != nullptr; ++i) { fmx_engine* r = group_replica(e, i); r->rows_clock_poisoned = 1; r->rows_clock_poison = value; }
+  return FMX_OK;
+}
 int fmx_debug_rows_pace_trace(fmx_engine* e, uint64_t* out, int64_t cap_words, int64_t* waves) {
   FMX_CHECK(e != nullptr && waves != nullptr, FMX_ERR_INVALID, "NULL engine or waves");
   return debug_rows_pace_trace(e, out, cap_words, waves);
diff --git a/fmwr_amd/csrc/fmx_internal.h b/fmwr_amd/csrc/fmx_internal.h
--- a/fmwr_amd/csrc/fmx_internal.h
+++ b/fmwr_amd/csrc/fmx_internal.h
@@ -243,6 +243,13 @@
   int64_t rows_pace_launches = 0;
   int rows_pace_poisoned = 0;
   uint32_t rows_pace_poison = 0;
+  uint64_t* rows_clock = nullptr;
+  int64_t rows_clock_launches = 0;
+  int rows_clock_prev = 0;
+  uint64_t rows_clock_uid = 0, rows_clock_gen = 0;
+  int64_t rows_clock_nrows = 0;
+  int rows_clock_poisoned = 0;
+  uint32_t rows_clock_poison = 0;
   uint64_t* rows_pace_trace = nullptr;
   int64_t rows_pace_trace_cap = 0, rows_pace_trace_waves = 0;
   double* probit = nullptr;
@@ -351,6 +358,7 @@
   int64_t nmat;
   int sort_rows;
   uint64_t mat_uid;
+  uint64_t mat_gen;
   int max_row_len;
   int col_skew;
   const uint32_t* sched;
@@ -366,6 +374,11 @@
   uint32_t pace_div, pace_rem;
   int pace_every, pace_lead, pace_sleep;
   uint64_t* pace_trace;
+  uint64_t* clk;
+  int clk_write;
+  int clk_read;
+  int clk_zero;
+  uint32_t clk_gain_q10;
   int fixed_schedule;
 };
 constexpr size_t FMX_SERIAL_TABLE_MAX = 1ull << 30;
@@ -398,7 +411,12 @@
 constexpr int PACE_LINE = 32;
 constexpr int PACE_WORDS = 2 * 8 * PACE_LINE;
 constexpr int PACE_TRACE_WORDS = 16;
+constexpr int CLK_LINE = 16;
+constexpr int CLK_WORDS = 3 * 8 * CLK_LINE;
+constexpr int CLK_TICK_BITS = 40;
 void debug_rows_pace_launches(int64_t out[2]);
+void debug_rows_clock_launches(int64_t out[2]);
+int debug_rows_clock_records(fmx_engine* e, uint64_t out[48]);
 int debug_rows_pace_counters(fmx_engine* e, uint32_t out[16]);
 int debug_rows_pace_trace(fmx_engine* e, uint64_t* out, int64_t cap_words, int64_t* waves);
 int rows_sched_build(fmx_matrix* m, int policy, int rho_q, hipStream_t stream);
diff --git a/fmwr_amd/csrc/fmx_test_hooks.h b/fmwr_amd/csrc/fmx_test_hooks.h
--- a/fmwr_amd/csrc/fmx_test_hooks.h
+++ b/fmwr_amd/csrc/fmx_test_hooks.h
@@ -32,6 +32,9 @@
 int fmx_debug_rows_pace_counters(fmx_engine* e, uint32_t* out );
 int fmx_debug_rows_pace_counters_of(fmx_engine* e, int32_t replica, uint32_t* out );
 int fmx_debug_rows_pace_poison(fmx_engine* e, uint32_t value);
+int fmx_debug_rows_clock_launches(int64_t* out );
+int fmx_debug_rows_clock_records_of(fmx_engine* e, int32_t replica, uint64_t* out );
+int fmx_debug_rows_clock_poison(fmx_engine* e, uint32_t value);
 int fmx_debug_rows_pace_trace(fmx_engine* e, uint64_t* out, int64_t cap_words, int64_t* waves);
 #ifdef __cplusplus
 }
diff --git a/profiles/rows_pace_sim.py b/profiles/rows_pace_sim.py
--- a/profiles/rows_pace_sim.py
+++ b/profiles/rows_pace_sim.py
@@ -36,6 +36,32 @@
     return waves, slept
 
 
+def arrival_times_clock(rng, rate, start, inside, clock, launches):
+    every, lead, sleep, gain = clock
+    o = rng.normal(0.0, start, S.BLOCKS)
+    r = rng.normal(0.0, rate, S.BLOCKS)
+    jitter = rng.normal(0.0, inside, S.BLOCKS * 4)
+    t = np.arange(N_STEPS, dtype=np.float64)
+    target, targets = 0.0, []
+    for _ in range(launches):
+        held = np.zeros((S.BLOCKS, N_STEPS))
+        delay = np.zeros(S.BLOCKS)
+        slept = 0
+        if target > 0.0:
+            for k in range(1, (N_STEPS - 1) // every + 1):
+                s = k * every
+                gone = (s + 1) * (1.0 + r) + delay
+                level = sum(((s + 1 - m * lead) * target > gone).astype(int) for m in (1, 2, 3))
+                slept += int((level > 0).sum())
+                delay = delay + level * sleep * 64.0 / STEP_CYCLES
+                held[:, s + 1:] = delay[:, None]
+        targets.append(target)
+        target = gain * float(np.sum(N_STEPS * (1.0 + r) + delay) / (S.BLOCKS * N_STEPS))
+    wg = o[:, None] + t[None, :] * (1.0 + r[:, None]) + held
+    waves = np.repeat(wg, 4, axis=0) + jitter[:, None]
+    return waves, slept, targets
+
+
 def lines_fetched(cols, when_wave):
     when = np.repeat(when_wave, 16, axis=0).ravel()
     order = np.argsort(when, kind="stable")
@@ -70,6 +96,9 @@
     ap.add_argument("--lead", type=float, nargs="*", default=[1.0, 2.0, 4.0])
     ap.add_argument("--sleep", type=int, nargs="*", default=[10, 20])
     ap.add_argument("--seed", type=int, default=1)
+    ap.add_argument("--clock", action="store_true", help="the clock pace in place of the counter pace: --every / --lead / --sleep and --gain")
+    ap.add_argument("--gain", type=float, nargs="*", default=[1.0, 0.97, 0.94])
+    ap.add_argument("--clock-launches", type=int, default=6)
     a = ap.parse_args()
     t0 = time.time()
     cols = S.streams(np.random.default_rng(a.seed), "deal")
@@ -82,7 +111,15 @@
         print(f"rate {rate:.2f}  no pace              V {S.XCDS * v / 1e6:5.2f}  w {S.XCDS * wl / 1e6:4.2f}  spread " + " ".join(f"{s}:{x:.1f}" for s, x in sp.items()), flush=True)
         if rate == 0.0:
             continue
-        for lead in a.lead:
+        for lead in a.lead if a.clock else []:
+            for sleep in a.sleep:
+                for gain in a.gain:
+                    w, slept, targets = arrival_times_clock(np.random.default_rng(a.seed + 1000), rate, a.start, a.inside, (a.every, lead, sleep, gain), a.clock_launches)
+                    v, wl = lines_fetched(cols, w)
+                    sp = spread(w)
+                    print(f"rate {rate:.2f}  clock every {a.every} lead {lead:.0f} sleep {sleep:2d} gain {gain:.2f}  V {S.XCDS * v / 1e6:5.2f}  w {S.XCDS * wl / 1e6:4.2f}  spread " +
+                          " ".join(f"{s}:{x:.1f}" for s, x in sp.items()) + f"  sleeps {slept}  end {w.max() - w.min():.1f} steps  target {targets[-1]:.4f}", flush=True)
+        for lead in [] if a.clock else a.lead:
             for sleep in a.sleep:
                 w, slept = arrival_times(np.random.default_rng(a.seed + 1000), rate, a.start, a.inside, (a.every, lead, sleep))
                 v, wl = lines_fetched(cols, w)
diff --git a/profiles/rows_pace_trace.py b/profiles/rows_pace_trace.py
--- a/profiles/rows_pace_trace.py
+++ b/profiles/rows_pace_trace.py
@@ -62,6 +62,7 @@
     ap = argparse.ArgumentParser()
     ap.add_argument("--pace", default="0")
     ap.add_argument("--tune", default=None)
+    ap.add_argument("--clock-tune", default=None, help="FMX_ROWS_PACE_CLOCK_TUNE for --pace 3 and 4")
     ap.add_argument("--launches", type=int, default=5)
     ap.add_argument("--rows", type=int, default=262144)
     ap.add_argument("--json", default=None)
@@ -71,6 +72,8 @@
     os.environ["FMX_ROWS_PACE"] = a.pace
     if a.tune:
         os.environ["FMX_ROWS_PACE_TUNE"] = a.tune
+    if a.clock_tune:
+        os.environ["FMX_ROWS_PACE_CLOCK_TUNE"] = a.clock_tune
     from fmwr_amd import _lib as L
     from fmwr_amd import engine
     lib = L.lib()
@@ -94,17 +97,19 @@
         per.append(reduce_launch(buf.reshape(-1, WORDS)))
         if a.raw and i == a.launches - 1:
             np.save(a.raw, buf.reshape(-1, WORDS))
-    pl = (ctypes.c_int64 * 2)()
+    pl, cl = (ctypes.c_int64 * 2)(), (ctypes.c_int64 * 2)()
     L.check(lib.fmx_debug_rows_pace_launches(pl))
+    L.check(lib.fmx_debug_rows_clock_launches(cl))
     keys = ["launch_us", "step_us", "first_step_spread_us", "sleeps", "waves_that_slept", "sd_inside_workgroup_steps_middle", "sd_between_workgroups_steps_middle",
             "sd_inside_workgroup_steps_end", "sd_between_workgroups_steps_end"]
     med = {q: float(np.median([r[q] for r in per])) for q in keys}
     med["drift_steps_by_step"] = {s: float(np.median([r["drift_steps_by_step"][s] for r in per])) for s in per[0]["drift_steps_by_step"]}
     med["sd_of_step_reached_at_time"] = {s: float(np.median([r["sd_of_step_reached_at_time"][s] for r in per])) for s in per[0]["sd_of_step_reached_at_time"]}
     med["variance_fit"] = {s: float(np.median([r["variance_fit"][s] for r in per])) for s in per[0]["variance_fit"]}
-    out = {"pace": a.pace, "tune": a.tune, "paced_launches": int(pl[0]), "unpaced_launches": int(pl[1]), "labels_are_xcds": all(r["labels_are_xcds"] for r in per),
+    out = {"pace": a.pace, "tune": a.clock_tune if a.pace in ("3", "4") else a.tune, "paced_launches": int(pl[0]), "unpaced_launches": int(pl[1]),
+           "clock_launches_with_target": int(cl[0]), "clock_launches_without": int(cl[1]), "labels_are_xcds": all(r["labels_are_xcds"] for r in per),
            "median": med, "launches": per}
-    print(json.dumps({q: out[q] for q in ("pace", "tune", "paced_launches", "unpaced_launches", "labels_are_xcds", "median")}, indent=1))
+    print(json.dumps({q: out[q] for q in ("pace", "tune", "paced_launches", "unpaced_launches", "clock_launches_with_target", "clock_launches_without", "labels_are_xcds", "median")}, indent=1))
     if a.json:
         with open(a.json, "w") as f:
             json.dump(out, f, indent=1)
```

After: 1.105 billion, median of 6. 1.3% higher.
